# matthewhoung/inference-arena

Measured on AMD Instinct MI355X. Metric: req/sec (whole node) + P50/P99 e2e latency, YOLOv5n→MobileNetV2 at 1/2/4/8 GPU, higher is better.
Workload: dtype fp32

## Files before the change

### csrc/bindings.cpp

```cpp
#include <pybind11/numpy.h>
#include <pybind11/pybind11.h>
#include <pybind11/stl.h>

#include <cstring>
#include <malloc.h>
#include <map>
#include <mutex>

#include "kernels/launch.h"
#include "runtime/executor.h"
#include "runtime/echo_instance.h"
#include "runtime/http_front.h"
#include "runtime/http_loadgen.h"
#include "runtime/ipc_buffer.h"
#include "runtime/peer.h"
#include "runtime/jpeg_decode.h"
#include "runtime/jpeg_ingest.h"
#include "runtime/batcher.h"
#include "runtime/split.h"
#include "runtime/crash_trace.h"

namespace py = pybind11;
using namespace arena;

namespace arena {
void bind_jpeg(py::module& m);
}

namespace {

template <typename T>
T get(const py::dict& d, const char* k, T dflt) {
  if (!d.contains(k)) return dflt;
  py::object o = d[k];
  if (o.is_none()) return dflt;
  return o.cast<T>();
}
template <typename T>
T req(const py::dict& d, const char* k) {
  if (!d.contains(k)) throw std::runtime_error(std::string("missing kernel parameter '") + k + "'");
  return d[k].cast<T>();
}
template <typename P>
P ptr(const py::dict& d, const char* k) {
  return reinterpret_cast<P>(get<uintptr_t>(d, k, 0));
}
hipStream_t stream_of(const py::dict& d) { return reinterpret_cast<hipStream_t>(get<uintptr_t>(d, "stream", 0)); }

void py_conv2d(const py::dict& d) {
  ConvParams p{};
  p.x = ptr<const void*>(d, "x");
  p.B = req<int>(d, "B");
  p.H = req<int>(d, "H");
  p.W = req<int>(d, "W");
  p.xs = req<int>(d, "xs");
  p.Cin = req<int>(d, "Cin");
  p.w = ptr<const void*>(d, "w");
  p.Kpad = req<int>(d, "Kpad");
  p.bias = ptr<const float*>(d, "bias");
  p.y = ptr<void*>(d, "y");
  p.Ho = req<int>(d, "Ho");
  p.Wo = req<int>(d, "Wo");
  p.ys = req<int>(d, "ys");
  p.Cout = req<int>(d, "Cout");
  p.Cout_pad = req<int>(d, "Cout_pad");
  p.KH = req<int>(d, "KH");
  p.KW = req<int>(d, "KW");
  p.stride = get<int>(d, "stride", 1);
  p.pad_t = get<int>(d, "pad_t", 0);
  p.pad_l = get<int>(d, "pad_l", 0);
  p.res = ptr<const void*>(d, "res");
  p.rs = get<int>(d, "rs", 0);
  p.y2 = ptr<void*>(d, "y2");
  p.y2s = get<int>(d, "y2s", 0);
  p.act = get<int>(d, "act", 0);
  p.f32out = get<int>(d, "f32out", 0);
  p.bdev = ptr<const int*>(d, "bdev");
  p.impl = get<int>(d, "impl", 0);
  p.pw_w = ptr<const void*>(d, "pw_w");
  p.pw_bias = ptr<const float*>(d, "pw_bias");
  p.pw_y = ptr<void*>(d, "pw_y");
  p.pw_ys = get<int>(d, "pw_ys", 0);
  p.pw_cout = get<int>(d, "pw_cout", 0);
  p.pw_kpad = get<int>(d, "pw_kpad", 0);
  p.pw_act = get<int>(d, "pw_act", 0);
  p.gate = ptr<const float*>(d, "gate");
  p.gate_n = get<int>(d, "gate_n", 0);
  p.gate_min = get<float>(d, "gate_min", 0.f);
  p.n_lo = get<int>(d, "n_lo", 0);
  p.n_hi = get<int>(d, "n_hi", 0);
  p.marks = ptr<const int*>(d, "marks");
  p.mark_uh = get<int>(d, "mark_uh", 0);
  p.mark_uw = get<int>(d, "mark_uw", 0);
  p.mark_halo = get<int>(d, "mark_halo", 0);
  p.w3 = ptr<const void*>(d, "w3");
  p.sk_ws = ptr<float*>(d, "sk_ws");
  p.sk_ws_bytes = get<int64_t>(d, "sk_ws_bytes", 0);
  prepare_kernels();
  if (get<int>(d, "f32", 0))
    conv2d_f32(p, stream_of(d));
  else
    conv2d(p, stream_of(d));
}

void py_head_mark(const py::dict& d) {
  HeadMarkParams p{};
  const std::vector<uintptr_t> logits = req<std::vector<uintptr_t>>(d, "logits");
  const std::vector<uintptr_t> marks = req<std::vector<uintptr_t>>(d, "marks");
  const std::vector<int> H = req<std::vector<int>>(d, "H"), W = req<std::vector<int>>(d, "W");
  const std::vector<int> ps = req<std::vector<int>>(d, "ps");
  const size_t n = logits.size();
  if (n < 1 || n > (size_t)kMarkMaxLevels || marks.size() != n || H.size() != n || W.size() != n || ps.size() != n)
    throw std::runtime_error("head_mark: 1..3 levels, one entry per level in every list");
  p.n_levels = (int)n;
  for (size_t l = 0; l < n; ++l) {
    p.logits[l] = reinterpret_cast<const float*>(logits[l]);
    p.marks[l] = reinterpret_cast<int*>(marks[l]);
    p.H[l] = H[l];
    p.W[l] = W[l];
    p.ps[l] = ps[l];
  }
  p.n = req<int>(d, "n");
  p.gate_min = req<float>(d, "gate_min");
  p.B = req<int>(d, "B");
  p.bdev = ptr<const int*>(d, "bdev");
  head_mark(p, stream_of(d));
}

void py_dwconv(const py::dict& d) {
  DwParams p{};
  p.x = ptr<const void*>(d, "x");
  p.B = req<int>(d, "B");
  p.H = req<int>(d, "H");
  p.W = req<int>(d, "W");
  p.xs = req<int>(d, "xs");
  p.C = req<int>(d, "C");
  p.w = ptr<const void*>(d, "w");
  p.bias = ptr<const float*>(d, "bias");
  p.y = ptr<void*>(d, "y");
  p.Ho = req<int>(d, "Ho");
  p.Wo = req<int>(d, "Wo");
  p.ys = req<int>(d, "ys");
  p.stride = get<int>(d, "stride", 1);
  p.act = get<int>(d, "act", 0);
  p.bdev = ptr<const int*>(d, "bdev");
  if (get<int>(d, "f32", 0))
    dwconv3x3_f32(p, stream_of(d));
  else
    dwconv3x3(p, stream_of(d));
}

void py_ir_block(const py::dict& d) {
  IrParams p{};
  p.x = ptr<const void*>(d, "x");
  p.x_cs = req<int>(d, "x_cs");
  p.H = req<int>(d, "H");
  p.W = req<int>(d, "W");
  p.inp = req<int>(d, "inp");
  p.inp_pad = req<int>(d, "inp_pad");
  p.hid_pad = req<int>(d, "hid_pad");
  p.oup = req<int>(d, "oup");
  p.oup_pad = req<int>(d, "oup_pad");
  p.stride = req<int>(d, "stride");
  p.expand = req<int>(d, "expand");
  p.res = get<int>(d, "res", 0);
  p.we = ptr<const void*>(d, "we");
  p.be = ptr<const float*>(d, "be");
  p.wd = ptr<const void*>(d, "wd");
  p.bd = ptr<const float*>(d, "bd");
  p.wp = ptr<const void*>(d, "wp");
  p.bp = ptr<const float*>(d, "bp");
  p.y = ptr<void*>(d, "y");
  p.y_cs = req<int>(d, "y_cs");
  p.Ho = req<int>(d, "Ho");
  p.Wo = req<int>(d, "Wo");
  p.B = req<int>(d, "B");
  p.bdev = ptr<const int*>(d, "bdev");
  p.x3w = get<int>(d, "x3w", 0);
  p.x_parts = get<int>(d, "x_parts", 0);
  p.y_parts = get<int>(d, "y_parts", 0);
  prepare_kernels();
  if (get<int>(d, "f32", 0))
    ir_block_f32(p, stream_of(d));
  else
    ir_block(p, stream_of(d));
}

void py_c3_block(const py::dict& d) {
  C3Params p{};
  p.x = ptr<const void*>(d, "x");
  p.xs = req<int>(d, "xs");
  p.B = req<int>(d, "B");
  p.H = req<int>(d, "H");
  p.W = req<int>(d, "W");
  p.bdev = ptr<const int*>(d, "bdev");
  p.C1 = req<int>(d, "C1");
  p.CH = req<int>(d, "CH");
  p.NB = req<int>(d, "NB");
  p.res = req<int>(d, "res");
  p.w12 = ptr<const void*>(d, "w12");
  p.b12 = ptr<const float*>(d, "b12");
  p.wb1[0] = p.wb1[1] = ptr<const void*>(d, "wb1");
  p.bb1[0] = p.bb1[1] = ptr<const float*>(d, "bb1");
  p.wb2[0] = p.wb2[1] = ptr<const void*>(d, "wb2");
  p.bb2[0] = p.bb2[1] = ptr<const float*>(d, "bb2");
  p.w3 = ptr<const void*>(d, "w3");
  p.b3 = ptr<const float*>(d, "b3");
  p.y = ptr<void*>(d, "y");
  p.ys = req<int>(d, "ys");
  prepare_kernels();
  if (get<int>(d, "f32", 0))
    c3_x3(p, stream_of(d));
  else
    c3_fused(p, stream_of(d));
}

void py_sppf(const py::dict& d) {
  SppfParams p{};
  p.buf = ptr<void*>(d, "buf");
  p.B = req<int>(d, "B");
  p.H = req<int>(d, "H");
  p.W = req<int>(d, "W");
  p.xs = req<int>(d, "xs");
  p.C = req<int>(d, "C");
  p.bdev = ptr<const int*>(d, "bdev");
  if (get<int>(d, "f32", 0))
    sppf_pool_f32(p, stream_of(d));
  else
    sppf_pool(p, stream_of(d));
}

void py_letterbox(const py::dict& d) {
  LetterboxParams p{};
  p.pool = ptr<const uint8_t*>(d, "pool");
  p.meta = ptr<const ImageMeta*>(d, "meta");
  p.ctrl = ptr<const Ctrl*>(d, "ctrl");
  p.out = ptr<void*>(d, "out");
  p.B = req<int>(d, "B");
  p.T = req<int>(d, "T");
  p.f32 = get<int>(d, "f32", 0);
  letterbox_s2d(p, stream_of(d));
}

void py_decode(const py::dict& d) {
  DecodeParams p{};
  auto heads = req<std::vector<uintptr_t>>(d, "head");
  auto hw = req<std::vector<int>>(d, "hw");
  auto xs = req<std::vector<int>>(d, "xs");
  auto st = req<std::vector<float>>(d, "strides");
  for (int l = 0; l < 3; ++l) {
    p.head[l] = (const void*)heads.at(l);
    p.hw[l] = hw.at(l);
    p.xs[l] = xs.at(l);
    p.stride[l] = st.at(l);
  }
  p.B = req<int>(d, "B");
  p.conf_thr = req<float>(d, "conf_thr");
  p.cand = ptr<Candidate*>(d, "cand");
  p.cand_count = ptr<int*>(d, "cand_count");
  p.cand_cap = req<int>(d, "cand_cap");
  p.ctrl = ptr<const Ctrl*>(d, "ctrl");
  p.f32 = get<int>(d, "f32", 0);
  detect_decode(p, stream_of(d));
}

void py_yolo_raw(const py::dict& d) {
  YoloRawParams p{};
  auto heads = req<std::vector<uintptr_t>>(d, "head");
  auto hw = req<std::vector<int>>(d, "hw");
  auto xs = req<std::vector<int>>(d, "xs");
  auto st = req<std::vector<float>>(d, "strides");
  for (int l = 0; l < 3; ++l) {
    p.head[l] = (const void*)heads.at(l);
    p.hw[l] = hw.at(l);
    p.xs[l] = xs.at(l);
    p.stride[l] = st.at(l);
  }
  p.B = req<int>(d, "B");
  p.out = ptr<void*>(d, "out");
  p.out_stride = req<size_t>(d, "out_stride");
  p.ctrl = ptr<const Ctrl*>(d, "ctrl");
  p.f32 = get<int>(d, "f32", 0);
  yolo_raw(p, stream_of(d));
}

void py_tensor_in(const py::dict& d) {
  TensorInParams p{};
  p.pool = ptr<const uint8_t*>(d, "pool");
  p.meta = ptr<const ImageMeta*>(d, "meta");
  p.ctrl = ptr<const Ctrl*>(d, "ctrl");
  p.out = ptr<void*>(d, "out");
  p.B = req<int>(d, "B");
  p.S = req<int>(d, "S");
  p.f32 = get<int>(d, "f32", 0);
  tensor_in_s2d(p, stream_of(d));
}

void py_nms(const py::dict& d) {
  prepare_kernels();
  NmsParams p{};
  p.cand = ptr<const Candidate*>(d, "cand");
  p.cand_count = ptr<const int*>(d, "cand_count");
  p.cand_cap = req<int>(d, "cand_cap");
  p.meta = ptr<const ImageMeta*>(d, "meta");
  p.B = req<int>(d, "B");
  p.iou_thr = req<float>(d, "iou_thr");
  p.det = ptr<Detection*>(d, "det");
  p.det_count = ptr<int*>(d, "det_count");
  p.max_det = req<int>(d, "max_det");
  p.ctrl = ptr<const Ctrl*>(d, "ctrl");
  nms(p, stream_of(d));
}

void py_crop_plan(const py::dict& d) {
  CropPlanParams p{};
  p.det = ptr<Detection*>(d, "det");
  p.det_count = ptr<int*>(d, "det_count");
  p.max_det = req<int>(d, "max_det");
  p.meta = ptr<const ImageMeta*>(d, "meta");
  p.B = req<int>(d, "B");
  p.crops = ptr<CropRef*>(d, "crops");
  p.ctrl = ptr<Ctrl*>(d, "ctrl");
  p.crop_cap = req<int>(d, "crop_cap");
  p.whole = get<int>(d, "whole", 0);
  crop_plan(p, stream_of(d));
}

void py_crop_gather(const py::dict& d) {
  CropGatherParams p{};
  p.pool = ptr<const uint8_t*>(d, "pool");
  p.meta = ptr<const ImageMeta*>(d, "meta");
  p.crops = ptr<const CropRef*>(d, "crops");
  p.ctrl = ptr<const Ctrl*>(d, "ctrl");
  p.out = ptr<void*>(d, "out");
  p.cap = req<int>(d, "cap");
  p.S = req<int>(d, "S");
  auto mean = req<std::vector<float>>(d, "mean");
  auto inv_std = req<std::vector<float>>(d, "inv_std");
  for (int c = 0; c < 3; ++c) {
    p.mean[c] = mean.at(c);
    p.inv_std[c] = inv_std.at(c);
  }
  p.f32 = get<int>(d, "f32", 0);
  crop_gather_s2d(p, stream_of(d));
}

void py_head_pool(const py::dict& d) {
  HeadPoolParams p{};
  p.x = ptr<const void*>(d, "x");
  p.xs = req<int>(d, "xs");
  p.HW = req<int>(d, "HW");
  p.K = req<int>(d, "K");
  p.w = ptr<const void*>(d, "w");
  p.Kpad = req<int>(d, "Kpad");
  p.bias = ptr<const float*>(d, "bias");
  p.N = req<int>(d, "N");
  p.Npad = req<int>(d, "Npad");
  p.y = ptr<void*>(d, "y");
  p.ys = req<int>(d, "ys");
  p.act = get<int>(d, "act", 0);
  p.B = req<int>(d, "B");
  p.bdev = ptr<const int*>(d, "bdev");
  prepare_kernels();
  if (get<int>(d, "f32", 0))
    head_pool_f32(p, stream_of(d));
  else
    head_pool(p, stream_of(d));
}

void py_avgpool(const py::dict& d) {
  AvgPoolParams p{};
  p.x = ptr<const void*>(d, "x");
  p.B = req<int>(d, "B");
  p.HW = req<int>(d, "HW");
  p.C = req<int>(d, "C");
  p.y = ptr<void*>(d, "y");
  p.bdev = ptr<const int*>(d, "bdev");
  p.f32 = get<int>(d, "f32", 0);
  global_avgpool(p, stream_of(d));
}

void py_topk(const py::dict& d) {
  TopkParams p{};
  p.logits = ptr<const float*>(d, "logits");
  p.B = req<int>(d, "B");
  p.N = req<int>(d, "N");
  p.ld = req<int>(d, "ld");
  p.out = ptr<TopkResult*>(d, "out");
  p.ctrl = ptr<const Ctrl*>(d, "ctrl");
  p.bdev = ptr<const int*>(d, "bdev");
  topk_softmax(p, stream_of(d));
}

ExecutorConfig config_from(const py::dict& d) {
  ExecutorConfig c;
  c.device = get<int>(d, "device", c.device);
  c.max_batch = get<int>(d, "max_batch", c.max_batch);
  c.max_det = get<int>(d, "max_det", c.max_det);
  c.cand_cap = get<int>(d, "cand_cap", c.cand_cap);
  c.crop_cap_per_image = get<int>(d, "crop_cap_per_image", c.crop_cap_per_image);
  c.min_crop_cap = get<int>(d, "min_crop_cap", c.min_crop_cap);
  c.pool_bytes_per_image = get<int64_t>(d, "pool_bytes_per_image", c.pool_bytes_per_image);
  c.pool_factor = get<int>(d, "pool_factor", c.pool_factor);
  c.det_size = get<int>(d, "det_size", c.det_size);
  c.cls_size = get<int>(d, "cls_size", c.cls_size);
  c.host_threads = get<int>(d, "host_threads", c.host_threads);
  c.raw_out_bytes = get<int64_t>(d, "raw_out_bytes", c.raw_out_bytes);
  return c;
}

ResultCallback py_result_cb(py::function cb) {
  std::shared_ptr<py::function> pycb(new py::function(std::move(cb)), [](py::function* fn) {
    py::gil_scoped_acquire gil;
    delete fn;
  });
  return [pycb](RequestResult&& r) {
    py::gil_scoped_acquire gil;
    py::dict d;
    d["id"] = r.id;
    d["error"] = r.error;
    d["det_count"] = r.det_count;
    const int k = (int)r.det.size();
    py::array_t<float> det({k, 8});
    if (k) std::memcpy(det.mutable_data(), r.det.data(), sizeof(Detection) * k);
    const int t = (int)r.topk.size();
    py::array_t<int32_t> ti({t, 5});
    py::array_t<float> tl({t, 5}), tp({t, 5});
    for (int i = 0; i < t; ++i)
      for (int j = 0; j < 5; ++j) {
        ti.mutable_at(i, j) = r.topk[i].idx[j];
        tl.mutable_at(i, j) = r.topk[i].logit[j];
        tp.mutable_at(i, j) = r.topk[i].prob[j];
      }
    d["det"] = det;
    d["topk_idx"] = ti;
    d["topk_logit"] = tl;
    d["topk_prob"] = tp;
    if (!r.raw.empty()) {
      py::array_t<uint8_t> raw((py::ssize_t)r.raw.size());
      std::memcpy(raw.mutable_data(), r.raw.data(), r.raw.size());
      d["raw"] = raw;
    }
    d["batch_size"] = r.batch_size;
    d["queue_us"] = r.queue_us;
    d["compute_us"] = r.compute_us;
    d["detection_ms"] = r.det_ms;
    d["classification_ms"] = r.cls_ms;
    try {
      (*pycb)(d);
    } catch (py::error_already_set& e) {
      e.discard_as_unraisable("DynamicBatcher callback");
    }
  };
}

struct JpegHolder {
  JpegInfo info;
  std::vector<int16_t> coef;
};
using JpegKeep = std::vector<std::shared_ptr<JpegHolder>>;
std::mutex g_jkeep_mu;
std::map<std::pair<const void*, int>, JpegKeep> g_jkeep;
struct JpegSet;
std::map<std::pair<const void*, int>, std::shared_ptr<JpegSet>> g_jset_keep;

struct JpegSet {
  struct Item {
    JpegInfo info;
    int16_t* coef = nullptr;
    bool pinned = false;
    ~Item() {
      if (coef == nullptr) return;
      if (pinned) (void)hipHostFree(coef);
      else std::free(coef);
    }
  };
  std::vector<std::shared_ptr<Item>> items;
};

std::shared_ptr<JpegSet> make_jpeg_set(const py::list& uploads, bool pinned) {
  auto set = std::make_shared<JpegSet>();
  for (auto h : uploads) {
    const std::string data = h.cast<std::string>();
    auto it = std::make_shared<JpegSet::Item>();
    std::string err;
    JpegStatus st = jpeg_parse((const uint8_t*)data.data(), data.size(), it->info, err);
    if (st != JpegStatus::Ok) throw py::value_error("JpegSet: not decodable by the split decoder: " + err);
    const bool compact = jpeg_compact_enabled();
    const size_t bytes =
        std::max<size_t>(2, compact ? (size_t)jpeg_compact_capacity(it->info) : (size_t)it->info.coef_count * 2);
    void* p = nullptr;
    if (pinned && hipHostMalloc(&p, bytes, hipHostMallocPortable) == hipSuccess) {
      it->pinned = true;
    } else {
      (void)hipGetLastError();
      p = std::malloc(bytes);
      if (p == nullptr) throw std::bad_alloc();
    }
    it->coef = (int16_t*)p;
    st = compact ? jpeg_decode_compact((const uint8_t*)data.data(), data.size(), it->info, (uint8_t*)it->coef, err)
                 : jpeg_decode_coefs((const uint8_t*)data.data(), data.size(), it->info, it->coef, err);
    if (st != JpegStatus::Ok) throw py::value_error("JpegSet: entropy decode failed: " + err);
    set->items.push_back(it);
  }
  return set;
}

std::vector<InputImage> images_from(const py::list& imgs, std::vector<py::array>& keep, JpegKeep* jkeep = nullptr) {
  std::vector<InputImage> v;
  v.reserve(imgs.size());
  for (auto h : imgs) {
    if (py::isinstance<py::bytes>(h)) {
      if (jkeep == nullptr) throw std::runtime_error("JPEG inputs are not accepted here");
      const std::string data = h.cast<std::string>();
      auto jh = std::make_shared<JpegHolder>();
      std::string err;
      JpegStatus st = jpeg_parse((const uint8_t*)data.data(), data.size(), jh->info, err);
      if (st == JpegStatus::Ok) {
        jh->coef.assign((size_t)jh->info.coef_count, 0);
        st = jpeg_decode_coefs((const uint8_t*)data.data(), data.size(), jh->info, jh->coef.data(), err);
      }
      if (st != JpegStatus::Ok) throw py::value_error("JPEG input not decodable by the split decoder: " + err);
      InputImage im{(const uint8_t*)jh->coef.data(), jh->info.out_height, jh->info.out_width};
      im.jpeg = &jh->info;
      jkeep->push_back(jh);
      v.push_back(im);
      continue;
    }
    py::array a = py::array::ensure(h, py::array::c_style);
    if (!a) throw std::runtime_error("inputs must be numpy arrays");
    InputImage im;
    if (a.ndim() == 3 && a.shape(2) == 3 && a.itemsize() == 1) {
      im.h = (int)a.shape(0);
      im.w = (int)a.shape(1);
    } else if (a.ndim() == 3 && a.shape(0) == 3 && a.itemsize() == 4 && a.shape(1) == a.shape(2)) {
      im.h = im.w = (int)a.shape(1);
      im.bytes = (int64_t)a.nbytes();
    } else {
      throw std::runtime_error("inputs must be uint8 HxWx3 images or float32 [3,S,S] tensors");
    }
    keep.push_back(a);
    im.data = (const uint8_t*)a.data();
    v.push_back(im);
  }
  return v;
}

py::dict result_to_py(const BatchResult& r, int max_det) {
  py::dict out;
  const int n = r.n_images;
  py::array_t<int32_t> cnt(n);
  std::memcpy(cnt.mutable_data(), r.det_count.data(), sizeof(int) * n);
  py::array_t<float> det({n, max_det, 8});
  static_assert(sizeof(Detection) == 32, "Detection layout");
  if (n) std::memcpy(det.mutable_data(), r.det.data(), sizeof(Detection) * (size_t)n * max_det);
  py::array_t<int32_t> offs(n + 1);
  std::memcpy(offs.mutable_data(), r.crop_offset.data(), sizeof(int) * (n + 1));
  static_assert(sizeof(TopkResult) == 64, "TopkResult layout");
  py::array_t<int32_t> tk_idx({(int)r.topk.size(), 5});
  py::array_t<float> tk_logit({(int)r.topk.size(), 5});
  py::array_t<float> tk_prob({(int)r.topk.size(), 5});
  for (size_t i = 0; i < r.topk.size(); ++i)
    for (int k = 0; k < 5; ++k) {
      tk_idx.mutable_at(i, k) = r.topk[i].idx[k];
      tk_logit.mutable_at(i, k) = r.topk[i].logit[k];
      tk_prob.mutable_at(i, k) = r.topk[i].prob[k];
    }
  out["det_count"] = cnt;
  out["det"] = det;
  out["crop_offset"] = offs;
  out["topk_idx"] = tk_idx;
  out["topk_logit"] = tk_logit;
  out["topk_prob"] = tk_prob;
  out["gpu_ms"] = r.gpu_ms;
  out["detection_ms"] = r.det_ms;
  out["classification_ms"] = r.cls_ms;
  out["bucket"] = r.bucket;
  out["total_crops"] = r.total_crops;
  if (!r.raw.empty()) {
    py::array_t<uint8_t> raw((py::ssize_t)r.raw.size());
    std::memcpy(raw.mutable_data(), r.raw.data(), r.raw.size());
    out["raw"] = raw;
  }
  return out;
}

}

PYBIND11_MODULE(_C, m) {
  m.doc() = "MI355X-native kernels and runtime of inference_arena_amd (gfx950)";
  {
    const char* e = std::getenv("ARENA_CRASH_TRACE");
    if (e == nullptr || std::strcmp(e, "0") != 0) arena::install_crash_trace();
  }
  m.def("install_crash_trace", &arena::install_crash_trace);
  m.def("crash_trace_installed", &arena::crash_trace_installed);
  m.def("dump_thread_stack", &arena::dump_thread_stack, py::arg("tid"));
  m.def("malloc_trim", []() {
    py::gil_scoped_release nogil;
    return malloc_trim(0) != 0;
  });
  m.def("malloc_info", []() {
    const struct mallinfo2 mi = mallinfo2();
    py::dict d;
    d["arena"] = (uint64_t)mi.arena;
    d["mmapped"] = (uint64_t)mi.hblkhd;
    d["in_use"] = (uint64_t)mi.uordblks;
    d["free"] = (uint64_t)mi.fordblks;
    d["releasable"] = (uint64_t)mi.keepcost;
    return d;
  });
  bind_jpeg(m);
  m.def("conv2d", &py_conv2d);
  m.def("set_conv_impl", &set_conv_impl);
  m.def("get_conv_impl", &get_conv_impl);
  m.def("dwconv3x3", &py_dwconv);
  m.def("sppf_pool", &py_sppf);
  m.def("ir_block", &py_ir_block);
  m.def("c3_block", &py_c3_block);
  m.def("set_conv_pw", &set_conv_pw);
  m.def("set_conv_v3", &set_conv_v3);
  m.def("set_ir_wave", &set_ir_wave);
  m.def("set_irx_parts", &set_irx_parts);
  m.def("set_irx_slices_big", &set_irx_slices_big);
  m.def("set_ir_t14", &set_ir_t14);
  m.def("set_ir_crop", &set_ir_crop);
  m.def("set_ir_s2k16", &set_ir_s2k16);
  m.def("set_ir_crop_split", &set_ir_crop_split);
  m.def("set_head_gate", &set_head_gate);
  m.def("get_head_gate", &get_head_gate);
  m.def(
      "head_gate_min",
      [](float conf_thr) -> py::object {
        float g;
        if (!head_gate_min(conf_thr, &g)) return py::none();
        return py::float_(g);
      },
      py::arg("conf_thr"), "the gate's logit threshold for a confidence threshold (float32); None: the gate is off");
  m.def(
      "head_gate_pairs",
      [](py::array_t<int64_t, py::array::c_style> ops) {
        if (ops.ndim() != 2 || ops.shape(1) != kOpFields) throw std::runtime_error("ops must be int64 [n, OP_FIELDS]");
        py::list out;
        for (const HeadGatePair& gp : head_gate_pairs(ops.data(), (int)ops.shape(0), kOpFields))
          out.append(py::make_tuple(gp.box, gp.cls, gp.level));
        return out;
      },
      py::arg("ops"), "[(box conv op, class conv op, level)] of a program's records");
  m.def("set_head_split", &set_head_split);
  m.def("get_head_split", &get_head_split);
  m.attr("HEAD_SPLIT_MIN_BUCKET") = kHeadSplitMinBucket;
  m.attr("HEAD_SPLIT_BOX_IMPL") = kF32X3HP + kHeadSplitBoxVariant;
  m.attr("HEAD_SPLIT_CLS_IMPL") = kF32X3HP + kHeadSplitClsVariant;
  m.attr("MARK_CELL") = kMarkCell;
  m.def("head_mark", &py_head_mark);
  m.def(
      "head_gate_first_convs",
      [](py::array_t<int64_t, py::array::c_style> ops) {
        if (ops.ndim() != 2 || ops.shape(1) != kOpFields) throw std::runtime_error("ops must be int64 [n, OP_FIELDS]");
        py::list out;
        for (const HeadGatePair& gp : head_gate_pairs(ops.data(), (int)ops.shape(0), kOpFields))
          out.append(head_gate_first_conv(ops.data(), (int)ops.shape(0), kOpFields, gp));
        return out;
      },
      py::arg("ops"), "per head-gate pair of a program's records: the op of its first head conv, or -1");
  m.def(
      "head_marks_needed",
      [](py::array_t<int, py::array::c_style | py::array::forcecast> marks, int H, int W, int th, int tw, int uh,
         int uw, int halo) {
        if (H <= 0 || W <= 0 || th <= 0 || tw <= 0 || uh <= 0 || uw <= 0 || halo < 0 || marks.ndim() != 2 ||
            marks.shape(0) != head_mark_cells(H) || marks.shape(1) != head_mark_cells(W))
          throw std::runtime_error("head_marks_needed: marks must be int32 [ceil(H / 8), ceil(W / 8)], sizes > 0");
        const int nty = (H + th - 1) / th, ntx = (W + tw - 1) / tw;
        py::array_t<bool> out({nty, ntx});
        auto o = out.mutable_unchecked<2>();
        for (int ty = 0; ty < nty; ++ty)
          for (int tx = 0; tx < ntx; ++tx)
            o(ty, tx) = head_marks_needed(marks.data(), H, W, ty, tx, th, tw, uh, uw, halo);
        return out;
      },
      py::arg("marks"), py::arg("H"), py::arg("W"), py::arg("th"), py::arg("tw"), py::arg("uh"), py::arg("uw"),
      py::arg("halo"),
      "bool [tiles_y, tiles_x]: the th x tw producer tiles of one image that a continuing uh x uw consumer tile, "
      "grown by halo pixels, reads (the host oracle of the x3hp mark gate)");
  m.attr("HEAD_BOX_CHANNELS") = kHeadBoxChannels;
  m.attr("HEAD_CLS_CHANNELS") = kHeadClsChannels;
  m.def("letterbox_s2d", &py_letterbox);
  m.def("detect_decode", &py_decode);
  m.def("yolo_raw", &py_yolo_raw);
  m.def("tensor_in_s2d", &py_tensor_in);
  m.def("nms", &py_nms);
  m.def("crop_plan", &py_crop_plan);
  m.def("crop_gather_s2d", &py_crop_gather);
  m.def("global_avgpool", &py_avgpool);
  m.def("head_pool", &py_head_pool);
  m.def("topk_softmax", &py_topk);
  m.attr("SIZEOF_IMAGE_META") = (int)sizeof(ImageMeta);
  m.attr("SIZEOF_CTRL") = (int)sizeof(Ctrl);
  m.attr("SIZEOF_CANDIDATE") = (int)sizeof(Candidate);
  m.attr("SIZEOF_DETECTION") = (int)sizeof(Detection);
  m.attr("SIZEOF_CROPREF") = (int)sizeof(CropRef);
  m.attr("SIZEOF_TOPK") = (int)sizeof(TopkResult);
  m.attr("OP_FIELDS") = kOpFields;

  py::class_<Executor, std::shared_ptr<Executor>>(m, "Executor")
      .def(py::init([](const py::dict& cfg) { return std::make_shared<Executor>(config_from(cfg)); }))
      .def("set_weights",
           [](Executor& e, py::array_t<uint8_t, py::array::c_style> blob) { e.set_weights(blob.data(), blob.size()); })
      .def("set_weights_device",
           [](Executor& e, uintptr_t ptr, size_t bytes) {
             py::gil_scoped_release nogil;
             e.set_weights_device((const void*)ptr, bytes);
           })
      .def("weights_host",
           [](Executor& e) {
             std::vector<uint8_t> v;
             {
               py::gil_scoped_release nogil;
               v = e.weights_host();
             }
             return py::bytes((const char*)v.data(), v.size());
           })
      .def("set_program",
           [](Executor& e, py::array_t<int64_t, py::array::c_style> ops, py::array_t<int64_t, py::array::c_style> cls) {
             if (ops.ndim() != 2 || ops.shape(1) != kOpFields || cls.ndim() != 2 || cls.shape(1) != kOpFields)
               throw std::runtime_error("programs must be int64 [n, OP_FIELDS]");
             e.set_program(ops.data(), (int)ops.shape(0), cls.data(), (int)cls.shape(0));
           })
      .def("add_bucket",
           [](Executor& e, int B, py::array_t<int64_t, py::array::c_style> offs, int64_t arena_bytes,
              py::object impl) {
             if (impl.is_none()) {
               e.add_bucket(B, offs.data(), (int)offs.size(), arena_bytes);
             } else {
               const std::vector<int> v = impl.cast<std::vector<int>>();
               e.add_bucket(B, offs.data(), (int)offs.size(), arena_bytes, &v);
             }
           },
           py::arg("B"), py::arg("offsets"), py::arg("arena_bytes"), py::arg("impl") = py::none())
      .def("buckets", &Executor::buckets)
      .def("crop_cap_for", &Executor::crop_cap_for)
      .def("submit",
           [](Executor& e, const py::list& imgs) {
             std::vector<py::array> keep;
             JpegKeep jkeep;
             auto v = images_from(imgs, keep, &jkeep);
             int slot;
             {
               py::gil_scoped_release nogil;
               slot = e.submit(v);
             }
             if (!jkeep.empty()) {
               std::lock_guard<std::mutex> lk(g_jkeep_mu);
               g_jkeep[{(const void*)&e, slot}] = std::move(jkeep);
             }
             return slot;
           })
      .def("submit_jpeg_set",
           [](Executor& e, std::shared_ptr<JpegSet> set, const std::vector<int>& idx) {
             std::vector<InputImage> v;
             v.reserve(idx.size());
             for (int i : idx) {
               if (i < 0 || i >= (int)set->items.size()) throw py::index_error("submit_jpeg_set: index out of range");
               const auto& it = set->items[i];
               InputImage im{(const uint8_t*)it->coef, it->info.out_height, it->info.out_width};
               im.jpeg = &it->info;
               v.push_back(im);
             }
             int slot;
             {
               py::gil_scoped_release nogil;
               slot = e.submit(v);
             }
             std::lock_guard<std::mutex> lk(g_jkeep_mu);
             g_jset_keep[{(const void*)&e, slot}] = set;
             return slot;
           })
      .def("collect",
           [](Executor& e, int slot) {
             BatchResult r;
             {
               py::gil_scoped_release nogil;
               r = e.collect(slot);
             }
             {
               std::lock_guard<std::mutex> lk(g_jkeep_mu);
               g_jkeep.erase({(const void*)&e, slot});
               g_jset_keep.erase({(const void*)&e, slot});
             }
             return result_to_py(r, e.config().max_det);
           })
      .def("run",
           [](Executor& e, const py::list& imgs) {
             std::vector<py::array> keep;
             JpegKeep jkeep;
             auto v = images_from(imgs, keep, &jkeep);
             BatchResult r;
             {
               py::gil_scoped_release nogil;
               r = e.run(v);
             }
             return result_to_py(r, e.config().max_det);
           })
      .def("replay",
           [](Executor& e, int B, int slot, int iters) {
             py::gil_scoped_release nogil;
             e.replay(B, slot, iters);
           })
      .def("num_slots", &Executor::num_slots)
      .def("synchronize",
           [](Executor& e) {
             py::gil_scoped_release nogil;
             e.synchronize();
           })
      .def("arena_ptr", &Executor::arena_ptr)
      .def("read_arena",
           [](Executor& e, int B, int64_t offset, size_t bytes) {
             py::array_t<uint8_t> out(bytes);
             {
               py::gil_scoped_release nogil;
               e.read_arena(B, offset, out.mutable_data(), bytes);
             }
             return out;
           })
      .def("weights_ptr", &Executor::weights_ptr)
      .def("set_peer_stage", &Executor::set_peer_stage)
      .def("device", &Executor::device)
      .def("submit_peer",
           [](Executor& e, Executor& src, int slot) {
             py::gil_scoped_release nogil;
             return e.submit_peer(src, slot);
           })
      .def("submit_device",
           [](Executor& e, const std::vector<std::tuple<uintptr_t, int, int, int>>& images,
              const std::vector<py::array_t<float, py::array::c_style | py::array::forcecast>>& boxes) {
             if (images.size() != boxes.size()) throw std::runtime_error("submit_device: one box array per image");
             std::vector<Executor::DeviceImage> imgs;
             std::vector<std::vector<Detection>> dets(images.size());
             for (size_t i = 0; i < images.size(); ++i) {
               Executor::DeviceImage d;
               d.ptr = std::get<0>(images[i]);
               d.h = std::get<1>(images[i]);
               d.w = std::get<2>(images[i]);
               d.device = std::get<3>(images[i]);
               imgs.push_back(d);
               const auto& b = boxes[i];
               if (b.size() == 0) continue;
               if (b.ndim() != 2 || b.shape(1) != 6) throw std::runtime_error("submit_device: boxes must be [k, 6]");
               const float* q = b.data();
               for (ssize_t k = 0; k < b.shape(0); ++k, q += 6) {
                 Detection dd{};
                 dd.x1 = q[0];
                 dd.y1 = q[1];
                 dd.x2 = q[2];
                 dd.y2 = q[3];
                 dd.conf = q[4];
                 dd.cls = (int)q[5];
                 dets[i].push_back(dd);
               }
             }
             py::gil_scoped_release nogil;
             return e.submit_device(imgs, dets);
           })
      .def("conv_choices", &Executor::conv_choices)
      .def("exec_order", &Executor::exec_order, py::arg("B"),
           "program op indices in the order bucket B's graphs launch them")
      .def("gated_ops", &Executor::gated_ops, py::arg("B"), "ops of bucket B that run with a tile gate")
      .def("launch_order", &Executor::launch_order, py::arg("B"),
           "every kernel launch of bucket B's graphs in order as (op, kind): 0 the whole op, 1 / 2 the class / "
           "box window of a split first head conv, 3 the cell marks launched before op's box conv")
      .def("stream", &Executor::stream);

  py::class_<SplitInstance, std::shared_ptr<SplitInstance>>(m, "SplitInstance")
      .def(py::init([](std::shared_ptr<Executor> det, std::shared_ptr<Executor> cls) {
        return std::make_shared<SplitInstance>(det, cls);
      }))
      .def("submit",
           [](SplitInstance& s, const py::list& imgs) {
             std::vector<py::array> keep;
             auto v = images_from(imgs, keep);
             py::gil_scoped_release nogil;
             return s.submit(v);
           })
      .def("collect",
           [](SplitInstance& s, int slot) {
             BatchResult r;
             {
               py::gil_scoped_release nogil;
               r = s.collect(slot);
             }
             return result_to_py(r, s.max_det());
           })
      .def("num_slots", &SplitInstance::num_slots)
      .def("buckets", &SplitInstance::buckets);

  py::class_<JpegSet, std::shared_ptr<JpegSet>>(m, "JpegSet")
      .def(py::init(&make_jpeg_set), py::arg("uploads"), py::arg("pinned") = true,
           "JPEG uploads entropy-decoded once into (pinned) host buffers, for Executor.submit_jpeg_set")
      .def("__len__", [](const JpegSet& s) { return s.items.size(); })
      .def("coef_bytes", [](const JpegSet& s, int i) { return (int64_t)jpeg_payload_bytes(s.items.at(i)->info); })
      .def_property_readonly("pinned", [](const JpegSet& s) {
        for (const auto& it : s.items)
          if (!it->pinned) return false;
        return true;
      });

  py::class_<EchoInstance, std::shared_ptr<EchoInstance>>(m, "EchoInstance")
      .def(py::init<int, int, int, int, int64_t>(), py::arg("slots") = 2, py::arg("max_batch") = 32,
           py::arg("max_det") = 4, py::arg("latency_us") = 0, py::arg("staging_cap") = 0);

  py::class_<DynamicBatcher>(m, "DynamicBatcher")
      .def(py::init([](py::list executors, const py::dict& cfg) {
             std::vector<std::shared_ptr<BatchInstance>> inst;
             for (auto h : executors) {
               if (py::isinstance<SplitInstance>(h))
                 inst.push_back(h.cast<std::shared_ptr<SplitInstance>>());
               else if (py::isinstance<EchoInstance>(h))
                 inst.push_back(h.cast<std::shared_ptr<EchoInstance>>());
               else
                 inst.push_back(h.cast<std::shared_ptr<Executor>>());
             }
             BatcherConfig c;
             c.max_batch = get<int>(cfg, "max_batch", c.max_batch);
             c.preferred = get<std::vector<int>>(cfg, "preferred", {});
             c.max_queue_delay_us = get<int64_t>(cfg, "max_queue_delay_us", c.max_queue_delay_us);
             c.idle_queue_delay_us = get<int64_t>(cfg, "idle_queue_delay_us", c.idle_queue_delay_us);
             c.max_queue_size = get<int64_t>(cfg, "max_queue_size", c.max_queue_size);
             c.overlap = get<int>(cfg, "overlap", c.overlap);
             return new DynamicBatcher(inst, c);
           }),
           py::keep_alive<1, 2>())
      .def("enqueue",
           [](DynamicBatcher& b, py::array img_in, py::function cb, uintptr_t export_to) {
             py::array img = py::array::ensure(img_in, py::array::c_style);
             int h = 0, w = 0;
             int64_t bytes = 0;
             if (img && img.ndim() == 3 && img.shape(2) == 3 && img.itemsize() == 1) {
               h = (int)img.shape(0);
               w = (int)img.shape(1);
             } else if (img && img.ndim() == 3 && img.shape(0) == 3 && img.itemsize() == 4 &&
                        img.shape(1) == img.shape(2)) {
               h = w = (int)img.shape(1);
               bytes = (int64_t)img.nbytes();
             } else {
               throw std::runtime_error("input must be a uint8 HxWx3 image or a float32 [3,S,S] tensor");
             }
             ResultCallback f = py_result_cb(std::move(cb));
             const uint8_t* data = (const uint8_t*)img.data();
             py::gil_scoped_release nogil;
             return b.enqueue(data, h, w, std::move(f), bytes, (uint8_t*)export_to);
           },
           py::arg("img"), py::arg("cb"), py::arg("export_to") = 0)
      .def("stats",
           [](DynamicBatcher& b) {
             BatcherStats s = b.stats();
             py::dict d;
             d["requests"] = s.requests;
             d["batches"] = s.batches;
             d["rejected"] = s.rejected;
             d["failed"] = s.failed;
             d["queue_depth"] = s.queue_depth;
             d["mean_batch"] = s.batches ? s.sum_batch / s.batches : 0.0;
             d["mean_queue_us"] = s.requests ? s.sum_queue_us / s.requests : 0.0;
             d["mean_compute_us"] = s.batches ? s.sum_compute_us / s.batches : 0.0;
             d["batch_hist"] = s.batch_hist;
             d["device_faults"] = s.device_faults;
             d["last_error"] = s.last_error;
             return d;
           })
      .def("shutdown", [](DynamicBatcher& b) {
        py::gil_scoped_release nogil;
        b.shutdown();
      });

  py::class_<JpegIngest>(m, "JpegIngest")
      .def(py::init([](DynamicBatcher& batcher, const py::dict& cfg) {
             IngestConfig c;
             c.threads = get<int>(cfg, "threads", c.threads);
             c.jpeg_device = get<bool>(cfg, "jpeg_device", c.jpeg_device);
             c.max_image_pixels = get<int64_t>(cfg, "max_image_pixels", c.max_image_pixels);
             c.buffer_cap = get<int64_t>(cfg, "buffer_cap", c.buffer_cap);
             int ndev = 0;
             const bool gpu = hipGetDeviceCount(&ndev) == hipSuccess && ndev > 0;
             (void)hipGetLastError();
             if (get<bool>(cfg, "pinned", gpu)) {
               c.host_alloc = [](size_t n) -> void* {
                 void* p = nullptr;
                 if (hipHostMalloc(&p, n, hipHostMallocPortable) != hipSuccess) {
                   (void)hipGetLastError();
                   return nullptr;
                 }
                 return p;
               };
               c.host_free = [](void* p) { (void)hipHostFree(p); };
             }
             py::gil_scoped_release nogil;
             return new JpegIngest(&batcher, c);
           }),
           py::keep_alive<1, 2>())
      .def(
          "submit",
          [](JpegIngest& g, py::bytes upload, py::function done, py::function fallback, uintptr_t export_to) {
            std::string u = upload;
            std::shared_ptr<py::function> fb(new py::function(std::move(fallback)), [](py::function* fn) {
              py::gil_scoped_acquire gil;
              delete fn;
            });
            ResultCallback cb = py_result_cb(std::move(done));
            py::gil_scoped_release nogil;
            g.submit(std::move(u), std::move(cb), [fb](std::string&&) {
              py::gil_scoped_acquire gil;
              try {
                (*fb)();
              } catch (py::error_already_set& e) {
                e.discard_as_unraisable("JpegIngest fallback");
              }
            }, (uint8_t*)export_to);
          },
          py::arg("upload"), py::arg("done"), py::arg("fallback"), py::arg("export_to") = 0,
          "Split-decode `upload` into the batcher: done(result dict) after its batch; fallback() (no arguments) "
          "when the split decoder does not cover the format (the caller decodes and enqueues it itself).")
      .def("stats",
           [](JpegIngest& g) {
             IngestStats s = g.stats();
             py::dict d;
             d["native"] = s.native;
             d["fallback"] = s.fallback;
             d["errors"] = s.errors;
             d["cpu_decode_ms"] = s.cpu_decode_ms;
             return d;
           })
      .def("stop", [](JpegIngest& g) {
        py::gil_scoped_release nogil;
        g.stop();
      });

  py::class_<IpcBuffer>(m, "IpcBuffer")
      .def(py::init<size_t, int>(), py::arg("bytes"), py::arg("device") = 0)
      .def("handle", [](const IpcBuffer& b) { return py::bytes(b.handle()); })
      .def_property_readonly("ptr", &IpcBuffer::ptr)
      .def_property_readonly("size", &IpcBuffer::size)
      .def_property_readonly("device", &IpcBuffer::device)
      .def("write",
           [](IpcBuffer& b, size_t off, py::buffer data) {
             py::buffer_info bi = data.request();
             const size_t n = (size_t)bi.size * (size_t)bi.itemsize;
             py::gil_scoped_release nogil;
             b.write(off, bi.ptr, n);
           })
      .def("read", [](const IpcBuffer& b, size_t off, size_t n) {
        std::string out(n, '\0');
        {
          py::gil_scoped_release nogil;
          b.read(off, out.data(), n);
        }
        return py::bytes(out);
      });
  m.def("ipc_open", [](py::bytes handle, int device, int src_device) {
    return ipc_open(std::string(handle), device, src_device);
  }, py::arg("handle"), py::arg("device") = 0, py::arg("src_device") = -1);
  m.def("ipc_close", &ipc_close);
  m.def("ipc_open_range", [](py::bytes handle, int device, int src_device) {
    const uintptr_t p = ipc_open(std::string(handle), device, src_device);
    return py::make_tuple(p, ipc_mapped_bytes(p));
  }, py::arg("handle"), py::arg("device") = 0, py::arg("src_device") = -1,
     "ipc_open + the mapped size: (device pointer, bytes); src_device >= 0 is checked for peer access first");
  m.def("can_access_peer", &hip_can_access_peer, py::arg("dst"), py::arg("src"), "hipDeviceCanAccessPeer");
  m.def("require_peer_access", [](int dst, int src, const std::string& what, py::object can) {
    PeerQuery q = hip_can_access_peer;
    if (!can.is_none()) q = [can](int d, int s) { py::gil_scoped_acquire g; return can(d, s).cast<int>(); };
    require_peer_access(dst, src, what.c_str(), q);
  }, py::arg("dst"), py::arg("src"), py::arg("what") = "peer copy", py::arg("can_access") = py::none(),
     "runtime/peer.h policy; can_access(dst, src) -> int overrides hipDeviceCanAccessPeer (tests)");

  auto bodies_py = [](const BodyCapture& c) {
    py::list body;
    for (const std::string& b : c.body) body.append(py::bytes(b));
    py::array_t<int64_t> at((py::ssize_t)c.at.size());
    for (size_t i = 0; i < c.at.size(); ++i) at.mutable_data()[i] = c.at[i];
    py::dict d;
    d["body"] = body;
    d["at"] = at;
    return d;
  };
  py::class_<HttpLoadGen>(m, "HttpLoadGen")
      .def(py::init([](const py::dict& cfg, const py::list& requests) {
             LoadGenConfig c;
             c.host = get<std::string>(cfg, "host", c.host);
             c.port = get<int>(cfg, "port", c.port);
             c.users = get<int>(cfg, "users", c.users);
             c.threads = get<int>(cfg, "threads", c.threads);
             c.max_requests = get<int64_t>(cfg, "max_requests", c.max_requests);
             c.keep_bodies = get<bool>(cfg, "keep_bodies", c.keep_bodies);
             std::vector<std::string> reqs;
             for (auto r : requests) reqs.push_back(r.cast<std::string>());
             return new HttpLoadGen(c, std::move(reqs));
           }))
      .def("start", [](HttpLoadGen& g) {
        py::gil_scoped_release nogil;
        g.start();
      })
      .def(
          "stop",
          [](HttpLoadGen& g, double timeout_s) {
            py::gil_scoped_release nogil;
            g.stop(timeout_s);
          },
          py::arg("timeout_s") = 30.0)
      .def("completed", &HttpLoadGen::completed)
      .def("connect_failures", &HttpLoadGen::connect_failures)
      .def("capture_until", &HttpLoadGen::capture_until, py::arg("n"))
      .def("bodies", [bodies_py](HttpLoadGen& g) { return bodies_py(g.bodies()); })
      .def(
          "wait_completed",
          [](HttpLoadGen& g, int64_t n, double timeout_s) {
            py::gil_scoped_release nogil;
            return g.wait_completed(n, timeout_s);
          },
          py::arg("n"), py::arg("timeout_s") = 600.0)
      .def(
          "records",
          [](HttpLoadGen& g, int64_t from, int64_t to) {
            std::vector<LoadGenRecord> r = g.records(from, to);
            py::array_t<double> t((py::ssize_t)r.size());
            py::array_t<float> lat((py::ssize_t)r.size());
            py::array_t<int16_t> st((py::ssize_t)r.size()), dets((py::ssize_t)r.size());
            for (size_t i = 0; i < r.size(); ++i) {
              t.mutable_data()[i] = r[i].t_done;
              lat.mutable_data()[i] = r[i].latency;
              st.mutable_data()[i] = r[i].status;
              dets.mutable_data()[i] = r[i].dets;
            }
            py::dict d;
            d["t_done"] = t;
            d["latency"] = lat;
            d["status"] = st;
            d["dets"] = dets;
            return d;
          },
          py::arg("from") = 0, py::arg("to") = -1);

  auto records_py = [](const std::vector<LoadGenRecord>& r) {
    py::array_t<double> t((py::ssize_t)r.size());
    py::array_t<float> lat((py::ssize_t)r.size());
    py::array_t<int16_t> st((py::ssize_t)r.size()), dets((py::ssize_t)r.size());
    for (size_t i = 0; i < r.size(); ++i) {
      t.mutable_data()[i] = r[i].t_done;
      lat.mutable_data()[i] = r[i].latency;
      st.mutable_data()[i] = r[i].status;
      dets.mutable_data()[i] = r[i].dets;
    }
    py::dict d;
    d["t_done"] = t;
    d["latency"] = lat;
    d["status"] = st;
    d["dets"] = dets;
    return d;
  };
  py::class_<LocalLoadGen>(m, "LocalLoadGen")
      .def(py::init([](HttpFrontEnd& fe, const py::list& uploads, int users) {
             std::vector<std::string> u;
             for (auto r : uploads) u.push_back(r.cast<std::string>());
             return new LocalLoadGen(&fe, std::move(u), users);
           }),
           py::keep_alive<1, 2>())
      .def("start", [](LocalLoadGen& g) {
        py::gil_scoped_release nogil;
        g.start();
      })
      .def(
// ... 176 lines not shown
```

### csrc/kernels/conv_f32.hip

```cpp
#include <algorithm>
#include <cstdlib>
#include <stdexcept>
#include <string>

#include "common.h"
#include "launch.h"
#include "letterbox.h"

namespace arena {

__device__ __forceinline__ float4 load_f4_or_zero(const float* p, const float* safe, bool ok) {
  const float4 v = *(const float4*)(ok ? p : safe);
  return ok ? v : make_float4(0.f, 0.f, 0.f, 0.f);
}

__device__ __forceinline__ float f4_get(const float4& v, int s) {
  return s == 0 ? v.x : s == 1 ? v.y : s == 2 ? v.z : v.w;
}

__device__ __forceinline__ int xcd_remap(int bx, int nx) {
  const int q = nx / 8, r = nx % 8, x = bx % 8, y = bx / 8;
  return (x < r ? x * (q + 1) : r * (q + 1) + (x - r) * q) + y;
}

// ... 1089 lines not shown
  const int M = live_batch(p.B, p.bdev) * HWo;
  const int tiles = (M + 15) / 16;
  int t = blockIdx.x * 4 + wave;
  if (blockIdx.x * 4 >= tiles) return;

  const float* __restrict__ w = (const float*)p.w;
  for (int i = tid; i < BN * K / 4; i += STR_THREADS) {
    const int row = i / (K / 4), k = 4 * (i - row * (K / 4));
    const bool ok = n0 + row < p.Cout_pad && k < p.Kpad;
    float4 v = *(const float4*)(ok ? w + (size_t)(n0 + row) * p.Kpad + k : w);
    if (!ok) v = make_float4(0.f, 0.f, 0.f, 0.f);
    bf16x4 h, m, l;
    bf16 th, tm, tl;
    split3(v.x, th, tm, tl); h[0] = th; m[0] = tm; l[0] = tl;
    split3(v.y, th, tm, tl); h[1] = th; m[1] = tm; l[1] = tl;
    split3(v.z, th, tm, tl); h[2] = th; m[2] = tm; l[2] = tl;
    split3(v.w, th, tm, tl); h[3] = th; m[3] = tm; l[3] = tl;
    uint8_t* r = sW + row * WP + k * 2;
    *(bf16x4*)r = h;
    *(bf16x4*)(r + 2 * K) = m;
    *(bf16x4*)(r + 4 * K) = l;
  }
  float4 bias[NF];
#pragma unroll
  for (int j = 0; j < NF; ++j) {
    const int cb = n0 + j * 16 + 4 * kq;
    bias[j] = cb < p.Cout ? *(const float4*)(p.bias + cb) : make_float4(0.f, 0.f, 0.f, 0.f);
  }
  __syncthreads();

  const float* __restrict__ x = (const float*)p.x;
  const int tstride = gridDim.x * 4;
  int tdy[KS], tdx[KS], tci[KS];
#pragma unroll
  for (int sl = 0; sl < KS; ++sl) {
    const int k0 = sl * 32 + kq * 8, tap = k0 / p.Cin;
    const int kh = tap / p.KW;
    tci[sl] = k0 - tap * p.Cin;
    tdy[sl] = tap < p.KH * p.KW ? kh - p.pad_t : -(1 << 20);
    tdx[sl] = tap - kh * p.KW - p.pad_l;
  }
  float4 b0[KS], b1[KS];
  auto load_b = [&](int tt) {
    const int pix = tt * 16 + col;
    const int b = pix / HWo, r = pix - b * HWo;
    const int oy = r / p.Wo, ox = r - (r / p.Wo) * p.Wo;
    const float* xb = x + (size_t)b * p.H * p.W * p.xs;
#pragma unroll
    for (int sl = 0; sl < KS; ++sl) {
      const int iy = oy * p.stride + tdy[sl], ix = ox * p.stride + tdx[sl];
      const bool ok = pix < M && (unsigned)iy < (unsigned)p.H && (unsigned)ix < (unsigned)p.W;
      const float* ptr = xb + ((size_t)iy * p.W + ix) * p.xs + tci[sl];
      b0[sl] = load_f4_or_zero(ptr, x, ok);
      b1[sl] = load_f4_or_zero(ptr + 4, x, ok);
    }
  };
  if (t < tiles) load_b(t);
  for (; t < tiles; t += tstride) {
    float4 c0[KS], c1[KS];
#pragma unroll
    for (int sl = 0; sl < KS; ++sl) {
      c0[sl] = b0[sl];
      c1[sl] = b1[sl];
    }
    if (t + tstride < tiles) load_b(t + tstride);
    f32x4 acc[NF];
#pragma unroll
    for (int j = 0; j < NF; ++j) acc[j] = f32x4{0.f, 0.f, 0.f, 0.f};
#pragma unroll
    for (int sl = 0; sl < KS; ++sl) {
      const float v[8] = {c0[sl].x, c0[sl].y, c0[sl].z, c0[sl].w, c1[sl].x, c1[sl].y, c1[sl].z, c1[sl].w};
      bf16x8 bh, bm, bl;
#pragma unroll
      for (int i = 0; i < 8; ++i) {
        bf16 th, tm, tl;
        split3(v[i], th, tm, tl);
        bh[i] = th;
        bm[i] = tm;
        bl[i] = tl;
      }
#pragma unroll
      for (int j = 0; j < NF; ++j) {
        const uint8_t* ra = sW + (j * 16 + col) * WP + sl * 64 + kq * 16;
        acc[j] = mfma_x3f(*(const bf16x8*)ra, *(const bf16x8*)(ra + 2 * K), *(const bf16x8*)(ra + 4 * K), bh, bm,
                          bl, acc[j]);
      }
    }
    const int pix = t * 16 + col;
    if (pix >= M) continue;
#pragma unroll
    for (int j = 0; j < NF; ++j) {
      const int cb = n0 + j * 16 + kq * 4;
      if (cb >= p.Cout) continue;
      float v[4] = {acc[j][0] + bias[j].x, acc[j][1] + bias[j].y, acc[j][2] + bias[j].z, acc[j][3] + bias[j].w};
#pragma unroll
      for (int r = 0; r < 4; ++r) v[r] = apply_act(v[r], p.act);
      if (p.res != nullptr) {
        const float4 rv = *(const float4*)((const float*)p.res + (size_t)pix * p.rs + cb);
        v[0] += rv.x; v[1] += rv.y; v[2] += rv.z; v[3] += rv.w;
      }
      const float4 o = make_float4(v[0], v[1], v[2], v[3]);
      *(float4*)((float*)p.y + (size_t)pix * p.ys + cb) = o;
      if (p.y2 != nullptr) {
        const int b = pix / HWo;
        const int r = pix - b * HWo;
        const int oy = r / p.Wo, ox = r - (r / p.Wo) * p.Wo;
        const int W2 = 2 * p.Wo;
        float* y2 = (float*)p.y2;
        const size_t base = ((size_t)(b * 2 * p.Ho + 2 * oy) * W2 + 2 * ox);
        *(float4*)(y2 + base * p.y2s + cb) = o;
        *(float4*)(y2 + (base + 1) * p.y2s + cb) = o;
        *(float4*)(y2 + (base + W2) * p.y2s + cb) = o;
        *(float4*)(y2 + (base + W2 + 1) * p.y2s + cb) = o;
      }
    }
  }
}

template <int NF, int KS>
static void launch_stream(const ConvParams& p, hipStream_t s) {
  constexpr int BN = NF * 16;
  const int ny = (p.Cout_pad + BN - 1) / BN;
  const long tiles = ((long)p.B * p.Ho * p.Wo + 15) / 16;
  const long gx = std::max(1L, std::min((tiles + 3) / 4, (long)std::max(1, 1024 / ny)));
  hipLaunchKernelGGL((conv_x3_stream_kernel<NF, KS>), dim3((unsigned)gx, (unsigned)ny), dim3(STR_THREADS), 0, s, p);
}

template <int NF>
static bool launch_stream_k(const ConvParams& p, hipStream_t s) {
  switch ((p.Kpad + 31) / 32) {
    case 1: launch_stream<NF, 1>(p, s); return true;
    case 2: launch_stream<NF, 2>(p, s); return true;
    case 3: launch_stream<NF, 3>(p, s); return true;
    case 4: launch_stream<NF, 4>(p, s); return true;
    case 5: launch_stream<NF, 5>(p, s); return true;
    case 6: launch_stream<NF, 6>(p, s); return true;
    default: return false;
  }
}

template <int NF, int KC>
__global__ __launch_bounds__(STR_THREADS) void conv_f32_stream_kernel(const ConvParams p) {
  constexpr int BN = NF * 16, K = KC * 16, WPF = K + 8;
  __shared__ __attribute__((aligned(16))) float sW[BN * WPF];
  const int tid = threadIdx.x, lane = tid & 63, wave = tid >> 6;
  const int col = lane & 15, kq = lane >> 4;
  const int n0 = blockIdx.y * BN;
  const int HWo = p.Ho * p.Wo;
  const int M = live_batch(p.B, p.bdev) * HWo;
  const int tiles = (M + 15) / 16;
  int t = blockIdx.x * 4 + wave;
  if (blockIdx.x * 4 >= tiles) return;

  const float* __restrict__ w = (const float*)p.w;
  for (int i = tid; i < BN * K / 4; i += STR_THREADS) {
    const int row = i / (K / 4), k = 4 * (i - row * (K / 4));
    const bool ok = n0 + row < p.Cout_pad && k < p.Kpad;
    *(float4*)&sW[row * WPF + k] = load_f4_or_zero(w + (size_t)(n0 + row) * p.Kpad + k, w, ok);
  }
  float4 bias[NF];
#pragma unroll
  for (int j = 0; j < NF; ++j) {
    const int cb = n0 + j * 16 + 4 * kq;
    bias[j] = cb < p.Cout ? *(const float4*)(p.bias + cb) : make_float4(0.f, 0.f, 0.f, 0.f);
  }
  __syncthreads();

  const float* __restrict__ x = (const float*)p.x;
  const int tstride = gridDim.x * 4;
  int tdy[KC], tdx[KC], tci[KC];
#pragma unroll
  for (int c = 0; c < KC; ++c) {
    const int k0 = c * 16 + kq * 4, tap = k0 / p.Cin;
    const int kh = tap / p.KW;
    tci[c] = k0 - tap * p.Cin;
    tdy[c] = (tap < p.KH * p.KW && k0 < p.Kpad) ? kh - p.pad_t : -(1 << 20);
    tdx[c] = tap - kh * p.KW - p.pad_l;
  }
  float4 bnext[KC];
  auto load_b = [&](int tt) {
    const int pix = tt * 16 + col;
    const int b = pix / HWo, r = pix - b * HWo;
    const int oy = r / p.Wo, ox = r - (r / p.Wo) * p.Wo;
    const float* xb = x + (size_t)b * p.H * p.W * p.xs;
#pragma unroll
    for (int c = 0; c < KC; ++c) {
      const int iy = oy * p.stride + tdy[c], ix = ox * p.stride + tdx[c];
      const bool ok = pix < M && (unsigned)iy < (unsigned)p.H && (unsigned)ix < (unsigned)p.W;
      bnext[c] = load_f4_or_zero(xb + ((size_t)iy * p.W + ix) * p.xs + tci[c], x, ok);
    }
  };
  if (t < tiles) load_b(t);
  for (; t < tiles; t += tstride) {
    float4 bc[KC];
#pragma unroll
    for (int c = 0; c < KC; ++c) bc[c] = bnext[c];
    if (t + tstride < tiles) load_b(t + tstride);
    f32x4 acc[NF];
#pragma unroll
    for (int j = 0; j < NF; ++j) acc[j] = f32x4{0.f, 0.f, 0.f, 0.f};
#pragma unroll
    for (int c = 0; c < KC; ++c) {
#pragma unroll
      for (int j = 0; j < NF; ++j) {
        const float4 a = *(const float4*)&sW[(j * 16 + col) * WPF + c * 16 + kq * 4];
#pragma unroll
        for (int s4 = 0; s4 < 4; ++s4)
          acc[j] = __builtin_amdgcn_mfma_f32_16x16x4f32(f4_get(a, s4), f4_get(bc[c], s4), acc[j], 0, 0, 0);
      }
    }
    const int pix = t * 16 + col;
    if (pix >= M) continue;
#pragma unroll
    for (int j = 0; j < NF; ++j) {
      const int cb = n0 + j * 16 + kq * 4;
      if (cb >= p.Cout) continue;
      float v[4] = {acc[j][0] + bias[j].x, acc[j][1] + bias[j].y, acc[j][2] + bias[j].z, acc[j][3] + bias[j].w};
#pragma unroll
      for (int r = 0; r < 4; ++r) v[r] = apply_act(v[r], p.act);
      if (p.res != nullptr) {
        const float4 rv = *(const float4*)((const float*)p.res + (size_t)pix * p.rs + cb);
        v[0] += rv.x; v[1] += rv.y; v[2] += rv.z; v[3] += rv.w;
      }
      const float4 o = make_float4(v[0], v[1], v[2], v[3]);
      *(float4*)((float*)p.y + (size_t)pix * p.ys + cb) = o;
      if (p.y2 != nullptr) {
        const int b = pix / HWo;
        const int r = pix - b * HWo;
        const int oy = r / p.Wo, ox = r - (r / p.Wo) * p.Wo;
        const int W2 = 2 * p.Wo;
        float* y2 = (float*)p.y2;
        const size_t base = ((size_t)(b * 2 * p.Ho + 2 * oy) * W2 + 2 * ox);
        *(float4*)(y2 + base * p.y2s + cb) = o;
        *(float4*)(y2 + (base + 1) * p.y2s + cb) = o;
        *(float4*)(y2 + (base + W2) * p.y2s + cb) = o;
        *(float4*)(y2 + (base + W2 + 1) * p.y2s + cb) = o;
      }
    }
  }
}

template <int NF, int KC>
static void launch_stream_exact(const ConvParams& p, hipStream_t s) {
  constexpr int BN = NF * 16;
  const int ny = (p.Cout_pad + BN - 1) / BN;
  const long tiles = ((long)p.B * p.Ho * p.Wo + 15) / 16;
  const long gx = std::max(1L, std::min((tiles + 3) / 4, (long)std::max(1, 1024 / ny)));
  hipLaunchKernelGGL((conv_f32_stream_kernel<NF, KC>), dim3((unsigned)gx, (unsigned)ny), dim3(STR_THREADS), 0, s, p);
}

template <int NF>
static bool launch_stream_exact_k(const ConvParams& p, hipStream_t s) {
  const int kc = p.Kpad / 16;
  if (kc <= 1) launch_stream_exact<NF, 1>(p, s);
  else if (kc <= 2) launch_stream_exact<NF, 2>(p, s);
  else if (kc <= 4) launch_stream_exact<NF, 4>(p, s);
  else if (kc <= 6) launch_stream_exact<NF, 6>(p, s);
  else if (kc <= 8) launch_stream_exact<NF, 8>(p, s);
  else if (kc <= 10) launch_stream_exact<NF, 10>(p, s);
  else if (kc <= 12) launch_stream_exact<NF, 12>(p, s);
  else return false;
  return true;
}

static bool f32_stream(const ConvParams& p, hipStream_t s) {
  if (p.Cin % 4 != 0 || p.Kpad > 192 || p.Kpad % 16 != 0 || p.Kpad < p.KH * p.KW * p.Cin || p.xs % 4 != 0)
    return false;
  const int ncf = p.Cout_pad / 16;
  const int nf = ncf <= 5 ? ncf : ncf % 4 == 0 ? 4 : ncf % 3 == 0 ? 3 : ncf % 5 == 0 ? 5 : ncf % 2 == 0 ? 2 : 1;
  switch (nf) {
    case 1: return launch_stream_exact_k<1>(p, s);
    case 2: return launch_stream_exact_k<2>(p, s);
    case 3: return launch_stream_exact_k<3>(p, s);
    case 4: return launch_stream_exact_k<4>(p, s);
    case 5: return launch_stream_exact_k<5>(p, s);
    default: return false;
  }
}

static bool x3_stream(const ConvParams& p, hipStream_t s, int nf_force) {
  if (p.Cin % 8 != 0 || p.Kpad > 192 || p.Kpad < p.KH * p.KW * p.Cin || p.xs % 4 != 0) return false;
  const int ncf = p.Cout_pad / 16;
  const int nf = nf_force ? nf_force
                          : ncf <= 5 ? ncf : ncf % 4 == 0 ? 4 : ncf % 3 == 0 ? 3 : ncf % 5 == 0 ? 5 : ncf % 2 == 0 ? 2 : 1;
  switch (nf) {
    case 1: return launch_stream_k<1>(p, s);
    case 2: return launch_stream_k<2>(p, s);
    case 3: return launch_stream_k<3>(p, s);
    case 4: return launch_stream_k<4>(p, s);
    case 5: return launch_stream_k<5>(p, s);
    default: return false;
  }
}

void conv2d_f32(const ConvParams& p, hipStream_t s) {
  if (p.Cin % 4 != 0 || p.xs % 4 != 0 || p.Kpad % 16 != 0 || p.Cout_pad % 16 != 0 || p.Cout % 4 != 0 ||
      p.Cout > p.Cout_pad || p.ys % 4 != 0)
    throw std::runtime_error("conv2d_f32: unsupported geometry (Cin/xs/ys %4, Kpad %16, Cout_pad %16, Cout %4)");
  if (p.Cin < 16) throw std::runtime_error("conv2d_f32: Cin must be >= 16");
  if (p.Kpad < p.KH * p.KW * p.Cin) throw std::runtime_error("conv2d_f32: Kpad < KH*KW*Cin");
  if ((p.n_lo != 0 || p.n_hi != 0 || p.marks != nullptr) &&
      !(p.pw_w == nullptr && p.impl >= kF32X3HP && p.impl < kF32X3HP + kF32X3HPVariants))
    throw std::runtime_error("conv2d_f32: an output-channel window or a mark gate needs an x3hp variant");
  if (p.pw_w != nullptr) {
    if (p.impl >= kF32X3HRPw && p.impl < kF32X3HRPw + kF32X3HRPwVariants) {
      if (!conv_x3hr_pw(p, s, p.impl - kF32X3HRPw))
        throw std::runtime_error("conv2d_f32: a fused pointwise epilogue needs an x3hr-pw variant that fits the conv");
      return;
    }
    const int v = x3hg_pw_variant(p.impl, p.Cout_pad);
    if (v < 0 || !conv_x3hg_pw(p, s, v))
      throw std::runtime_error("conv2d_f32: a fused pointwise epilogue needs an x3hg-pw variant that fits the conv");
    return;
  }
  if (p.res != nullptr && p.rs % 4 != 0) throw std::runtime_error("conv2d_f32: residual stride % 4");
  if (p.y2 != nullptr && p.y2s % 4 != 0) throw std::runtime_error("conv2d_f32: upsampled stride % 4");
  const long M = (long)p.B * p.Ho * p.Wo;
  if (M <= 0) return;
  if (M > 0x7fffffffL || (long)p.B * p.H * p.W * p.xs > 0x7fffffffL) throw std::runtime_error("conv2d_f32: too large");
  const int ncf = p.Cout_pad / 16;
  if (p.lb_meta != nullptr) {
    if (p.lb_pool == nullptr || !x3_h16(p, s))
      throw std::runtime_error("conv2d_f32: a letterbox-source conv must be a 3x3 s1 pad-1 conv over 16 channels");
    return;
  }
  if (p.impl >= 10) {
    if (p.impl >= kF32X3G && p.impl < kF32X3G + kF32X3GVariants) {
      if (!conv_x3g(p, s, p.impl - kF32X3G))
        throw std::runtime_error("conv2d_f32: not an x3g-eligible conv (needs pre-split weights)");
      return;
    }
    if (p.impl >= kF32X3GSK && p.impl < kF32X3GSK + kF32X3GSKVariants) {
      if (!conv_x3g_sk(p, s, p.impl - kF32X3GSK))
        throw std::runtime_error("conv2d_f32: not a split-K x3g-eligible conv (pre-split weights, workspace)");
      return;
    }
    if (p.impl >= kF32X3HG && p.impl < kF32X3HG + kF32X3HGVariants) {
      if (!conv_x3hg(p, s, p.impl - kF32X3HG))
        throw std::runtime_error("conv2d_f32: not an x3hg-eligible conv (3x3 s1 with pre-split weights)");
      return;
    }
    if (p.impl >= kF32X3HR && p.impl < kF32X3HR + kF32X3HRVariants) {
      if (!conv_x3hr(p, s, p.impl - kF32X3HR))
        throw std::runtime_error("conv2d_f32: not an x3hr-eligible conv (3x3 s1 with pre-split weights)");
      return;
    }
    if (p.impl >= kF32X3HP && p.impl < kF32X3HP + kF32X3HPVariants) {
      if (!conv_x3hp(p, s, p.impl - kF32X3HP))
        throw std::runtime_error("conv2d_f32: not an x3hp-eligible conv (3x3 s1 with pre-split weights)");
      return;
    }
    if (p.impl == kF32X3H16) {
      if (!x3_h16(p, s)) throw std::runtime_error("conv2d_f32: not an x3-h16-eligible conv (3x3 s1 over 16 channels)");
      return;
    }
    if (p.impl == kF32Fc) {
      if (!conv_fc_f32(p, s)) throw std::runtime_error("conv2d_f32: not an FC-eligible conv (1x1 map, Kpad 1280)");
      return;
    }
    if (p.impl == kF32StreamExact) {
      if (!f32_stream(p, s)) throw std::runtime_error("conv2d_f32: not a stream-eligible conv (Cin % 4, Kpad <= 192)");
      return;
    }
    if (p.impl == kF32Stream || p.impl == kF32StreamN2) {
      if (!x3_stream(p, s, p.impl == kF32StreamN2 ? 2 : 0))
        throw std::runtime_error("conv2d_f32: not a stream-eligible conv (Cin % 8, Kpad <= 192)");
      return;
    }
    if (p.impl == kF32X3Halo || p.impl == kF32X3HaloN3 || p.impl == kF32X3HaloN2 || p.impl == kF32X3Halo16 ||
        p.impl == kF32X3Halo16N3) {
      const int nf = (p.impl == kF32X3HaloN3 || p.impl == kF32X3Halo16N3) ? 3 : p.impl == kF32X3HaloN2 ? 2 : 0;
      const int th = (p.impl == kF32X3Halo16 || p.impl == kF32X3Halo16N3) ? 16 : 8;
      if (!x3_halo(p, s, nf, th)) throw std::runtime_error("conv2d_f32: not an x3-halo-eligible conv");
      return;
    }
    if (p.impl == kF32Halo) {
      if (!halo_f32(p, s, true)) throw std::runtime_error("conv2d_f32: not a halo-eligible conv");
      return;
    }
    if (p.impl >= kF32X3) {
      if (p.impl >= kF32X3 + kF32X3Variants || !launch_x3_variant(p, s, M, p.impl - kF32X3))
        throw std::runtime_error("conv2d_f32: unknown x3 variant");
      return;
    }
    if (p.impl >= 10 + kF32Variants || !launch_lds_variant(p, s, M, p.impl - 10)) throw std::runtime_error("conv2d_f32: unknown variant");
    return;
  }
  if (p.impl == 0 && conv_fc_f32(p, s)) return;
  const int impl = p.impl == 1 ? 1 : p.impl >= 2 ? 2 : f32_conv_family();
  if (impl == 2 && halo_f32(p, s)) return;
  if (impl == 2) {
    if (ncf == 1)
      launch_lds_m<1, 4, 1>(p, s, M);
    else if (ncf == 2)
      launch_lds_m<2, 4, 1>(p, s, M);
    else if (ncf == 3 || ncf == 9)
      launch_lds_m<3, 4, 1>(p, s, M);
    else if (ncf == 5)
      launch_lds_m<5, 4, 1>(p, s, M);
    else if (ncf == 6)
      launch_lds_m<3, 2, 2>(p, s, M);
    else
      launch_lds_m<2, 2, 2>(p, s, M);
    return;
  }
  if (ncf % 4 == 0 || ncf > 12)
    launch_f32_wc<4>(p, s, M);
  else if (ncf % 3 == 0)
    launch_f32_wc<3>(p, s, M);
  else if (ncf % 2 == 0)
    launch_f32_wc<2>(p, s, M);
  else if (ncf == 5)
    launch_f32_wc<5>(p, s, M);
  else
    launch_f32_wc<1>(p, s, M);
}

template <int R, int S, int CX>
__global__ __launch_bounds__(256) void dwconv_f32_kernel(const DwParams p) {
  const int B = live_batch(p.B, p.bdev);
  const int cg = p.C >> 2;
  const int strips = (p.Ho + R - 1) / R;
  const int colb = (p.Wo + CX - 1) / CX;
  const int total = B * strips * colb * cg;
  const int tid = blockIdx.x * blockDim.x + threadIdx.x;
  if (tid >= total) return;
  const int g = tid % cg;
  int t = tid / cg;
  const int ox0 = (t % colb) * CX;
  t /= colb;
  const int st = t % strips;
  const int b = t / strips;
  const int c0 = g * 4;
  const int oy0 = st * R;
  const float* x = (const float*)p.x + (size_t)b * p.H * p.W * p.xs + c0;
  const float* w = (const float*)p.w + c0;
  float4 wt[9];
#pragma unroll
  for (int k = 0; k < 9; ++k) wt[k] = *(const float4*)(w + k * p.C);
  const float4 bias = *(const float4*)(p.bias + c0);
  float4 acc[R][CX];
#pragma unroll
  for (int r = 0; r < R; ++r)
#pragma unroll
    for (int c = 0; c < CX; ++c) acc[r][c] = bias;
  constexpr int NIN = (R - 1) * S + 3, NCOL = (CX - 1) * S + 3;
  const int iy0 = oy0 * S - 1, ix0 = ox0 * S - 1;
#pragma unroll
  for (int ri = 0; ri < NIN; ++ri) {
    const int iy = iy0 + ri;
    if ((unsigned)iy >= (unsigned)p.H) continue;
    const float* row = x + (size_t)iy * p.W * p.xs;
    float4 v[NCOL];
#pragma unroll
    for (int q = 0; q < NCOL; ++q)
      v[q] = load_f4_or_zero(row + (ix0 + q) * p.xs, x, (unsigned)(ix0 + q) < (unsigned)p.W);
#pragma unroll
    for (int r = 0; r < R; ++r) {
      const int ky = ri - r * S;
      if (ky < 0 || ky > 2) continue;
#pragma unroll
      for (int c = 0; c < CX; ++c)
#pragma unroll
        for (int kx = 0; kx < 3; ++kx) {
          const float4 ww = wt[ky * 3 + kx];
          const float4 vv = v[c * S + kx];
          acc[r][c].x = fmaf(vv.x, ww.x, acc[r][c].x);
          acc[r][c].y = fmaf(vv.y, ww.y, acc[r][c].y);
          acc[r][c].z = fmaf(vv.z, ww.z, acc[r][c].z);
          acc[r][c].w = fmaf(vv.w, ww.w, acc[r][c].w);
        }
    }
  }
  float* y = (float*)p.y + (size_t)b * p.Ho * p.Wo * p.ys + c0;
#pragma unroll
  for (int r = 0; r < R; ++r) {
    const int oy = oy0 + r;
    if (oy >= p.Ho) break;
#pragma unroll
    for (int c = 0; c < CX; ++c) {
      const int ox = ox0 + c;
      if (ox >= p.Wo) break;
      const float4 a = acc[r][c];
      *(float4*)(y + (size_t)(oy * p.Wo + ox) * p.ys) =
          make_float4(apply_act(a.x, p.act), apply_act(a.y, p.act), apply_act(a.z, p.act), apply_act(a.w, p.act));
    }
  }
}

template <int R, int S, int CX>
static void dw_f32_launch(const DwParams& p, hipStream_t s) {
  const long total = (long)p.B * ((p.Ho + R - 1) / R) * ((p.Wo + CX - 1) / CX) * (p.C / 4);
  if (total <= 0) return;
  if (total >= (1L << 31) || (long)p.B * p.H * p.W * p.xs >= (1L << 31))
    throw std::runtime_error("dwconv3x3_f32: too large");
  hipLaunchKernelGGL((dwconv_f32_kernel<R, S, CX>), dim3((unsigned)((total + 255) / 256)), dim3(256), 0, s, p);
}

static int dw_f32_cols() {
  static const int v = [] {
    const char* e = std::getenv("ARENA_DW_CX");
    return (e != nullptr && std::atoi(e) == 1) ? 1 : 2;
  }();
  return v;
}

void dwconv3x3_f32(const DwParams& p, hipStream_t s) {
  if (p.C % 4 != 0 || p.xs % 4 != 0 || p.ys % 4 != 0)
    throw std::runtime_error("dwconv3x3_f32: C, xs, ys must be multiples of 4");
  const bool two = dw_f32_cols() == 2;
  if (p.stride == 1)
    two ? dw_f32_launch<4, 1, 2>(p, s) : dw_f32_launch<4, 1, 1>(p, s);
  else if (p.stride == 2)
    two ? dw_f32_launch<2, 2, 2>(p, s) : dw_f32_launch<2, 2, 1>(p, s);
  else
    throw std::runtime_error("dwconv3x3_f32: stride must be 1 or 2");
}

constexpr int SPPF_F32_MAX_PIX = 512;

__global__ __launch_bounds__(256) void sppf_f32_kernel(const SppfParams p) {
  __shared__ float4 in[SPPF_F32_MAX_PIX];
  __shared__ float4 h5[SPPF_F32_MAX_PIX], h9[SPPF_F32_MAX_PIX], h13[SPPF_F32_MAX_PIX];
  const int B = live_batch(p.B, p.bdev);
  const int groups = p.C >> 2;
  const int b = blockIdx.x / groups;
  if (b >= B) return;
  const int c0 = (blockIdx.x - b * groups) * 4;
  const int H = p.H, W = p.W, HW = H * W;
  float* buf = (float*)p.buf + (size_t)b * HW * p.xs;
  for (int i = threadIdx.x; i < HW; i += 256) in[i] = *(const float4*)(buf + (size_t)i * p.xs + c0);
  __syncthreads();
  auto mx = [](float4 a, float4 v) {
    return make_float4(fmaxf(a.x, v.x), fmaxf(a.y, v.y), fmaxf(a.z, v.z), fmaxf(a.w, v.w));
  };
  const float4 ninf = make_float4(-INFINITY, -INFINITY, -INFINITY, -INFINITY);
  for (int i = threadIdx.x; i < HW; i += 256) {
    const int y = i / W, xx = i - y * W;
    float4 m5 = ninf, m9 = ninf, m13 = ninf;
#pragma unroll
    for (int dx = -6; dx <= 6; ++dx) {
      const int ix = xx + dx;
      if ((unsigned)ix >= (unsigned)W) continue;
      const float4 v = in[y * W + ix];
      const int a = dx < 0 ? -dx : dx;
      m13 = mx(m13, v);
      if (a <= 4) m9 = mx(m9, v);
      if (a <= 2) m5 = mx(m5, v);
    }
    h5[i] = m5;
    h9[i] = m9;
    h13[i] = m13;
  }
  __syncthreads();
  for (int i = threadIdx.x; i < HW; i += 256) {
    const int y = i / W, xx = i - y * W;
    float4 m5 = ninf, m9 = ninf, m13 = ninf;
#pragma unroll
    for (int dy = -6; dy <= 6; ++dy) {
      const int iy = y + dy;
      if ((unsigned)iy >= (unsigned)H) continue;
      const int j = iy * W + xx;
      const int a = dy < 0 ? -dy : dy;
      m13 = mx(m13, h13[j]);
      if (a <= 4) m9 = mx(m9, h9[j]);
      if (a <= 2) m5 = mx(m5, h5[j]);
    }
    float* o = buf + (size_t)i * p.xs + c0;
    *(float4*)(o + p.C) = m5;
    *(float4*)(o + 2 * p.C) = m9;
    *(float4*)(o + 3 * p.C) = m13;
  }
}

void sppf_pool_f32(const SppfParams& p, hipStream_t s) {
  if (p.C % 4 != 0 || p.xs < 4 * p.C || p.xs % 4 != 0 || p.H * p.W > SPPF_F32_MAX_PIX)
    throw std::runtime_error("sppf_pool_f32: bad geometry (C % 4, xs >= 4C, H*W <= 512)");
  if (p.B <= 0) return;
  hipLaunchKernelGGL(sppf_f32_kernel, dim3((unsigned)(p.B * (p.C / 4))), dim3(256), 0, s, p);
}

}
```

### csrc/kernels/gemm_x3.hip

```cpp
#include <stdexcept>
#include <string>

#include "common.h"
#include "launch.h"

namespace arena {

namespace {

typedef float f32x16 __attribute__((ext_vector_type(16)));
typedef unsigned u32x4 __attribute__((ext_vector_type(4)));

constexpr int XG_PITCH = 104;

__host__ __device__ constexpr int xg_lds_bytes(int BM, int BN) { return 2 * (BM + BN) * XG_PITCH * 2; }

__device__ __forceinline__ int xg_xcd_remap(int bx, int nx) {
  const int q = nx / 8, r = nx % 8, x = bx % 8, y = bx / 8;
  return (x < r ? x * (q + 1) : r * (q + 1) + (x - r) * q) + y;
}

__device__ __forceinline__ f32x4 xg_load_f4(const float* p, const float* safe, bool ok) {
  const f32x4 v = *(const f32x4*)(ok ? p : safe);
  return ok ? v : f32x4{0.f, 0.f, 0.f, 0.f};
}

__device__ __forceinline__ u32x4 xg_load_u4(const bf16* p, const bf16* safe, bool ok) {
  const u32x4 v = *(const u32x4*)(ok ? p : safe);
  return ok ? v : u32x4{0u, 0u, 0u, 0u};
}

__device__ __forceinline__ void xg_split8(const f32x4 a, const f32x4 b, bf16x8& h, bf16x8& m, bf16x8& l) {
  const float v[8] = {a[0], a[1], a[2], a[3], b[0], b[1], b[2], b[3]};
#pragma unroll
  for (int i = 0; i < 8; ++i) {
    const bf16 th = (bf16)v[i];
    const float r = v[i] - (float)th;
    const bf16 tm = (bf16)r;
    h[i] = th;
    m[i] = tm;
    l[i] = (bf16)(r - (float)tm);
  }
}

__device__ __forceinline__ f32x16 xg_mfma_x3(const bf16x8& ah, const bf16x8& am, const bf16x8& al,
                                             const bf16x8& bh, const bf16x8& bm, const bf16x8& bl, f32x16 c) {
  c = __builtin_amdgcn_mfma_f32_32x32x16_bf16(am, bm, c, 0, 0, 0);
  c = __builtin_amdgcn_mfma_f32_32x32x16_bf16(al, bh, c, 0, 0, 0);
  c = __builtin_amdgcn_mfma_f32_32x32x16_bf16(ah, bl, c, 0, 0, 0);
  c = __builtin_amdgcn_mfma_f32_32x32x16_bf16(am, bh, c, 0, 0, 0);
  c = __builtin_amdgcn_mfma_f32_32x32x16_bf16(ah, bm, c, 0, 0, 0);
  return __builtin_amdgcn_mfma_f32_32x32x16_bf16(ah, bh, c, 0, 0, 0);
}

}

template <int WM, int WN, int TM, int TN, bool IL = false, bool SK = false>
__global__ __launch_bounds__(WM * WN * 64) void conv_x3g_kernel(const ConvParams p) {
  constexpr int NT = WM * WN * 64;
  static_assert(WM * WN == 4 || WM * WN == 8, "four or eight waves");
  constexpr int BM = WM * TM * 32, BN = WN * TN * 32;
  constexpr int AI = BM * 4 / NT;
  constexpr int WI = (BN * 12 + NT - 1) / NT;
  static_assert(BM * 4 % NT == 0, "every thread stages the same number of pixel rows");
  extern __shared__ __attribute__((aligned(16))) bf16 xg_lds[];
  bf16* sA = xg_lds;
  bf16* sB = xg_lds + 2 * BM * XG_PITCH;

  const int tid = threadIdx.x, lane = tid & 63, wave = tid >> 6;
  const int wm = wave % WM, wn = wave / WM;
  const int HWo = p.Ho * p.Wo;
  const int M = live_batch(p.B, p.bdev) * HWo;
  const int ntn = (p.Cout_pad + BN - 1) / BN;
  const int nsplit = SK ? p.sk_splits : 1;
  const int ntiles = (int)gridDim.x / nsplit;
  const int split = SK ? (int)blockIdx.x / ntiles : 0;
  const int bx = xg_xcd_remap((int)blockIdx.x - split * ntiles, ntiles);
  const int mt = bx / ntn, nt = bx - mt * ntn;
  const int m0 = mt * BM, n0 = nt * BN;
  if (m0 >= M) return;

  const __amdgpu_buffer_rsrc_t xr = __builtin_amdgcn_make_buffer_rsrc(
      const_cast<void*>(p.x), (short)0, (int)((size_t)p.B * p.H * p.W * p.xs * 4), 0x00020000);
  const int Cin32 = (p.Cin + 31) & ~31;
  const int nk_all = p.KH * p.KW * (Cin32 >> 5);
  const int kc_begin = SK ? split * nk_all / nsplit : 0;
  const int nk = SK ? (split + 1) * nk_all / nsplit - kc_begin : nk_all;
  const __amdgpu_buffer_rsrc_t wr = __builtin_amdgcn_make_buffer_rsrc(
      const_cast<void*>(p.w3), (short)0, (int)((size_t)nk_all * p.Cout_pad * 192), 0x00020000);
  const int Cin = p.Cin, H = p.H, W = p.W, S = p.stride;
  constexpr int kOob = 0x7fffffff & ~15;

  int a_iy[AI], a_ix[AI], a_off[AI];
#pragma unroll
  for (int j = 0; j < AI; ++j) {
    const int i = tid + NT * j;
    const int m = m0 + (i >> 2);
    if (m < M) {
      const int b = m / HWo, r = m - b * HWo;
      const int oy = r / p.Wo, ox = r - oy * p.Wo;
      a_iy[j] = oy * S - p.pad_t;
      a_ix[j] = ox * S - p.pad_l;
      a_off[j] = (((b * H + a_iy[j]) * W + a_ix[j]) * p.xs + 8 * (i & 3)) * 4;
    } else {
      a_iy[j] = -0x40000000;
      a_ix[j] = 0;
      a_off[j] = 0;
    }
  }
  int w_off[WI];
#pragma unroll
  for (int j = 0; j < WI; ++j) {
    const int i = tid + NT * j;
    const int row = i / 12, part = i - (i / 12) * 12;
    w_off[j] = i < BN * 12 ? ((n0 + row) * 96 + part * 8) * 2 : kOob;
  }

  f32x4 ra0[AI][2], ra1[AI][2];
  u32x4 rw0[WI], rw1[WI];
  int ld_ky = 0, ld_kx = 0, ld_c0 = 0;
  if (SK) {
    const int cpt = Cin32 >> 5, tap = kc_begin / cpt;
    ld_c0 = (kc_begin - tap * cpt) * 32;
    ld_ky = tap / p.KW;
    ld_kx = tap - ld_ky * p.KW;
  }
  auto load = [&](int kc_local, f32x4 (&ra)[AI][2], u32x4 (&rw)[WI]) {
    const int kc = kc_begin + kc_local;
    const int ky = ld_ky, kx = ld_kx, c0 = ld_c0;
    ld_c0 += 32;
    const bool wrap = ld_c0 >= Cin32;
    ld_c0 = wrap ? 0 : ld_c0;
    ld_kx += wrap ? 1 : 0;
    const bool wrap2 = ld_kx == p.KW;
    ld_kx = wrap2 ? 0 : ld_kx;
    ld_ky += wrap2 ? 1 : 0;
    const int step = ((ky * W + kx) * p.xs + c0) * 4;
#pragma unroll
    for (int j = 0; j < AI; ++j) {
      const int i = tid + NT * j;
      const int c = c0 + 8 * (i & 3);
      const bool in = (unsigned)(a_iy[j] + ky) < (unsigned)H && (unsigned)(a_ix[j] + kx) < (unsigned)W;
      const int o0 = in && c < Cin ? a_off[j] + step : kOob;
      const int o1 = in && c + 4 < Cin ? a_off[j] + step + 16 : kOob;
      ra[j][0] = __builtin_bit_cast(f32x4, __builtin_amdgcn_raw_buffer_load_b128(xr, o0, 0, 0));
      ra[j][1] = __builtin_bit_cast(f32x4, __builtin_amdgcn_raw_buffer_load_b128(xr, o1, 0, 0));
    }
    const int wstep = kc * p.Cout_pad * 192;
#pragma unroll
    for (int j = 0; j < WI; ++j) rw[j] = __builtin_amdgcn_raw_buffer_load_b128(wr, w_off[j], wstep, 0);
  };
  auto store = [&](int buf, const f32x4 (&ra)[AI][2], const u32x4 (&rw)[WI]) {
    bf16* a = sA + buf * BM * XG_PITCH;
    bf16* bw = sB + buf * BN * XG_PITCH;
#pragma unroll
    for (int j = 0; j < AI; ++j) {
      const int i = tid + NT * j;
      bf16x8 h, m, l;
      xg_split8(ra[j][0], ra[j][1], h, m, l);
      bf16* d = a + (i >> 2) * XG_PITCH + 8 * (i & 3);
      *(bf16x8*)d = h;
      *(bf16x8*)(d + 32) = m;
      *(bf16x8*)(d + 64) = l;
    }
#pragma unroll
    for (int j = 0; j < WI; ++j) {
      const int i = tid + NT * j;
      if (BN * 12 % NT == 0 || i < BN * 12) {
        const int row = i / 12, part = i - (i / 12) * 12;
        *(u32x4*)(bw + row * XG_PITCH + part * 8) = rw[j];
      }
    }
  };

  f32x16 acc[TM][TN];
#pragma unroll
  for (int a = 0; a < TM; ++a)
#pragma unroll
    for (int b = 0; b < TN; ++b)
#pragma unroll
      for (int r = 0; r < 16; ++r) acc[a][b][r] = 0.f;

  const int fr = lane & 31, fk = 8 * (lane >> 5);
  auto compute = [&](int buf) {
    const bf16* a = sA + buf * BM * XG_PITCH;
    const bf16* bw = sB + buf * BN * XG_PITCH;
#pragma unroll
    for (int ks = 0; ks < 2; ++ks) {
      bf16x8 wh[TN], wmid[TN], wl[TN];
#pragma unroll
      for (int tn = 0; tn < TN; ++tn) {
        const bf16* r = bw + ((wn * TN + tn) * 32 + fr) * XG_PITCH + ks * 16 + fk;
        wh[tn] = *(const bf16x8*)r;
        wmid[tn] = *(const bf16x8*)(r + 32);
        wl[tn] = *(const bf16x8*)(r + 64);
      }
#pragma unroll
      for (int tm = 0; tm < TM; ++tm) {
        const bf16* r = a + ((wm * TM + tm) * 32 + fr) * XG_PITCH + ks * 16 + fk;
        const bf16x8 xh = *(const bf16x8*)r, xm = *(const bf16x8*)(r + 32), xl = *(const bf16x8*)(r + 64);
#pragma unroll
        for (int tn = 0; tn < TN; ++tn) acc[tm][tn] = xg_mfma_x3(wh[tn], wmid[tn], wl[tn], xh, xm, xl, acc[tm][tn]);
      }
    }
  };

  load(0, ra0, rw0);
  if (nk > 1) load(1, ra1, rw1);
  store(0, ra0, rw0);
  __syncthreads();
  int kc = 0;
  constexpr int NMF = TM * TN * 12;
  constexpr int NVA = (AI * 40 + NMF - 1) / NMF;
  auto shape = [&]() {
    if constexpr (IL) {
#pragma unroll
      for (int i = 0; i < NMF; ++i) {
        __builtin_amdgcn_sched_group_barrier(0x008, 1, 0);
        __builtin_amdgcn_sched_group_barrier(0x002, NVA, 0);
        if (i % 4 == 3) __builtin_amdgcn_sched_group_barrier(0x200, 1, 0);
      }
    }
  };
  for (; kc + 1 < nk; kc += 2) {
    load(kc + 2, ra0, rw0);
    compute(0);
    store(1, ra1, rw1);
    shape();
    __syncthreads();
    load(kc + 3, ra1, rw1);
    compute(1);
    store(0, ra0, rw0);
    shape();
    __syncthreads();
  }
  if (kc < nk) compute(0);

  const int kh4 = 4 * (lane >> 5);
  if constexpr (SK) {
    const int Mcap = p.B * HWo;
    float* ws = p.sk_ws + (size_t)split * Mcap * p.Cout_pad;
#pragma unroll
    for (int tm = 0; tm < TM; ++tm) {
      const int m = m0 + (wm * TM + tm) * 32 + fr;
      if (m >= M) continue;
#pragma unroll
      for (int tn = 0; tn < TN; ++tn)
#pragma unroll
        for (int g = 0; g < 4; ++g) {
          const int c = n0 + (wn * TN + tn) * 32 + 8 * g + kh4;
          if (c >= p.Cout) continue;
          *(float4*)(ws + (size_t)m * p.Cout_pad + c) =
              make_float4(acc[tm][tn][4 * g], acc[tm][tn][4 * g + 1], acc[tm][tn][4 * g + 2], acc[tm][tn][4 * g + 3]);
        }
    }
    return;
  }

#pragma unroll
  for (int tm = 0; tm < TM; ++tm) {
    const int m = m0 + (wm * TM + tm) * 32 + fr;
    if (m >= M) continue;
    int b = 0, oy = 0, ox = 0;
    if (p.y2 != nullptr) {
      b = m / HWo;
      const int r = m - b * HWo;
      oy = r / p.Wo;
      ox = r - oy * p.Wo;
    }
#pragma unroll
    for (int tn = 0; tn < TN; ++tn) {
#pragma unroll
      for (int g = 0; g < 4; ++g) {
        const int c = n0 + (wn * TN + tn) * 32 + 8 * g + kh4;
        if (c >= p.Cout) continue;
        const float4 bias = *(const float4*)(p.bias + c);
        float v[4] = {acc[tm][tn][4 * g] + bias.x, acc[tm][tn][4 * g + 1] + bias.y, acc[tm][tn][4 * g + 2] + bias.z,
                      acc[tm][tn][4 * g + 3] + bias.w};
#pragma unroll
        for (int r = 0; r < 4; ++r) v[r] = apply_act(v[r], p.act);
        if (p.res != nullptr) {
          const float4 rv = *(const float4*)((const float*)p.res + (size_t)m * p.rs + c);
          v[0] += rv.x; v[1] += rv.y; v[2] += rv.z; v[3] += rv.w;
        }
        const float4 o = make_float4(v[0], v[1], v[2], v[3]);
        *(float4*)((float*)p.y + (size_t)m * p.ys + c) = o;
        if (p.y2 != nullptr) {
          const int W2 = 2 * p.Wo;
          float* y2 = (float*)p.y2;
          const size_t base = ((size_t)(b * 2 * p.Ho + 2 * oy) * W2 + 2 * ox);
          *(float4*)(y2 + base * p.y2s + c) = o;
          *(float4*)(y2 + (base + 1) * p.y2s + c) = o;
          *(float4*)(y2 + (base + W2) * p.y2s + c) = o;
          *(float4*)(y2 + (base + W2 + 1) * p.y2s + c) = o;
        }
      }
    }
  }
}


__global__ __launch_bounds__(256) void x3g_sk_reduce_kernel(const ConvParams p) {
  const int HWo = p.Ho * p.Wo;
  const int M = live_batch(p.B, p.bdev) * HWo, Mcap = p.B * HWo;
  const int c4n = p.Cout >> 2;
  const int i = (int)blockIdx.x * 256 + (int)threadIdx.x;
  if (i >= M * c4n) return;
  const int m = i / c4n, c = 4 * (i - m * c4n);
  float4 a = *(const float4*)(p.sk_ws + (size_t)m * p.Cout_pad + c);
  for (int k = 1; k < p.sk_splits; ++k) {
    const float4 v = *(const float4*)(p.sk_ws + ((size_t)k * Mcap + m) * p.Cout_pad + c);
    a.x += v.x; a.y += v.y; a.z += v.z; a.w += v.w;
  }
  const float4 bias = *(const float4*)(p.bias + c);
  float v[4] = {a.x + bias.x, a.y + bias.y, a.z + bias.z, a.w + bias.w};
#pragma unroll
  for (int r = 0; r < 4; ++r) v[r] = apply_act(v[r], p.act);
  if (p.res != nullptr) {
    const float4 rv = *(const float4*)((const float*)p.res + (size_t)m * p.rs + c);
    v[0] += rv.x; v[1] += rv.y; v[2] += rv.z; v[3] += rv.w;
  }
  const float4 o = make_float4(v[0], v[1], v[2], v[3]);
  *(float4*)((float*)p.y + (size_t)m * p.ys + c) = o;
  if (p.y2 != nullptr) {
    const int b = m / HWo, r = m - b * HWo, oy = r / p.Wo, ox = r - oy * p.Wo;
    const int W2 = 2 * p.Wo;
    float* y2 = (float*)p.y2;
    const size_t base = ((size_t)(b * 2 * p.Ho + 2 * oy) * W2 + 2 * ox);
    *(float4*)(y2 + base * p.y2s + c) = o;
    *(float4*)(y2 + (base + 1) * p.y2s + c) = o;
    *(float4*)(y2 + (base + W2) * p.y2s + c) = o;
    *(float4*)(y2 + (base + W2 + 1) * p.y2s + c) = o;
  }
}

namespace {

template <int WM, int WN, int TM, int TN, bool IL>
void xg_launch(const ConvParams& p, hipStream_t s) {
  constexpr int BM = WM * TM * 32, BN = WN * TN * 32;
  const long M = (long)p.B * p.Ho * p.Wo;
  const long tiles = ((M + BM - 1) / BM) * ((p.Cout_pad + BN - 1) / BN);
  hipLaunchKernelGGL((conv_x3g_kernel<WM, WN, TM, TN, IL>), dim3((unsigned)tiles), dim3(WM * WN * 64), xg_lds_bytes(BM, BN), s,
                     p);
}

template <int WM, int WN, int TM, int TN>
bool xg_launch_sk(const ConvParams& p, hipStream_t s, int splits) {
  constexpr int BM = WM * TM * 32, BN = WN * TN * 32;
  const long M = (long)p.B * p.Ho * p.Wo;
  const int nk = p.KH * p.KW * ((p.Cin + 31) / 32);
  splits = splits < nk ? splits : nk;
  if (p.sk_ws == nullptr || splits < 2 || (long)splits * M * p.Cout_pad * 4 > p.sk_ws_bytes || p.Cout_pad % 4)
    return false;
  const long tiles = ((M + BM - 1) / BM) * ((p.Cout_pad + BN - 1) / BN);
  ConvParams q = p;
  q.sk_splits = splits;
  hipLaunchKernelGGL((conv_x3g_kernel<WM, WN, TM, TN, false, true>), dim3((unsigned)(tiles * splits)),
                     dim3(WM * WN * 64), xg_lds_bytes(BM, BN), s, q);
  const long items = M * (p.Cout / 4);
  hipLaunchKernelGGL(x3g_sk_reduce_kernel, dim3((unsigned)((items + 255) / 256)), dim3(256), 0, s, q);
  return true;
}

#define XG_SK_VARIANTS(X) \
  X(0, 2, 2, 1, 1, 2)   \
  X(1, 2, 2, 1, 1, 4)  \
  X(2, 2, 2, 1, 1, 8)  \
  X(3, 4, 1, 1, 1, 2)   \
  X(4, 4, 1, 1, 1, 4)  \
  X(5, 4, 1, 1, 1, 8)  \
  X(6, 2, 2, 1, 2, 2)   \
  X(7, 2, 2, 1, 2, 4)  \
  X(8, 2, 2, 1, 2, 8)

#define XG_VARIANTS(X) \
  X(0, 2, 2, 2, 1)      \
  X(1, 2, 2, 2, 2)      \
  X(2, 4, 1, 1, 1)      \
  X(3, 4, 1, 1, 2)      \
  X(4, 2, 2, 1, 2)      \
  X(5, 2, 2, 1, 1)      \
  X(6, 2, 4, 2, 1)      \
  X(7, 4, 2, 1, 2)      \
  X(8, 4, 2, 2, 1)      \
  X(9, 4, 2, 1, 1)


}

bool x3g_supported(const ConvParams& p) {
  const size_t x_bytes = (size_t)p.B * p.H * p.W * p.xs * 4;
  const size_t w_bytes = (size_t)p.KH * p.KW * ((p.Cin + 31) / 32) * p.Cout_pad * 192;
  return p.w3 != nullptr && x_bytes < (1u << 31) - (1u << 20) && w_bytes < (1u << 31) - (1u << 20) && p.Cin % 4 == 0 && p.xs % 4 == 0 && p.Kpad >= p.KH * p.KW * p.Cin &&
         p.Cout % 4 == 0 && p.ys % 4 == 0 &&
         (p.res == nullptr || p.rs % 4 == 0) && (p.y2 == nullptr || p.y2s % 4 == 0) && p.lb_meta == nullptr &&
         p.pw_w == nullptr;
}

bool conv_x3g(const ConvParams& p, hipStream_t s, int v) {
  if (!x3g_supported(p)) return false;
  switch (v) {
#define XG_CASE(V, WM, WN, TM, TN) \
  case V: xg_launch<WM, WN, TM, TN, false>(p, s); return true; \
  case V + 10: xg_launch<WM, WN, TM, TN, true>(p, s); return true;
    XG_VARIANTS(XG_CASE)
#undef XG_CASE
    default: return false;
  }
}

bool conv_x3g_sk(const ConvParams& p, hipStream_t s, int v) {
  if (!x3g_supported(p) || p.Cout % 4) return false;
  switch (v) {
#define XG_SK_CASE(V, WM, WN, TM, TN, S)                                   \
  case V:                                                                  \
    if (!xg_launch_sk<WM, WN, TM, TN>(p, s, S)) xg_launch<WM, WN, TM, TN, false>(p, s); \
    return true;
    XG_SK_VARIANTS(XG_SK_CASE)
#undef XG_SK_CASE
    default: return false;
  }
}

void x3g_prepare() {
#define XG_ATTR(V, WM, WN, TM, TN)                                                                       \
  ARENA_HIP_CHECK(hipFuncSetAttribute((const void*)conv_x3g_kernel<WM, WN, TM, TN, false>,                \
                                      hipFuncAttributeMaxDynamicSharedMemorySize,                         \
                                      xg_lds_bytes(WM * TM * 32, WN * TN * 32)));                         \
  ARENA_HIP_CHECK(hipFuncSetAttribute((const void*)conv_x3g_kernel<WM, WN, TM, TN, true>,                 \
                                      hipFuncAttributeMaxDynamicSharedMemorySize,                         \
                                      xg_lds_bytes(WM * TM * 32, WN * TN * 32)));
  XG_VARIANTS(XG_ATTR)
#undef XG_ATTR
#define XG_SK_ATTR(V, WM, WN, TM, TN, S)                                                                  \
  ARENA_HIP_CHECK(hipFuncSetAttribute((const void*)conv_x3g_kernel<WM, WN, TM, TN, false, true>,          \
                                      hipFuncAttributeMaxDynamicSharedMemorySize,                         \
                                      xg_lds_bytes(WM * TM * 32, WN * TN * 32)));
  XG_SK_VARIANTS(XG_SK_ATTR)
#undef XG_SK_ATTR
}

}
```

### csrc/kernels/launch.h

```cpp
#pragma once
#include <hip/hip_runtime.h>
#include <stdint.h>
#include <stdexcept>
#include <string>

namespace arena {

struct ImageMeta;
struct CropRef;
struct Ctrl;
struct ConvParams {
  const void* x;
  int B, H, W;
  int xs;
  int Cin;
  const void* w;
  int Kpad;
  const float* bias;
  void* y;
  int Ho, Wo, ys;
  int Cout;
  int Cout_pad;
  int KH, KW, stride, pad_t, pad_l;
  const void* res;
  int rs;
  void* y2;
  int y2s;
  int act;
  int f32out;
  const int* bdev;
  int impl;
  const void* pw_w;
  const float* pw_bias;
  void* pw_y;
  int pw_ys, pw_cout, pw_kpad, pw_act;
  const float* gate;
  int gate_n;
  float gate_min;
  int n_lo, n_hi;
  const int* marks;
  int mark_uh, mark_uw, mark_halo;
  const uint8_t* lb_pool;
  const ImageMeta* lb_meta;
  const void* w3;
  float* sk_ws;
  int64_t sk_ws_bytes;
  int sk_splits;
};
void conv2d(const ConvParams& p, hipStream_t s);
void conv_igemm(const ConvParams& p, hipStream_t s);
bool conv_pw(const ConvParams& p, hipStream_t s);
void set_conv_pw(bool v);
bool conv3x3_v3(const ConvParams& p, hipStream_t s);
bool conv_fc(const ConvParams& p, hipStream_t s);
void set_conv_v3(bool v);
void set_conv_impl(int v);
int get_conv_impl();

constexpr int kF32Variants = 16;
constexpr int kF32X3 = 40;
constexpr int kF32X3Variants = 12;
constexpr int kF32Halo = 100;
constexpr int kF32X3Halo = 101;
constexpr int kF32X3HaloN3 = 102;
constexpr int kF32X3HaloN2 = 103;
constexpr int kF32Stream = 104;
constexpr int kF32StreamN2 = 105;
constexpr int kF32Fc = 106;
constexpr int kF32StreamExact = 107;
constexpr int kF32X3Halo16 = 108;
constexpr int kF32X3Halo16N3 = 109;
constexpr int kF32X3H16 = 110;
constexpr int kF32X3G = 111;
constexpr int kF32X3GVariants = 20;
void x3_halo_prepare();
bool x3g_supported(const ConvParams& p);
bool conv_x3g(const ConvParams& p, hipStream_t s, int v);
constexpr int kF32X3GSK = 171;
constexpr int kF32X3GSKVariants = 9;
bool conv_x3g_sk(const ConvParams& p, hipStream_t s, int v);
void x3g_prepare();
constexpr int kF32X3HG = 131;
constexpr int kF32X3HGVariants = 14;
bool x3hg_supported(const ConvParams& p);
bool conv_x3hg(const ConvParams& p, hipStream_t s, int v);
void x3hg_prepare();
constexpr int kF32X3HGPw = 145;
constexpr int kF32X3HGPwVariants = 6;
constexpr int kF32X3HGPwSmall = 181;
constexpr int kF32X3HGPwSmallVariants = 2;
bool conv_x3hg_pw(const ConvParams& p, hipStream_t s, int v);
constexpr int kF32X3HR = 151;
constexpr int kF32X3HRVariants = 10;
constexpr int kF32X3HRPw = 161;
constexpr int kF32X3HRPwVariants = 6;
constexpr int kF32X3HP = 191;
constexpr int kF32X3HPVariants = 10;
bool x3hp_supported(const ConvParams& p);
bool conv_x3hp(const ConvParams& p, hipStream_t s, int v);
void x3hp_prepare();
int x3hg_pw_variant(int impl, int cout_pad);
bool x3hg_pw_tile(int impl, int cout_pad, int* th, int* tw);
struct HeadMarkParams {
  int n_levels;
  const float* logits[3];
  int H[3], W[3], ps[3];
  int* marks[3];
  int n;
  float gate_min;
  int B;
  const int* bdev;
};
void head_mark(const HeadMarkParams& p, hipStream_t s);
bool conv_x3hr(const ConvParams& p, hipStream_t s, int v);
bool conv_x3hr_pw(const ConvParams& p, hipStream_t s, int v);
bool conv_fc_f32(const ConvParams& p, hipStream_t s);
void conv2d_f32(const ConvParams& p, hipStream_t s);

struct DwParams {
  const void* x;
  int B, H, W, xs, C;
  const void* w;
  const float* bias;
  void* y;
  int Ho, Wo, ys, stride, act;
  const int* bdev;
};
void dwconv3x3(const DwParams& p, hipStream_t s);
void dwconv3x3_f32(const DwParams& p, hipStream_t s);

struct IrParams {
  const void* x;
  int x_cs, H, W;
  int inp, inp_pad;
  int hid_pad;
  int oup, oup_pad;
  int stride, expand, res;
  const void* we;
  const float* be;
  const void* wd;
  const float* bd;
  const void* wp;
  const float* bp;
  void* y;
  int y_cs, Ho, Wo;
  int B;
  const int* bdev;
  int x3w;
  int x_parts, y_parts;
  int stem;
  const uint8_t* st_pool;
  const ImageMeta* st_meta;
  const CropRef* st_crops;
  const Ctrl* st_ctrl;
  int st_S;
  float st_mean[3], st_inv_std[3];
  const float* st_w;
  const float* st_b;
};
void ir_block(const IrParams& p, hipStream_t s);
void ir_block_f32(const IrParams& p, hipStream_t s);
bool ir_block_f32_supported(int stride, int inp_pad, int hid_pad, int oup_pad, int expand);
bool ir_block_crop_f32(const IrParams& p, hipStream_t s);
bool ir_block_crop_f32_supported(int H, int stride, int inp_pad, int hid_pad, int oup_pad, int expand);
bool ir_tile_x3(const IrParams& p, hipStream_t s);
bool ir_tile_x3_supported(int stride, int inp_pad, int hid_pad, int oup_pad, int expand);
void ir_tile_x3_prepare();
bool ir_stem_x3(const IrParams& p, hipStream_t s);
bool ir_s2k16_x3(const IrParams& p, hipStream_t s);
void set_ir_s2k16(bool v);
void ir_prepare();
void set_ir_t14(bool v);
void set_ir_crop(bool v);
void set_ir_crop_split(int v);
void set_ir_wave(bool v);
void set_irx_slices_big(int n);
void set_irx_parts(int n);

struct C3Params {
  const void* x;
  int xs;
  int B, H, W;
  const int* bdev;
  int C1, CH, NB, res;
  const void* w12;
  const float* b12;
  const void* wb1[2];
  const float* bb1[2];
  const void* wb2[2];
  const float* bb2[2];
  const void* w3;
  const float* b3;
  void* y;
  int ys;
};
bool c3_fused_supported(int C1, int CH, int NB, bool res, int H, int W);
bool c3_x3_supported(int C1, int CH, int NB, bool res, int H, int W);
void c3_x3(const C3Params& p, hipStream_t s);
void c3_x3_prepare();
void c3_fused(const C3Params& p, hipStream_t s);

struct SppfParams {
  void* buf;
  int B, H, W, xs, C;
  const int* bdev;
};
void sppf_pool(const SppfParams& p, hipStream_t s);
void sppf_pool_f32(const SppfParams& p, hipStream_t s);

struct ImageMeta {
  int64_t offset;
  int h, w;
  int new_w, new_h;
  int pad_w, pad_h;
  float scale;
  float pad_[3];
};
static_assert(sizeof(ImageMeta) == 48, "ImageMeta layout");

struct Ctrl {
  int n_images;
  int n_crops;
  int crop_base;
  int total_crops;
  int pad_[12];
};

struct LetterboxParams {
  const uint8_t* pool;
  const ImageMeta* meta;
  const Ctrl* ctrl;
  void* out;
  int B, T;
  int f32;
};
void letterbox_s2d(const LetterboxParams& p, hipStream_t s);

struct TensorInParams {
  const uint8_t* pool;
  const ImageMeta* meta;
  const Ctrl* ctrl;
  void* out;
  int B, S;
  int f32;
};
void tensor_in_s2d(const TensorInParams& p, hipStream_t s);

struct Candidate {
  float x1, y1, x2, y2;
  float score;
  int cls;
  int anchor;
  int pad_;
};
struct DecodeParams {
  const void* head[3];
  int hw[3];
  int xs[3];
  float stride[3];
  int B;
  float conf_thr;
  Candidate* cand;
  int* cand_count;
  int cand_cap;
  const Ctrl* ctrl;
  int f32;
};
void detect_decode(const DecodeParams& p, hipStream_t s);

struct YoloRawParams {
  const void* head[3];
  int hw[3];
  int xs[3];
  float stride[3];
  int B;
  void* out;
  size_t out_stride;
  const Ctrl* ctrl;
  int f32;
};
void yolo_raw(const YoloRawParams& p, hipStream_t s);

struct Detection {
  float x1, y1, x2, y2;
  float conf;
  int cls;
  float pad_[2];
};
struct NmsParams {
  const Candidate* cand;
  const int* cand_count;
  int cand_cap;
  const ImageMeta* meta;
  int B;
  float iou_thr;
  Detection* det;
  int* det_count;
  int max_det;
  const Ctrl* ctrl;
};
void nms(const NmsParams& p, hipStream_t s);

void prepare_kernels();

struct CropRef {
  int img;
  int x1, y1, x2, y2;
  int det;
  int pad_[2];
};
struct CropPlanParams {
  Detection* det;
  int* det_count;
  int max_det;
  const ImageMeta* meta;
  int B;
  CropRef* crops;
  Ctrl* ctrl;
  int crop_cap;
  int whole;
};
void crop_plan(const CropPlanParams& p, hipStream_t s);

struct CropGatherParams {
  const uint8_t* pool;
  const ImageMeta* meta;
  const CropRef* crops;
  const Ctrl* ctrl;
  void* out;
  int cap, S;
  float mean[3], inv_std[3];
  int f32;
};
void crop_gather_s2d(const CropGatherParams& p, hipStream_t s);

struct StemFusedParams {
  int src;
  const uint8_t* pool;
  const ImageMeta* meta;
  const Ctrl* ctrl;
  const CropRef* crops;
  int cap;
  int S;
  float mean[3], inv_std[3];
  int KS;
  const void* w;
  int Kpad;
  const float* bias;
  int Cout;
  void* y;
  int ys;
  int act;
  const void* w2;
  int Kpad2;
  const float* bias2;
  int Cout2, act2;
  void* y2;
  int y2s;
  const void* ir_wd;
  const float* ir_bd;
  const void* ir_wp;
  const float* ir_bp;
  void* ir_y;
  int ir_ys;
};
void stem_fused(const StemFusedParams& p, hipStream_t s);
void stem_s2_f32(const StemFusedParams& p, hipStream_t s);
void stem_s2_f32_prepare();

struct AvgPoolParams {
  const void* x;
  int B, HW, C;
  void* y;
  const int* bdev;
  int f32;
};
void global_avgpool(const AvgPoolParams& p, hipStream_t s);

struct HeadPoolParams {
// ... 44 lines not shown
```

### csrc/runtime/executor.cpp

```cpp
#include "executor.h"
#include "peer.h"

#include <pthread.h>
#include <sys/prctl.h>

#include <algorithm>
#include <chrono>
#include <cmath>
#include <cstdio>
#include <cstdlib>
#include <cstring>
#include <thread>
#include <stdexcept>
#include <string>

#include "../kernels/common.h"
#include "../kernels/jpeg_desc.h"
#include "jpeg_decode.h"
#include "trace.h"

namespace arena {

namespace {
float bits_to_float(int64_t v) {
  uint32_t u = (uint32_t)v;
  float f;
  std::memcpy(&f, &u, 4);
  return f;
}
size_t align_up(size_t v, size_t a) { return (v + a - 1) / a * a; }
constexpr size_t kCtrlBytes = 256;
static_assert(kHgOpConv == OP_CONV && kHgOpDecode == OP_DECODE && kHgDtypeField == kDtypeField &&
                  sizeof(OpRecord) == sizeof(int64_t) * kOpFields,
              "head_gate.h reads the executor's op records");
bool g_head_gate = [] {
  const char* e = std::getenv("ARENA_HEAD_GATE");
  return e == nullptr || std::atoi(e) != 0;
}();
int g_head_split = [] {
  const char* e = std::getenv("ARENA_HEAD_SPLIT");
  return e == nullptr ? 1 : std::max(0, std::min(2, std::atoi(e)));
}();
}

void set_head_gate(bool v) { g_head_gate = v; }
bool get_head_gate() { return g_head_gate; }
void set_head_split(int v) { g_head_split = std::max(0, std::min(2, v)); }
int get_head_split() { return g_head_split; }

Executor::Executor(const ExecutorConfig& cfg) : cfg_(cfg) {
  if (cfg_.max_batch <= 0 || cfg_.max_batch > 1024) throw std::runtime_error("Executor: max_batch out of range");
  if (cfg_.cand_cap > 16384) throw std::runtime_error("Executor: cand_cap > 16384");
  ARENA_HIP_CHECK(hipSetDevice(cfg_.device));
  prepare_kernels();
  max_B_ = cfg_.max_batch;
  {
    int khz = 0;
    if (hipDeviceGetAttribute(&khz, hipDeviceAttributeWallClockRate, cfg_.device) == hipSuccess && khz > 0)
      wall_khz_ = (double)khz;
  }
  {
    const char* e = std::getenv("ARENA_DEBUG_SYNC");
    debug_sync_ = e != nullptr ? std::atoi(e) : 0;
    const char* at = std::getenv("ARENA_AUTOTUNE");
    autotune_ = at != nullptr ? std::atoi(at) : 1;
    const char* c = std::getenv("ARENA_COPY_MODE");
    copy_mode_ = c != nullptr && std::atoi(c) == 2 ? 2 : 0;
    const char* cc = std::getenv("ARENA_CONCURRENT");
    concurrent_ = cc != nullptr ? std::atoi(cc) : 1;
    if (debug_sync_) concurrent_ = 0;
    const char* ns = std::getenv("ARENA_SLOTS");
    n_slots_ = concurrent_ ? std::min(kMaxSlots, std::max(2, ns != nullptr ? std::atoi(ns) : 4)) : 2;
    const char* nc = std::getenv("ARENA_CONCURRENCY");
    n_streams_ = concurrent_ ? std::min(n_slots_, std::max(1, nc != nullptr ? std::atoi(nc) : 3)) : 1;
    const char* sg = std::getenv("ARENA_STAGGER");
    if (concurrent_ && n_streams_ > 1) {
      std::string spec = sg != nullptr ? sg : "0.25";
      for (size_t a = 0; a < spec.size();) {
        size_t e = spec.find(',', a);
        if (e == std::string::npos) e = spec.size();
        const double f = std::atof(spec.substr(a, e - a).c_str());
        if (f > 0.0 && f < 1.0 && (int)stagger_.size() < kMaxStaggerParts - 1) stagger_.push_back(f);
        a = e + 1;
      }
      std::sort(stagger_.begin(), stagger_.end());
    }
    const char* sm = std::getenv("ARENA_STAGGER_MIN_BATCH");
    stagger_min_batch_ = sm != nullptr ? std::max(1, std::atoi(sm)) : 32;
  }
  ARENA_HIP_CHECK(hipStreamCreateWithFlags(&compute_, hipStreamNonBlocking));
  ARENA_HIP_CHECK(hipStreamCreateWithFlags(&copy_, hipStreamNonBlocking));
  streams_[0] = compute_;
  for (int i = 1; i < n_streams_; ++i) ARENA_HIP_CHECK(hipStreamCreateWithFlags(&streams_[i], hipStreamNonBlocking));
  for (int s = 0; s < n_slots_; ++s) {
    slots_[s].idx = s;
    slots_[s].stream = streams_[s % n_streams_];
  }
  alloc_slots();
  const int nthreads = std::max(1, cfg_.host_threads);
  for (int t = 0; t < nthreads; ++t) {
    workers_.emplace_back([this]() {
      pthread_setname_np(pthread_self(), "arena-pack");
      uint64_t seen = 0;
      for (;;) {
        std::vector<std::function<void()>>* jobs;
        {
          std::unique_lock<std::mutex> lk(pool_mu_);
          pool_cv_.wait(lk, [&] { return pool_stop_ || pool_gen_ != seen; });
          if (pool_stop_) return;
          seen = pool_gen_;
          jobs = pool_jobs_;
          if (jobs == nullptr) continue;
          ++pool_active_;
        }
        for (;;) {
          const int i = pool_next_.fetch_add(1);
          if (i >= (int)jobs->size()) break;
          (*jobs)[i]();
        }
        std::lock_guard<std::mutex> lk(pool_mu_);
        if (--pool_active_ == 0) pool_done_cv_.notify_all();
      }
    });
  }
}

Executor::~Executor() {
  {
    std::lock_guard<std::mutex> lk(pool_mu_);
    pool_stop_ = true;
  }
  pool_cv_.notify_all();
  for (auto& t : workers_) t.join();
  hipSetDevice(cfg_.device);
  for (int i = 0; i < n_streams_; ++i)
    if (streams_[i]) hipStreamSynchronize(streams_[i]);
  if (copy_) hipStreamSynchronize(copy_);
  for (auto& kv : buckets_) {
    for (int s = 0; s < n_slots_; ++s) destroy_graphs(kv.second, s);
    free_arenas(kv.second);
  }
  for (int i = 1; i < n_streams_; ++i)
    if (streams_[i]) hipStreamDestroy(streams_[i]);
  for (int s = 0; s < n_slots_; ++s) {
    Slot& sl = slots_[s];
    if (sl.d_in) hipFree(sl.d_in);
    if (sl.d_out) hipFree(sl.d_out);
    if (sl.sk_ws) hipFree(sl.sk_ws);
    if (sl.h_in) hipHostFree(sl.h_in);
    if (sl.h_out) hipHostFree(sl.h_out);
  }
  for (uint8_t* p : retired_h_in_) hipHostFree(p);
  retired_h_in_.clear();
  for (int s = 0; s < n_slots_; ++s) {
    Slot& sl = slots_[s];
    if (sl.copied) hipEventDestroy(sl.copied);
    if (sl.started) hipEventDestroy(sl.started);
    if (sl.done) hipEventDestroy(sl.done);
    if (sl.fork_ev) hipEventDestroy(sl.fork_ev);
    for (hipEvent_t& e : sl.phase)
      if (e) hipEventDestroy(e);
    for (int l = 0; l < kMaxLanes; ++l) {
      if (sl.lane_ev[l]) hipEventDestroy(sl.lane_ev[l]);
      if (sl.lane_stream[l]) hipStreamDestroy(sl.lane_stream[l]);
    }
  }
  if (d_weights_) hipFree(d_weights_);
  if (compute_) hipStreamDestroy(compute_);
  if (copy_) hipStreamDestroy(copy_);
}

size_t Executor::jpeg_desc_off() const { return kCtrlBytes + align_up(sizeof(ImageMeta) * (size_t)max_B_, 256); }
size_t Executor::in_bytes_meta() const { return jpeg_desc_off() + align_up(sizeof(JpegDesc) * (size_t)max_B_, 256); }
size_t Executor::pool_cap() const {
  return align_up((size_t)cfg_.pool_bytes_per_image * (size_t)std::max(1, cfg_.pool_factor) * max_B_, 256);
}
size_t Executor::in_bytes_total() const { return in_bytes_meta() + pool_cap(); }
size_t Executor::out_off_det() const { return align_up(sizeof(int) * (size_t)max_B_, 256); }
size_t Executor::out_off_topk() const {
  return out_off_det() + align_up(sizeof(Detection) * (size_t)max_B_ * cfg_.max_det, 256);
}
size_t Executor::out_off_raw() const {
  return align_up(out_off_topk() + sizeof(TopkResult) * (size_t)max_B_ * cfg_.max_det, 256);
}
size_t Executor::out_off_xcrops() const { return align_up(out_off_raw() + (size_t)cfg_.raw_out_bytes * max_B_, 256); }
size_t Executor::out_off_stamps() const {
  return align_up(out_off_xcrops() + sizeof(CropRef) * (size_t)max_B_ * cfg_.max_det, 256);
}
size_t Executor::out_bytes_total() const { return out_off_stamps() + 4 * sizeof(uint64_t); }

void Executor::sync_slots() {
  for (int i = 0; i < n_streams_; ++i) ARENA_HIP_CHECK(hipStreamSynchronize(streams_[i]));
}

void Executor::free_arenas(Bucket& bk) {
  for (int s = 0; s < n_slots_; ++s) {
    if (bk.d_arena[s] == nullptr) continue;
    bool first = true;
    for (int t = 0; t < s; ++t) first &= bk.d_arena[t] != bk.d_arena[s];
    if (first) hipFree(bk.d_arena[s]);
  }
  for (int s = 0; s < kMaxSlots; ++s) bk.d_arena[s] = nullptr;
}

void Executor::alloc_slots() {
  for (int s = 0; s < n_slots_; ++s) {
    Slot& sl = slots_[s];
    ARENA_HIP_CHECK(hipMalloc(&sl.d_in, in_bytes_total() + 256));
    ARENA_HIP_CHECK(hipMalloc(&sl.d_out, out_bytes_total()));
    ARENA_HIP_CHECK(hipMalloc(&sl.sk_ws, (size_t)sk_lane_bytes() * (kMaxLanes + 1)));
    sl.h_cap = in_bytes_meta() + align_up((size_t)cfg_.pool_bytes_per_image * max_B_, 256);
    ARENA_HIP_CHECK(hipHostMalloc(&sl.h_in, sl.h_cap, hipHostMallocDefault));
    ARENA_HIP_CHECK(hipHostMalloc(&sl.h_out, out_bytes_total(), hipHostMallocDefault));
    ARENA_HIP_CHECK(hipMemset(sl.d_in, 0, in_bytes_total()));
    ARENA_HIP_CHECK(hipMemset(sl.d_out, 0, out_bytes_total()));
    std::memset(sl.h_in, 0, in_bytes_meta());
    ARENA_HIP_CHECK(hipEventCreateWithFlags(&sl.copied, hipEventDisableTiming));
    for (hipEvent_t& e : sl.phase) ARENA_HIP_CHECK(hipEventCreateWithFlags(&e, hipEventDisableTiming));
    ARENA_HIP_CHECK(hipEventCreate(&sl.started));
    static const bool blocking = [] {
      const char* e = std::getenv("ARENA_SYNC");
      return e != nullptr && std::string(e) == "blocking";
    }();
    ARENA_HIP_CHECK(hipEventCreateWithFlags(&sl.done, blocking ? hipEventBlockingSync : hipEventDefault));
  }
}

void Executor::ensure_lanes(Slot& sl) {
  if (sl.fork_ev != nullptr) return;
  bool lanes = false;
  for (const OpRecord& r : prog_) lanes |= r[kLaneField] > 0;
  if (!lanes) return;
  for (int l = 0; l < kMaxLanes; ++l) {
    ARENA_HIP_CHECK(hipStreamCreateWithFlags(&sl.lane_stream[l], hipStreamNonBlocking));
    ARENA_HIP_CHECK(hipEventCreateWithFlags(&sl.lane_ev[l], hipEventDisableTiming));
  }
  ARENA_HIP_CHECK(hipEventCreateWithFlags(&sl.fork_ev, hipEventDisableTiming));
}

void Executor::set_weights(const void* host, size_t bytes) {
  ARENA_HIP_CHECK(hipSetDevice(cfg_.device));
  if (d_weights_ != nullptr && bytes != weights_bytes_) {
    if (!buckets_.empty()) throw std::runtime_error("set_weights: size change after buckets were captured");
    ARENA_HIP_CHECK(hipFree(d_weights_));
    d_weights_ = nullptr;
  }
  if (d_weights_ == nullptr) ARENA_HIP_CHECK(hipMalloc(&d_weights_, bytes));
  sync_slots();
  ARENA_HIP_CHECK(hipMemcpy(d_weights_, host, bytes, hipMemcpyHostToDevice));
  weights_bytes_ = bytes;
}

void Executor::set_weights_device(const void* dev, size_t bytes) {
  ARENA_HIP_CHECK(hipSetDevice(cfg_.device));
  if (d_weights_ == nullptr || bytes != weights_bytes_)
    throw std::runtime_error("set_weights_device: only a same-size update of uploaded weights is supported");
  sync_slots();
  ARENA_HIP_CHECK(hipMemcpy(d_weights_, dev, bytes, hipMemcpyDeviceToDevice));
}

std::vector<uint8_t> Executor::weights_host() {
  std::vector<uint8_t> out(weights_bytes_);
  if (d_weights_ == nullptr || weights_bytes_ == 0) return out;
  ARENA_HIP_CHECK(hipSetDevice(cfg_.device));
  sync_slots();
  ARENA_HIP_CHECK(hipMemcpy(out.data(), d_weights_, weights_bytes_, hipMemcpyDeviceToHost));
  return out;
}

void Executor::set_program(const int64_t* ops, int n_ops, const int64_t* cls_ops, int n_cls_ops) {
  prog_.resize(n_ops);
  for (int i = 0; i < n_ops; ++i) std::memcpy(prog_[i].data(), ops + (size_t)i * kOpFields, sizeof(OpRecord));
  cls_prog_.resize(n_cls_ops);
  for (int i = 0; i < n_cls_ops; ++i)
    std::memcpy(cls_prog_[i].data(), cls_ops + (size_t)i * kOpFields, sizeof(OpRecord));
  has_topk_ = has_det_ = has_raw_ = has_stamps_ = false;
  for (const auto& r : prog_) {
    has_topk_ |= r[0] == OP_TOPK;
    has_stamps_ |= r[0] == OP_STAMP;
    has_det_ |= r[0] == OP_NMS || r[0] == OP_CROPPLAN;
    for (int f = 1; f < kOpFields; ++f) has_raw_ |= r[f] == BUF_RAWOUT && (r[0] == OP_YOLORAW || r[0] == OP_CONV);
  }
  if (has_raw_ && cfg_.raw_out_bytes <= 0) throw std::runtime_error("program exports raw outputs: raw_out_bytes = 0");
  gate_pairs_ = head_gate_pairs(prog_.empty() ? nullptr : prog_[0].data(), n_ops, kOpFields);
  gate_first_.clear();
  for (const HeadGatePair& gp : gate_pairs_)
    gate_first_.push_back(head_gate_first_conv(prog_[0].data(), n_ops, kOpFields, gp));
}

int Executor::crop_cap_for(int B) const { return std::max(cfg_.min_crop_cap, B * cfg_.crop_cap_per_image); }

std::vector<int> Executor::buckets() const {
  std::vector<int> r;
  for (auto& kv : buckets_) r.push_back(kv.first);
  return r;
}

uintptr_t Executor::arena_ptr(int B) const {
  auto it = buckets_.find(B);
  return it == buckets_.end() ? 0 : (uintptr_t)it->second.d_arena[0];
}

void Executor::read_arena(int B, int64_t offset, void* dst, size_t bytes) {
  auto it = buckets_.find(B);
  if (it == buckets_.end()) throw std::runtime_error("read_arena: unknown bucket");
  if (offset < 0 || offset + (int64_t)bytes > it->second.info.arena_bytes)
    throw std::runtime_error("read_arena: range outside the arena");
  ARENA_HIP_CHECK(hipSetDevice(cfg_.device));
  sync_slots();
  ARENA_HIP_CHECK(hipMemcpy(dst, it->second.d_arena[it->second.last_slot] + offset, bytes, hipMemcpyDeviceToHost));
}

void Executor::add_bucket(int B, const int64_t* offsets, int n_buffers, int64_t arena_bytes,
                          const std::vector<int>* impl) {
  if (B <= 0 || B > max_B_) throw std::runtime_error("add_bucket: B outside (0, max_batch]");
  if (prog_.empty()) throw std::runtime_error("add_bucket: set_program first");
  if (d_weights_ == nullptr) throw std::runtime_error("add_bucket: set_weights first");
  ARENA_HIP_CHECK(hipSetDevice(cfg_.device));
  Bucket& bk = buckets_[B];
  bk.info.B = B;
  bk.info.crop_cap = crop_cap_for(B);
  bk.info.offsets.assign(offsets, offsets + n_buffers);
  bk.info.arena_bytes = arena_bytes;
  sync_slots();
  free_arenas(bk);
  size_t abytes = align_up((size_t)std::max<int64_t>(arena_bytes, 256), 256);
  bk.marks_off.assign(gate_pairs_.size(), -1);
  for (size_t i = 0; i < gate_pairs_.size(); ++i) {
    if (gate_first_[i] < 0) continue;
    const OpRecord& f = prog_[gate_first_[i]];
    const OpRecord& c = prog_[gate_pairs_[i].cls];
    const int64_t cb = c[34] > 0 ? c[36] : c[10], cst = c[34] > 0 ? c[38] : c[12];
    if (f[1] < 0 || f[1] >= n_buffers || cb < 0 || cb >= n_buffers) continue;
    const int64_t in_lo = offsets[f[1]], in_hi = in_lo + (int64_t)B * f[4] * f[5] * f[3] * 4;
    const int64_t w_lo = offsets[cb], w_hi = w_lo + (int64_t)B * c[13] * c[14] * cst * 4;
    if (f[1] == cb || (in_lo < w_hi && w_lo < in_hi)) continue;
    bk.marks_off[i] = (int64_t)abytes;
    abytes += align_up((size_t)B * head_mark_cells((int)f[13]) * head_mark_cells((int)f[14]) * sizeof(int), 256);
  }
  for (int s = 0; s < n_slots_; ++s) {
    ARENA_HIP_CHECK(hipMalloc(&bk.d_arena[s], abytes));
    ARENA_HIP_CHECK(hipMemset(bk.d_arena[s], 0, abytes));
  }
  bk.impl.assign(prog_.size(), 0);
  if (impl != nullptr) {
    if (impl->size() != prog_.size()) throw std::runtime_error("add_bucket: tuning table does not match the program");
    for (size_t i = 0; i < prog_.size(); ++i) {
      const int v = (*impl)[i];
      const bool f32 = prog_[i][kDtypeField] == 1;
      const bool ok = f32 ? (v >= 0 && v <= 2) || (v >= 10 && v < 10 + kF32Variants) ||
                                (v >= kF32X3 && v < kF32X3 + kF32X3Variants) || v == kF32Halo || v == kF32X3Halo ||
                                v == kF32X3HaloN3 || v == kF32X3HaloN2 || v == kF32Stream || v == kF32StreamN2 ||
                                v == kF32Fc || v == kF32StreamExact || v == kF32X3Halo16 || v == kF32X3Halo16N3 ||
                                v == kF32X3H16 || (v >= kF32X3G && v < kF32X3G + kF32X3GVariants) ||
                                (v >= kF32X3HG && v < kF32X3HG + kF32X3HGVariants) ||
                                (v >= kF32X3HGPw && v < kF32X3HGPw + kF32X3HGPwVariants) ||
                                (v >= kF32X3HGPwSmall && v < kF32X3HGPwSmall + kF32X3HGPwSmallVariants) ||
                                (v >= kF32X3HR && v < kF32X3HR + kF32X3HRVariants) ||
                                (v >= kF32X3HRPw && v < kF32X3HRPw + kF32X3HRPwVariants) ||
                                (v >= kF32X3HP && v < kF32X3HP + kF32X3HPVariants) ||
                                (v >= kF32X3GSK && v < kF32X3GSK + kF32X3GSKVariants)
                          : v >= 0 && v <= 3;
      if (!ok || (v != 0 && prog_[i][0] != OP_CONV)) throw std::runtime_error("add_bucket: bad tuning entry");
      bk.impl[i] = (int16_t)v;
    }
  } else if (autotune_) {
    autotune(bk);
  }
  for (int s = 0; s < n_slots_; ++s) capture(bk, s);
  if (debug_sync_ || std::getenv("ARENA_DEBUG_ALLOC")) {
    fprintf(stderr, "[arena alloc] bucket %d arena %p..%p (%lld B)\n", B, (void*)bk.d_arena[0],
            (void*)(bk.d_arena[0] + arena_bytes), (long long)arena_bytes);
    for (int s = 0; s < n_slots_; ++s)
      fprintf(stderr, "[arena alloc] slot %d in %p..%p out %p..%p\n", s, (void*)slots_[s].d_in,
              (void*)(slots_[s].d_in + in_bytes_total()), (void*)slots_[s].d_out,
              (void*)(slots_[s].d_out + out_bytes_total()));
    fprintf(stderr, "[arena alloc] weights %p..%p\n", (void*)d_weights_, (void*)(d_weights_ + weights_bytes_));
  }
}

void Executor::autotune(Bucket& bk) {
  Slot& sl = slots_[0];
  Ctrl c{};
  c.n_images = bk.info.B;
  c.n_crops = bk.info.crop_cap;
  ARENA_HIP_CHECK(hipStreamSynchronize(compute_));
  ARENA_HIP_CHECK(hipMemcpy(sl.d_in, &c, sizeof(Ctrl), hipMemcpyHostToDevice));
  hipEvent_t e0, e1;
  ARENA_HIP_CHECK(hipEventCreate(&e0));
  ARENA_HIP_CHECK(hipEventCreate(&e1));
  static const int kF32Candidates[] = {0,      12,     13,     14,     17,     19,     20,         21,
                                       23,     24,     kF32Halo, kF32X3, kF32X3 + 1, kF32X3 + 4, kF32X3 + 5,
                                       kF32X3 + 6, kF32X3 + 7, kF32X3 + 8, kF32X3Halo, kF32X3HaloN3,
                                       kF32X3HaloN2, kF32Stream, kF32StreamN2, kF32Fc, kF32StreamExact,
                                       kF32X3Halo16, kF32X3Halo16N3, kF32X3H16,
                                       kF32X3G + 5, kF32X3G + 6, kF32X3G + 7, kF32X3G + 9, kF32X3G + 15,
                                       kF32X3G + 16, kF32X3G + 17, kF32X3G + 19,
                                       kF32X3HG + 0, kF32X3HG + 1, kF32X3HG + 2, kF32X3HG + 4, kF32X3HG + 6,
                                       kF32X3HG + 7, kF32X3HG + 8, kF32X3HG + 9, kF32X3HG + 10,
                                       kF32X3HGPw + 0, kF32X3HGPw + 1, kF32X3HGPw + 2, kF32X3HGPw + 3,
                                       kF32X3HGPw + 4, kF32X3HGPw + 5, kF32X3HGPwSmall + 0, kF32X3HGPwSmall + 1,
                                       kF32X3HR + 0, kF32X3HR + 1, kF32X3HR + 2, kF32X3HR + 3, kF32X3HR + 4,
                                       kF32X3HR + 5, kF32X3HR + 6, kF32X3HR + 7, kF32X3HR + 8, kF32X3HR + 9,
                                       kF32X3HRPw + 0, kF32X3HRPw + 1, kF32X3HRPw + 2, kF32X3HRPw + 3,
                                       kF32X3HRPw + 4, kF32X3HRPw + 5,
                                       kF32X3HP + 0, kF32X3HP + 1, kF32X3HP + 2, kF32X3HP + 3, kF32X3HP + 4,
                                       kF32X3HP + 5, kF32X3HP + 6, kF32X3HP + 7, kF32X3HP + 8,
                                       kF32X3GSK + 0, kF32X3GSK + 1, kF32X3GSK + 2, kF32X3GSK + 3, kF32X3GSK + 4,
                                       kF32X3GSK + 5, kF32X3GSK + 6, kF32X3GSK + 7, kF32X3GSK + 8};
  static const int kBf16Candidates[] = {1, 2, 3};
  for (size_t i = 0; i < prog_.size(); ++i) {
    if (prog_[i][0] != OP_CONV) continue;
    const bool f32 = prog_[i][kDtypeField] == 1;
    if (prog_[i][1] == BUF_POOL) {
      bk.impl[i] = kF32X3H16;
      continue;
    }
    if (!f32 && prog_[i][34] > 0) {
      bk.impl[i] = 2;
      continue;
    }
    const int reps = f32 ? 5 : 3;
    std::vector<OpRecord> one(1, prog_[i]);
    float best = 1e30f;
    int best_impl = -1;
    const int* cand = f32 ? kF32Candidates : kBf16Candidates;
    const int n_cand = f32 ? (int)(sizeof(kF32Candidates) / sizeof(int)) : 3;
    for (int ci = 0; ci < n_cand; ++ci) {
      const int impl = cand[ci];
      try {
        enqueue_program(one, bk, sl, compute_, (int)i, impl);
      } catch (const std::runtime_error&) {
        continue;
      }
      ARENA_HIP_CHECK(hipEventRecord(e0, compute_));
      for (int k = 0; k < reps; ++k) enqueue_program(one, bk, sl, compute_, (int)i, impl);
      ARENA_HIP_CHECK(hipEventRecord(e1, compute_));
      ARENA_HIP_CHECK(hipEventSynchronize(e1));
      float ms = 0.f;
      ARENA_HIP_CHECK(hipEventElapsedTime(&ms, e0, e1));
      if (best_impl < 0 || ms < best * 0.97f) {
        best = ms;
        best_impl = impl;
      }
    }
    bk.impl[i] = (int16_t)std::max(best_impl, 0);
    if (autotune_ > 1)
      fprintf(stderr, "[arena autotune] B=%d op %zu -> impl %d (%.1f us)\n", bk.info.B, i, best_impl,
              best * 1e3f / reps);
  }
  ARENA_HIP_CHECK(hipEventDestroy(e0));
  ARENA_HIP_CHECK(hipEventDestroy(e1));
  ARENA_HIP_CHECK(hipMemset(bk.d_arena[0], 0, std::max<int64_t>(bk.info.arena_bytes, 256)));
}

static int lanes_max_batch() {
  static const int v = [] {
    const char* e = std::getenv("ARENA_LANES_MAX_BATCH");
    return e != nullptr ? std::atoi(e) : 2;
  }();
  return v;
}

bool Executor::lanes_for(const Bucket& bk) const {
  if (bk.info.B > lanes_max_batch()) return false;
  for (const OpRecord& r : prog_)
    if (r[kLaneField] >= 1 && r[kLaneField] <= kMaxLanes) return true;
  return false;
}

int64_t Executor::sk_lane_bytes() {
  static const int64_t v = [] {
    const char* e = std::getenv("ARENA_SPLITK_WS_MB");
    return (int64_t)std::max(1, e != nullptr ? std::atoi(e) : 16) << 20;
  }();
  return v;
}

void Executor::destroy_graphs(Bucket& bk, int s) {
  if (bk.graph[s]) hipGraphExecDestroy(bk.graph[s]);
  bk.graph[s] = nullptr;
  for (hipGraphExec_t g : bk.parts[s])
    if (g) hipGraphExecDestroy(g);
  bk.parts[s].clear();
  for (auto& sg : bk.segs[s])
    if (sg.g) hipGraphExecDestroy(sg.g);
  bk.segs[s].clear();
}

void Executor::capture(Bucket& bk, int s) {
  Slot& sl = slots_[s];
  hipStream_t st = sl.stream;
  ARENA_HIP_CHECK(hipStreamSynchronize(st));
  destroy_graphs(bk, s);
  if (s == 0) {
    bk.exec_order.clear();
    bk.gated.clear();
    bk.launches.clear();
  }
  auto capture_range = [&](size_t a, size_t b) {
    std::vector<OpRecord> part(prog_.begin() + a, prog_.begin() + b);
    if (s == 0) {
      std::vector<const HeadGatePair*> gate;
      const std::vector<size_t> order = exec_plan(part, bk, (int)a, 0, gate);
      for (size_t k = 0; k < order.size(); ++k) {
        bk.exec_order.push_back((int)(a + order[k]));
        if (gate[k] != nullptr) bk.gated.push_back((int)(a + order[k]));
      }
      for (const Step& st : launch_plan(part, bk, (int)a, 0)) bk.launches.emplace_back((int)(a + st.pos), st.kind);
    }
    hipGraph_t g = nullptr;
    hipGraphExec_t ge = nullptr;
    ARENA_HIP_CHECK(hipStreamBeginCapture(st, hipStreamCaptureModeThreadLocal));
    try {
      enqueue_program(part, bk, sl, st, (int)a);
    } catch (...) {
      hipStreamEndCapture(st, &g);
      if (g) hipGraphDestroy(g);
      throw;
    }
    ARENA_HIP_CHECK(hipStreamEndCapture(st, &g));
    ARENA_HIP_CHECK(hipGraphInstantiate(&ge, g, nullptr, nullptr, 0));
    ARENA_HIP_CHECK(hipGraphDestroy(g));
    return ge;
  };
  if (!lanes_for(bk)) {
    std::vector<size_t> cuts{0};
    if (bk.info.B >= 16)
      for (double f : stagger_) {
        const size_t k = (size_t)std::lround(f * (double)prog_.size());
        if (k > cuts.back() && k < prog_.size()) cuts.push_back(k);
      }
    if (cuts.size() > 1) {
      cuts.push_back(prog_.size());
      for (size_t i = 0; i + 1 < cuts.size(); ++i) bk.parts[s].push_back(capture_range(cuts[i], cuts[i + 1]));
    } else {
      bk.graph[s] = capture_range(0, prog_.size());
    }
    return;
  }
  ensure_lanes(sl);
  auto lane_of = [&](size_t i) {
    const int64_t l = prog_[i][kLaneField];
    return l >= 1 && l <= kMaxLanes ? (int)l : 0;
  };
  for (size_t a = 0; a < prog_.size();) {
    size_t b = a + 1;
    while (b < prog_.size() && lane_of(b) == lane_of(a)) ++b;
    Bucket::Seg sg;
    sg.lane = lane_of(a);
    sg.g = capture_range(a, b);
    bk.segs[s].push_back(sg);
    a = b;
  }
}

void Executor::launch_graph(Bucket& bk, int s, hipStream_t st, int n_live) {
  if (bk.segs[s].empty()) {
    if (!bk.parts[s].empty()) {
      int others = 0;
      for (int k = 0; k < n_slots_; ++k) others += k != s && slots_[k].busy ? 1 : 0;
      const bool gate = n_live < 0 || (n_live >= std::min(stagger_min_batch_, bk.info.B) && others >= 2);
      const Slot* prev = gate && last_launched_ >= 0 && last_launched_ != s ? &slots_[last_launched_] : nullptr;
      const size_t np = bk.parts[s].size();
      for (size_t i = 0; i < np; ++i) {
        if (prev && i + 1 < np) ARENA_HIP_CHECK(hipStreamWaitEvent(st, prev->phase[i], 0));
        ARENA_HIP_CHECK(hipGraphLaunch(bk.parts[s][i], st));
        ARENA_HIP_CHECK(hipEventRecord(slots_[s].phase[i], st));
      }
      last_launched_ = s;
      return;
    }
    ARENA_HIP_CHECK(hipGraphLaunch(bk.graph[s], st));
    return;
  }
  Slot& sl = slots_[s];
  bool forked[kMaxLanes] = {};
  bool fork_recorded = false;
  auto join = [&]() {
    for (int l = 0; l < kMaxLanes; ++l)
      if (forked[l]) {
        ARENA_HIP_CHECK(hipEventRecord(sl.lane_ev[l], sl.lane_stream[l]));
        ARENA_HIP_CHECK(hipStreamWaitEvent(st, sl.lane_ev[l], 0));
        forked[l] = false;
      }
    fork_recorded = false;
  };
  for (const Bucket::Seg& sg : bk.segs[s]) {
    if (sg.lane == 0) {
      join();
      ARENA_HIP_CHECK(hipGraphLaunch(sg.g, st));
      continue;
    }
    const int l = sg.lane - 1;
    if (!forked[l]) {
      if (!fork_recorded) {
        ARENA_HIP_CHECK(hipEventRecord(sl.fork_ev, st));
        fork_recorded = true;
      }
      ARENA_HIP_CHECK(hipStreamWaitEvent(sl.lane_stream[l], sl.fork_ev, 0));
      forked[l] = true;
    }
    ARENA_HIP_CHECK(hipGraphLaunch(sg.g, sl.lane_stream[l]));
  }
  join();
}

uint8_t* Executor::resolve(Bucket& bk, Slot& sl, int64_t buf, int64_t coff, int eb) {
  uint8_t* base = nullptr;
  switch (buf) {
    case BUF_NONE: return nullptr;
    case BUF_CTRL: base = sl.d_in; break;
    case BUF_META: base = sl.d_in + kCtrlBytes; break;
    case BUF_POOL: base = sl.d_in + in_bytes_meta(); break;
    case BUF_DETCOUNT: base = sl.d_out; break;
    case BUF_DET: base = sl.d_out + out_off_det(); break;
    case BUF_TOPK: base = sl.d_out + out_off_topk(); break;
    case BUF_RAWOUT: base = sl.d_out + out_off_raw(); break;
    case BUF_XCROPS: base = sl.d_out + out_off_xcrops(); break;
    default:
      if (buf < 0 || buf >= (int64_t)bk.info.offsets.size())
        throw std::runtime_error("program references unknown buffer " + std::to_string(buf));
      base = bk.d_arena[sl.idx] + bk.info.offsets[buf];
  }
  return base + coff * eb;
}

std::vector<size_t> Executor::exec_plan(const std::vector<OpRecord>& prog, const Bucket& bk, int op_offset,
                                        int force_impl, std::vector<const HeadGatePair*>& gate) const {
  std::vector<size_t> order(prog.size());
  for (size_t k = 0; k < order.size(); ++k) order[k] = k;
  gate.assign(prog.size(), nullptr);
  if (!g_head_gate || force_impl != 0) return order;
  for (const HeadGatePair& gp : gate_pairs_) {
    const long li = (long)gp.box - op_offset;
    float gm;
    if (li < 0 || li + 1 >= (long)prog.size() || gp.cls >= (int)prog_.size()) continue;
    if (!head_gate_min(gp.conf_thr, &gm)) continue;
    if (prog[li] != prog_[gp.box] || prog[li + 1] != prog_[gp.cls]) continue;
    const int impl = gp.box < (int)bk.impl.size() ? bk.impl[gp.box] : 0;
    const bool x3hg_pw = impl == 0 || (impl >= kF32X3HGPw && impl < kF32X3HGPw + kF32X3HGPwVariants) ||
                         (impl >= kF32X3HGPwSmall && impl < kF32X3HGPwSmall + kF32X3HGPwSmallVariants);
    if (!x3hg_pw) continue;
    order[li] = (size_t)li + 1;
    order[li + 1] = (size_t)li;
    gate[li + 1] = &gp;
  }
  return order;
}

std::vector<Executor::Step> Executor::launch_plan(const std::vector<OpRecord>& prog, const Bucket& bk, int op_offset,
                                                  int force_impl) const {
  std::vector<const HeadGatePair*> gate;
  const std::vector<size_t> order = exec_plan(prog, bk, op_offset, force_impl, gate);
  std::vector<Step> steps;
  steps.reserve(order.size() + 6);
  for (size_t k = 0; k < order.size(); ++k) steps.push_back(Step{order[k], LAUNCH_OP, gate[k]});
  if (g_head_split == 0 || (g_head_split == 1 && bk.info.B < kHeadSplitMinBucket)) return steps;
  for (size_t i = 0; i < gate_pairs_.size(); ++i) {
    const HeadGatePair& gp = gate_pairs_[i];
    const int fi = gate_first_[i];
    const long lf = (long)fi - op_offset;
    if (fi < 0 || lf < 0 || i >= bk.marks_off.size() || bk.marks_off[i] < 0) continue;
    size_t k = 0;
    while (k < steps.size() && !(steps[k].kind == LAUNCH_OP && steps[k].gate == &gp)) ++k;
    if (k >= steps.size() || k < 2 || steps[k - 2].pos != (size_t)lf || steps[k - 2].kind != LAUNCH_OP) continue;
    if (prog[lf] != prog_[fi] || prog_[fi][30] != BATCH_IMAGES) continue;
    const int f_impl = fi < (int)bk.impl.size() ? bk.impl[fi] : 0;
    if (!(f_impl >= kF32X3HP && f_impl < kF32X3HP + kF32X3HPVariants)) continue;
    int uh = 0, uw = 0;
    if (gp.box >= (int)bk.impl.size() || !x3hg_pw_tile(bk.impl[gp.box], (int)prog_[gp.box][16], &uh, &uw)) continue;
    if (uh % kMarkCell != 0 || uw % kMarkCell != 0) continue;
    const size_t box_pos = steps[k].pos;
    steps[k - 2].kind = LAUNCH_CLS_WINDOW;
    steps[k - 2].gate = &gp;
    const Step extra[2] = {Step{box_pos, LAUNCH_MARK, &gp}, Step{(size_t)lf, LAUNCH_BOX_WINDOW, &gp}};
    steps.insert(steps.begin() + (long)k, extra, extra + 2);
  }
  return steps;
}

void Executor::enqueue_program(const std::vector<OpRecord>& prog, Bucket& bk, Slot& sl, hipStream_t s_main,
                               int op_offset, int force_impl) {
  Ctrl* ctrl = (Ctrl*)resolve(bk, sl, BUF_CTRL, 0, 1);
  const ImageMeta* meta = (const ImageMeta*)resolve(bk, sl, BUF_META, 0, 1);
  const uint8_t* pool = resolve(bk, sl, BUF_POOL, 0, 1);
  const int B = bk.info.B, CC = bk.info.crop_cap;
  auto batch = [&](int64_t kind) { return kind == BATCH_CROPS ? CC : B; };
  auto bdev = [&](int64_t kind) -> const int* { return kind == BATCH_CROPS ? &ctrl->n_crops : &ctrl->n_images; };
  const uint8_t* W = d_weights_;

  const std::vector<Step> steps = launch_plan(prog, bk, op_offset, force_impl);
  auto marks_of = [&](const HeadGatePair* gp) {
    return (int*)(bk.d_arena[sl.idx] + bk.marks_off[(size_t)(gp - gate_pairs_.data())]);
  };
  for (const Step& step : steps) {
    const size_t oi = step.pos;
    const OpRecord& r = prog[oi];
    hipStream_t s = s_main;
    if (step.kind == LAUNCH_MARK) {
      HeadMarkParams m{};
      m.n_levels = 1;
      m.logits[0] = (const float*)resolve(bk, sl, r[36], r[37] + kHeadBoxChannels, 4);
      m.H[0] = (int)r[13];
      m.W[0] = (int)r[14];
      m.ps[0] = (int)r[38];
      m.marks[0] = marks_of(step.gate);
      m.n = kHeadClsChannels;
      head_gate_min(step.gate->conf_thr, &m.gate_min);
      m.B = batch(r[30]);
      m.bdev = bdev(r[30]);
      head_mark(m, s);
      continue;
    }
    const bool f32 = r[kDtypeField] == 1;
    const int eb = f32 ? 4 : 2;
    switch (r[0]) {
      case OP_CONV: {
        ConvParams p{};
        const size_t gi = (size_t)op_offset + oi;
        p.impl = force_impl ? force_impl : (gi < bk.impl.size() ? bk.impl[gi] : 0);
        p.x = resolve(bk, sl, r[1], r[2], eb);
        p.xs = (int)r[3];
        p.H = (int)r[4];
        p.W = (int)r[5];
        p.Cin = (int)r[6];
        p.w = W + r[7];
        p.Kpad = (int)r[8];
        p.bias = (const float*)(W + r[9]);
        p.f32out = (int)r[29];
        p.y = resolve(bk, sl, r[10], r[11], p.f32out ? 4 : eb);
        p.ys = (int)r[12];
        p.Ho = (int)r[13];
        p.Wo = (int)r[14];
        p.Cout = (int)r[15];
        p.Cout_pad = (int)r[16];
        p.KH = (int)r[17];
        p.KW = (int)r[18];
        p.stride = (int)r[19];
        p.pad_t = (int)r[20];
        p.pad_l = (int)r[21];
        p.res = resolve(bk, sl, r[22], r[23], eb);
        p.rs = (int)r[24];
        p.y2 = resolve(bk, sl, r[25], r[26], eb);
        p.y2s = (int)r[27];
        p.act = (int)r[28];
        p.B = batch(r[30]);
        p.bdev = bdev(r[30]);
        if (r[41] != 0) p.w3 = W + r[40];
        {
          const int64_t ln = r[kLaneField];
          const int li = ln >= 1 && ln <= kMaxLanes ? (int)ln : 0;
          p.sk_ws = (float*)((uint8_t*)sl.sk_ws + (size_t)li * sk_lane_bytes());
          p.sk_ws_bytes = sk_lane_bytes();
        }
        if (r[1] == BUF_POOL) {
          if (!f32 || r[30] != 0) throw std::runtime_error("executor: letterbox-source conv must be fp32 over images");
          p.x = nullptr;
          p.lb_pool = pool;
          p.lb_meta = meta;
          p.impl = kF32X3H16;
        }
        if (r[34] > 0) {
          p.pw_w = W + r[31];
          p.pw_kpad = (int)r[32];
          p.pw_bias = (const float*)(W + r[33]);
          p.pw_cout = (int)r[34];
          p.pw_y = resolve(bk, sl, r[36], r[37], eb);
          p.pw_ys = (int)r[38];
          p.pw_act = (int)r[39];
          if (!f32) p.impl = 2;
          if (step.gate != nullptr) {
            p.gate = (const float*)resolve(bk, sl, r[36], r[37] + kHeadBoxChannels, eb);
            p.gate_n = kHeadClsChannels;
            head_gate_min(step.gate->conf_thr, &p.gate_min);
          }
        }
        if (step.kind == LAUNCH_CLS_WINDOW || step.kind == LAUNCH_BOX_WINDOW) {
          const bool box = step.kind == LAUNCH_BOX_WINDOW;
          p.n_lo = box ? 0 : kHeadBoxChannels;
          p.n_hi = box ? kHeadBoxChannels : kHeadBoxChannels + kHeadClsChannels;
          if (box) {
            p.marks = marks_of(step.gate);
            p.mark_halo = 1;
            x3hg_pw_tile(bk.impl[step.gate->box], (int)prog_[step.gate->box][16], &p.mark_uh, &p.mark_uw);
          }
          if (!conv_x3hp(p, s, box ? kHeadSplitBoxVariant : kHeadSplitClsVariant))
            throw std::runtime_error("executor: the split first head conv does not fit its x3hp window kernel");
          break;
        }
        if (f32)
          conv2d_f32(p, s);
        else
          conv2d(p, s);
        break;
      }
      case OP_DWCONV: {
        DwParams p{};
        p.x = resolve(bk, sl, r[1], r[2], eb);
        p.xs = (int)r[3];
        p.H = (int)r[4];
        p.W = (int)r[5];
        p.C = (int)r[6];
        p.w = W + r[7];
        p.bias = (const float*)(W + r[8]);
        p.y = resolve(bk, sl, r[9], r[10], eb);
        p.ys = (int)r[11];
        p.Ho = (int)r[12];
        p.Wo = (int)r[13];
        p.stride = (int)r[14];
        p.act = (int)r[15];
        p.B = batch(r[16]);
        p.bdev = bdev(r[16]);
        if (f32)
          dwconv3x3_f32(p, s);
        else
          dwconv3x3(p, s);
        break;
      }
      case OP_IRBLOCK: {
        IrParams p{};
        p.x = resolve(bk, sl, r[1], r[2], eb);
        p.x_cs = (int)r[3];
        p.H = (int)r[4];
        p.W = (int)r[5];
        p.inp = (int)r[6];
        p.inp_pad = (int)r[7];
        p.hid_pad = (int)r[8];
        p.oup = (int)r[9];
        p.oup_pad = (int)r[10];
        p.stride = (int)r[11];
        p.expand = (int)r[12];
        p.res = (int)r[13];
        p.we = W + r[14];
        p.be = (const float*)(W + r[15]);
        p.wd = W + r[16];
        p.bd = (const float*)(W + r[17]);
        p.wp = W + r[18];
        p.bp = (const float*)(W + r[19]);
        p.y = resolve(bk, sl, r[20], r[21], eb);
        p.y_cs = (int)r[22];
        p.Ho = (int)r[23];
        p.Wo = (int)r[24];
        p.B = batch(r[25]);
        p.bdev = bdev(r[25]);
        p.x3w = (int)r[26];
        p.x_parts = (int)r[27];
        p.y_parts = (int)r[28];
        if (!f32 && (p.x_parts > 1 || p.y_parts > 1))
          throw std::runtime_error("executor: partial-sum ir_block tensors are fp32-only");
        p.stem = (int)r[31];
        if (p.stem) {
          p.st_pool = pool;
          p.st_meta = meta;
          p.st_crops = (const CropRef*)resolve(bk, sl, r[32], 0, 1);
          p.st_ctrl = ctrl;
          p.st_S = (int)r[33];
          for (int c = 0; c < 3; ++c) {
            p.st_mean[c] = bits_to_float(r[34 + c]);
            p.st_inv_std[c] = bits_to_float(r[37 + c]);
          }
          p.st_w = (const float*)(W + r[40]);
          p.st_b = (const float*)(W + r[41]);
        }
        if (f32)
          ir_block_f32(p, s);
        else
          ir_block(p, s);
        break;
      }
      case OP_SPPF: {
        SppfParams p{};
        p.buf = resolve(bk, sl, r[1], r[2], eb);
        p.xs = (int)r[3];
        p.H = (int)r[4];
        p.W = (int)r[5];
        p.C = (int)r[6];
        p.B = batch(r[7]);
        p.bdev = bdev(r[7]);
        if (f32)
          sppf_pool_f32(p, s);
        else
          sppf_pool(p, s);
        break;
      }
      case OP_LETTERBOX: {
        LetterboxParams p{};
        p.pool = pool;
        p.meta = meta;
        p.ctrl = ctrl;
        p.out = resolve(bk, sl, r[1], 0, eb);
        p.B = B;
        p.T = (int)r[2];
        p.f32 = f32;
        letterbox_s2d(p, s);
        break;
      }
      case OP_STAMP: {
        if (r[1] < 0 || r[1] >= 4) throw std::runtime_error("OP_STAMP: stamp index out of range");
        stamp(sl.d_out + out_off_stamps() + sizeof(uint64_t) * (size_t)r[1], s);
        break;
      }
      case OP_ZERO: {
        uint8_t* ptr = resolve(bk, sl, r[1], 0, 1);
        const size_t bytes = (size_t)r[2] * batch(r[3]);
        zero_fill(ptr, bytes, s);
        break;
      }
      case OP_DECODE: {
        DecodeParams p{};
        for (int l = 0; l < 3; ++l) {
          p.head[l] = resolve(bk, sl, r[1 + 4 * l], r[2 + 4 * l], eb);
          p.xs[l] = (int)r[3 + 4 * l];
          p.hw[l] = (int)r[4 + 4 * l];
          p.stride[l] = (float)r[13 + l];
        }
        p.cand = (Candidate*)resolve(bk, sl, r[16], 0, 1);
        p.cand_count = (int*)resolve(bk, sl, r[17], 0, 1);
        p.conf_thr = bits_to_float(r[18]);
        p.cand_cap = cfg_.cand_cap;
        p.B = B;
        p.ctrl = ctrl;
        p.f32 = f32;
        detect_decode(p, s);
        break;
      }
      case OP_NMS: {
        NmsParams p{};
        p.cand = (const Candidate*)resolve(bk, sl, r[1], 0, 1);
        p.cand_count = (const int*)resolve(bk, sl, r[2], 0, 1);
        p.cand_cap = cfg_.cand_cap;
        p.meta = meta;
        p.B = B;
        p.det = (Detection*)resolve(bk, sl, r[3], 0, 1);
        p.det_count = (int*)resolve(bk, sl, r[4], 0, 1);
        p.max_det = cfg_.max_det;
        p.iou_thr = bits_to_float(r[5]);
        p.ctrl = ctrl;
        nms(p, s);
        break;
      }
      case OP_CROPPLAN: {
        CropPlanParams p{};
        p.det = (Detection*)resolve(bk, sl, r[1], 0, 1);
        p.det_count = (int*)resolve(bk, sl, r[2], 0, 1);
        p.max_det = cfg_.max_det;
        p.meta = meta;
        p.B = B;
        p.crops = (CropRef*)resolve(bk, sl, r[3], 0, 1);
        p.ctrl = ctrl;
        p.crop_cap = CC;
        p.whole = (int)r[4];
        crop_plan(p, s);
        break;
      }
      case OP_CROPGATHER: {
        CropGatherParams p{};
        p.pool = pool;
        p.meta = meta;
        p.crops = (const CropRef*)resolve(bk, sl, r[1], 0, 1);
        p.ctrl = ctrl;
        p.out = resolve(bk, sl, r[2], 0, eb);
        p.f32 = f32;
        p.cap = CC;
        p.S = (int)r[3];
        for (int c = 0; c < 3; ++c) {
          p.mean[c] = bits_to_float(r[4 + c]);
          p.inv_std[c] = bits_to_float(r[7 + c]);
        }
        crop_gather_s2d(p, s);
        break;
      }
      case OP_C3FUSED: {
        C3Params p{};
        p.x = resolve(bk, sl, r[1], r[2], eb);
        p.xs = (int)r[3];
        p.H = (int)r[4];
        p.W = (int)r[5];
        p.C1 = (int)r[6];
        p.CH = (int)r[7];
        p.NB = (int)r[8];
        p.res = (int)r[9];
        p.w12 = W + r[10];
        p.b12 = (const float*)(W + r[11]);
        for (int k = 0; k < 2; ++k) {
          p.wb1[k] = W + r[12 + 4 * k];
          p.bb1[k] = (const float*)(W + r[13 + 4 * k]);
          p.wb2[k] = W + r[14 + 4 * k];
          p.bb2[k] = (const float*)(W + r[15 + 4 * k]);
        }
        p.w3 = W + r[20];
        p.b3 = (const float*)(W + r[21]);
        p.y = resolve(bk, sl, r[22], r[23], eb);
        p.ys = (int)r[24];
        p.B = batch(r[25]);
        p.bdev = bdev(r[25]);
        if (f32)
          c3_x3(p, s);
        else
          c3_fused(p, s);
        break;
      }
      case OP_STEMFUSED: {
        StemFusedParams p{};
        p.src = (int)r[1];
        p.y = resolve(bk, sl, r[2], r[3], eb);
        p.ys = (int)r[4];
        p.S = (int)r[5];
        p.w = W + r[6];
        p.Kpad = (int)r[7];
        p.bias = (const float*)(W + r[8]);
        p.Cout = (int)r[9];
        p.act = (int)r[10];
        p.crops = p.src == 1 ? (const CropRef*)resolve(bk, sl, r[11], 0, 1) : nullptr;
        for (int c = 0; c < 3; ++c) {
          p.mean[c] = bits_to_float(r[12 + c]);
          p.inv_std[c] = bits_to_float(r[15 + c]);
        }
        p.cap = batch(r[18]);
        p.KS = (int)r[19];
        if (r[20]) {
          p.w2 = W + r[21];
          p.Kpad2 = (int)r[22];
          p.bias2 = (const float*)(W + r[23]);
          p.Cout2 = (int)r[24];
          p.act2 = (int)r[25];
          p.y2 = p.y;
          p.y2s = p.ys;
          p.y = nullptr;
        }
        if (r[26]) {
          p.ir_wd = W + r[27];
          p.ir_bd = (const float*)(W + r[28]);
          p.ir_wp = W + r[29];
          p.ir_bp = (const float*)(W + r[30]);
          p.ir_y = p.y;
          p.ir_ys = p.ys;
          p.y = nullptr;
        }
        p.pool = pool;
        p.meta = meta;
        p.ctrl = ctrl;
        if (f32)
          stem_s2_f32(p, s);
        else
          stem_fused(p, s);
        break;
      }
      case OP_HEADPOOL: {
        HeadPoolParams p{};
        p.x = resolve(bk, sl, r[1], r[2], eb);
        p.xs = (int)r[3];
// ... 638 lines not shown
```

### csrc/runtime/executor.h

```cpp
#pragma once
#include <chrono>
#include <hip/hip_runtime.h>

#include <array>
#include <atomic>
#include <condition_variable>
#include <cstdint>
#include <functional>
#include <map>
#include <mutex>
#include <thread>
#include <vector>

#include "../kernels/launch.h"
#include "head_gate.h"
#include "head_marks.h"
#include "instance.h"

namespace arena {

constexpr int kOpFields = 48;
constexpr int kDtypeField = 47;
constexpr int kLaneField = 46;
constexpr int kMaxLanes = 3;
constexpr int kMaxSlots = 6;
constexpr int kMaxStaggerParts = 5;
constexpr int kMaxEstBuckets = 257;
using OpRecord = std::array<int64_t, kOpFields>;

void set_head_gate(bool v);
bool get_head_gate();
void set_head_split(int v);
int get_head_split();
constexpr int kHeadSplitMinBucket = 32;
constexpr int kHeadSplitBoxVariant = 2, kHeadSplitClsVariant = 9;
enum LaunchKind : int { LAUNCH_OP = 0, LAUNCH_CLS_WINDOW = 1, LAUNCH_BOX_WINDOW = 2, LAUNCH_MARK = 3 };

enum OpType : int64_t {
  OP_CONV = 1,
  OP_DWCONV = 2,
  OP_SPPF = 3,
  OP_LETTERBOX = 4,
  OP_ZERO = 5,
  OP_DECODE = 6,
  OP_NMS = 7,
  OP_CROPPLAN = 8,
  OP_CROPGATHER = 9,
  OP_AVGPOOL = 10,
  OP_TOPK = 11,
  OP_TENSORIN = 12,
  OP_YOLORAW = 13,
  OP_IRBLOCK = 14,
  OP_STEMFUSED = 15,
  OP_C3FUSED = 16,
  OP_HEADPOOL = 17,
  OP_STAMP = 18,
};

enum ReservedBuf : int64_t {
  BUF_NONE = -1,
  BUF_CTRL = -10,
  BUF_META = -11,
  BUF_POOL = -12,
  BUF_DET = -13,
  BUF_DETCOUNT = -14,
  BUF_TOPK = -15,
  BUF_RAWOUT = -16,
  BUF_XCROPS = -17,
};

enum BatchKind : int64_t { BATCH_IMAGES = 0, BATCH_CROPS = 1 };

struct ExecutorConfig {
  int device = 0;
  int max_batch = 32;
  int max_det = 300;
  int cand_cap = 8400;
  int crop_cap_per_image = 6;
  int min_crop_cap = 16;
  int64_t pool_bytes_per_image = 640LL * 640 * 3;
  int pool_factor = 3;
  int det_size = 640;
  int cls_size = 224;
  int host_threads = 8;
  int64_t raw_out_bytes = 0;
};

struct BucketInfo {
  int B = 0;
  int crop_cap = 0;
  std::vector<int64_t> offsets;
  int64_t arena_bytes = 0;
};

class Executor : public BatchInstance {
 public:
  explicit Executor(const ExecutorConfig& cfg);
  ~Executor() override;
  Executor(const Executor&) = delete;
  Executor& operator=(const Executor&) = delete;

  void set_weights(const void* host, size_t bytes);
  void set_weights_device(const void* dev, size_t bytes);
  std::vector<uint8_t> weights_host();
  void set_program(const int64_t* ops, int n_ops, const int64_t* cls_ops, int n_cls_ops);
  void add_bucket(int B, const int64_t* offsets, int n_buffers, int64_t arena_bytes,
                  const std::vector<int>* impl = nullptr);
  std::vector<int> buckets() const override;
  int crop_cap_for(int B) const;
  const ExecutorConfig& config() const { return cfg_; }
  int max_det() const override { return cfg_.max_det; }
  int64_t raw_out_bytes() const override { return cfg_.raw_out_bytes; }
  int64_t staging_bytes() const override { return (int64_t)pool_cap(); }

  int submit(const std::vector<InputImage>& imgs) override;
  BatchResult collect(int slot) override;
  int ready(int slot) override;
  double remaining_us(int slot) override;
  BatchResult run(const std::vector<InputImage>& imgs);

  int submit_peer(Executor& src, int src_slot);
  struct DeviceImage {
    uintptr_t ptr = 0;
    int h = 0, w = 0;
    int device = -1;
  };
  int submit_device(const std::vector<DeviceImage>& imgs, const std::vector<std::vector<Detection>>& dets);
  void set_peer_stage(bool v) { peer_stage_ = v; }
  bool peer_stage() const { return peer_stage_; }
  int device() const { return cfg_.device; }

  void replay(int B, int slot, int iters);
  void synchronize();
  int num_slots() const override { return n_slots_; }

  uintptr_t arena_ptr(int B) const;
  void read_arena(int B, int64_t offset, void* dst, size_t bytes);
  uintptr_t weights_ptr() const { return (uintptr_t)d_weights_; }
  uintptr_t stream() const { return (uintptr_t)compute_; }

 private:
  std::vector<uint8_t*> retired_h_in_;
  int64_t staging_growths_ = 0;

 public:
  int64_t staging_growths() const { return staging_growths_; }

 private:
  struct Slot {
    uint8_t* d_in = nullptr;
    uint8_t* d_out = nullptr;
    float* sk_ws = nullptr;
    uint8_t* h_in = nullptr;
    size_t h_cap = 0;
    uint8_t* h_out = nullptr;
    hipEvent_t copied = nullptr, started = nullptr, done = nullptr;
    hipEvent_t phase[kMaxStaggerParts] = {};
    hipStream_t stream = nullptr;
    hipStream_t lane_stream[kMaxLanes] = {};
    hipEvent_t fork_ev = nullptr, lane_ev[kMaxLanes] = {};
    int idx = 0;
    std::chrono::steady_clock::time_point t_submit{};
    bool polled = false;
    std::chrono::steady_clock::time_point t_poll{};
    bool busy = false;
    int bucket = 0;
    int n_images = 0;
    size_t in_used = 0;
  };
  struct Bucket {
    BucketInfo info;
    uint8_t* d_arena[kMaxSlots] = {};
    int last_slot = 0;
    hipGraphExec_t graph[kMaxSlots] = {};
    std::vector<hipGraphExec_t> parts[kMaxSlots];
    struct Seg {
      int lane = 0;
      hipGraphExec_t g = nullptr;
    };
    std::vector<Seg> segs[kMaxSlots];
    std::vector<int16_t> impl;
    std::vector<int> exec_order, gated;
    std::vector<std::pair<int, int>> launches;
    std::vector<int64_t> marks_off;
  };
  struct Step {
    size_t pos;
    int kind;
    const HeadGatePair* gate;
  };

  void alloc_slots();
  void ensure_lanes(Slot& sl);
  void sync_slots();
  void free_arenas(Bucket& bk);
  void capture(Bucket& bk, int slot);
  void wait_done(Slot& sl);
  void note_done(Slot& sl);
  void release_copy(Slot& sl);
  static int64_t sk_lane_bytes();
  uint64_t copy_release_n_ = 0;
  void launch_graph(Bucket& bk, int slot, hipStream_t st, int n_live = -1);
  void destroy_graphs(Bucket& bk, int slot);
  bool lanes_for(const Bucket& bk) const;
  void enqueue_program(const std::vector<OpRecord>& prog, Bucket& bk, Slot& sl, hipStream_t s,
                       int op_offset = 0, int force_impl = 0);
  void autotune(Bucket& bk);
  std::vector<size_t> exec_plan(const std::vector<OpRecord>& prog, const Bucket& bk, int op_offset, int force_impl,
                                std::vector<const HeadGatePair*>& gate) const;
  std::vector<Step> launch_plan(const std::vector<OpRecord>& prog, const Bucket& bk, int op_offset,
                                int force_impl) const;

 public:
  std::vector<int> exec_order(int B) const {
    auto it = buckets_.find(B);
    return it == buckets_.end() ? std::vector<int>{} : it->second.exec_order;
  }
  std::vector<int> gated_ops(int B) const {
    auto it = buckets_.find(B);
    return it == buckets_.end() ? std::vector<int>{} : it->second.gated;
  }
  std::vector<std::pair<int, int>> launch_order(int B) const {
    auto it = buckets_.find(B);
    return it == buckets_.end() ? std::vector<std::pair<int, int>>{} : it->second.launches;
  }
  std::vector<int> conv_choices(int B) const {
    auto it = buckets_.find(B);
    if (it == buckets_.end()) return {};
    return std::vector<int>(it->second.impl.begin(), it->second.impl.end());
  }

 private:
  void enqueue_results_d2h(Bucket& bk, Slot& sl, int n);
  uint8_t* resolve(Bucket& bk, Slot& sl, int64_t buf, int64_t coff_elems, int elem_bytes);
  int pick_bucket(int n) const;
  size_t in_bytes_meta() const;
  size_t jpeg_desc_off() const;
  size_t pool_cap() const;
  size_t in_bytes_total() const;
  size_t out_off_det() const;
  size_t out_off_topk() const;
  size_t out_bytes_total() const;
  size_t out_off_raw() const;
  size_t out_off_xcrops() const;
  size_t out_off_stamps() const;
  int acquire_slot();
  void parallel_copy(std::vector<std::function<void()>>& jobs);

  ExecutorConfig cfg_;
  int max_B_ = 0;
  hipStream_t compute_ = nullptr, copy_ = nullptr;
  uint8_t* d_weights_ = nullptr;
  size_t weights_bytes_ = 0;
  std::vector<OpRecord> prog_, cls_prog_;
  std::vector<HeadGatePair> gate_pairs_;
  std::vector<int> gate_first_;
  std::map<int, Bucket> buckets_;
  Slot slots_[kMaxSlots];
  int n_slots_ = 2;
  int next_slot_ = 0;
  hipStream_t streams_[kMaxSlots] = {};
  int n_streams_ = 1;
  uint64_t seq_ = 0;
  std::vector<double> stagger_;
  int stagger_min_batch_ = 32;
  int last_launched_ = -1;
  bool has_topk_ = false, has_det_ = false, has_raw_ = false, has_stamps_ = false;
  double wall_khz_ = 100000.0;
  bool peer_stage_ = false;
  std::vector<int> peer_enabled_;
  void enable_peer(int src, const char* what);
  int copy_mode_ = 0;
  int concurrent_ = 1;
  int autotune_ = 1;
  int debug_sync_ = 0;
  std::mutex mu_;
  std::vector<std::thread> workers_;
  std::mutex pool_mu_;
  std::condition_variable pool_cv_, pool_done_cv_;
  std::vector<std::function<void()>>* pool_jobs_ = nullptr;
  std::atomic<int> pool_next_{0};
  std::atomic<float> wall_est_us_[kMaxEstBuckets] = {};
  int pool_active_ = 0;
  uint64_t pool_gen_ = 0;
  bool pool_stop_ = false;
};

}
```

### inference_arena_amd/ops/functional.py

```python
from __future__ import annotations

import ctypes
import struct

import numpy as np
import torch

from ..engine.planner import ACT, pack_conv_weight, pack_conv_weight_x3
from . import native

IMAGE_META = struct.Struct("<qiiiiiif12x")


def _stream() -> int:
    return torch.cuda.current_stream().cuda_stream


def _ptr(t: torch.Tensor | None, elem_off: int = 0) -> int:
    if t is None:
        return 0
    return t.data_ptr() + elem_off * t.element_size()


def pack_weights(w: torch.Tensor, b: torch.Tensor, device, dtype: str = "bf16"):
    wb, bb, kpad, cpad = pack_conv_weight(w.detach().cpu().float(), b.detach().cpu().float(), dtype)
    wt = torch.frombuffer(bytearray(wb), dtype=torch.float32 if dtype == "fp32" else torch.bfloat16).to(device)
    bt = torch.frombuffer(bytearray(bb), dtype=torch.float32).to(device)
    w3 = None
    if dtype == "fp32":
        w3 = torch.frombuffer(bytearray(pack_conv_weight_x3(w.detach().cpu().float())), dtype=torch.int16).to(device)
    return wt, bt, kpad, cpad, w3


def conv2d_nhwc(x: torch.Tensor, w: torch.Tensor, b: torch.Tensor, *, stride: int = 1, pad=None, act=None,
                x_coff: int = 0, cin: int | None = None, out: torch.Tensor | None = None, out_coff: int = 0,
                res: torch.Tensor | None = None, res_coff: int = 0, out2: torch.Tensor | None = None,
                out2_coff: int = 0, f32out: bool = False, out_hw=None, bdev: torch.Tensor | None = None,
                packed=None, impl: int = 0, pw=None, pw_out: torch.Tensor | None = None, pw_out_coff: int = 0,
                gate=None, window=None, marks=None) -> torch.Tensor:
    f32 = x.dtype == torch.float32
    B, H, W, Cx = x.shape
    cout, cin_w, kh, kw = w.shape
    cin = cin or cin_w
    if pad is None:
        pad = (kh // 2, kw // 2)
    if isinstance(pad, int):
        pad = (pad, pad)
    if out_hw is None:
        Ho = (H + 2 * pad[0] - kh) // stride + 1
        Wo = (W + 2 * pad[1] - kw) // stride + 1
    else:
        Ho, Wo = out_hw
    if out is None:
        out = torch.empty(B, Ho, Wo, cout, dtype=torch.float32 if (f32out or f32) else torch.bfloat16, device=x.device)
    wt, bt, kpad, cpad, w3 = packed if packed is not None else pack_weights(w, b, x.device, "fp32" if f32 else "bf16")
    pwd = {}
    if pw is not None:
        from ..engine.planner import pack_pw_weight_x3

        if not f32:
            raise ValueError("conv2d_nhwc: the functional fused pointwise path is fp32-only")
        w2, b2 = pw
        co2 = w2.shape[0]
        k2 = (cout + 31) // 32 * 32
        w2p = torch.frombuffer(bytearray(pack_pw_weight_x3(w2.detach().cpu().float(), k2)),
                               dtype=torch.int16).to(x.device)
        b2p = torch.zeros((co2 + 15) // 16 * 16)
        b2p[:co2] = b2.detach().float()
        b2p = b2p.to(x.device)
        if pw_out is None:
            out = torch.empty(B, Ho, Wo, co2, dtype=torch.float32, device=x.device)
            pw_out_coff = 0
        else:
            out = pw_out
            if (out.shape[:3] != (B, Ho, Wo) or out.shape[3] < pw_out_coff + co2 or out.dtype != torch.float32
                    or out.device != x.device or not out.is_contiguous()):
                raise ValueError(f"conv2d_nhwc: pw_out {tuple(out.shape)} {out.dtype} does not fit the 1x1 output")
        pwd = {"pw_w": _ptr(w2p), "pw_bias": _ptr(b2p), "pw_y": _ptr(out, pw_out_coff), "pw_ys": out.shape[-1],
               "pw_cout": co2, "pw_kpad": k2, "pw_act": 0}
        if gate is not None:
            gt, gcoff, gn, gmin = gate
            if (gt.shape != out.shape or gt.dtype != torch.float32 or gt.device != x.device or not gt.is_contiguous()
                    or gcoff < 0 or gn <= 0 or gcoff + gn > gt.shape[3]):
                raise ValueError("conv2d_nhwc: the gate logits must match the 1x1 output tensor's shape and stride")
            pwd.update({"gate": _ptr(gt, gcoff), "gate_n": int(gn), "gate_min": float(gmin)})
    elif gate is not None or pw_out is not None:
        raise ValueError("conv2d_nhwc: gate / pw_out need pw")
    if window is not None:
        pwd.update({"n_lo": int(window[0]), "n_hi": int(window[1])})
    if marks is not None:
        mt, uh, uw, halo = marks
        if (mt.dtype != torch.int32 or mt.device != x.device or not mt.is_contiguous()
                or tuple(mt.shape) != (B, (Ho + 7) // 8, (Wo + 7) // 8)):
            raise ValueError("conv2d_nhwc: marks must be contiguous int32 [B, ceil(Ho / 8), ceil(Wo / 8)]")
        pwd.update({"marks": _ptr(mt), "mark_uh": int(uh), "mark_uw": int(uw), "mark_halo": int(halo)})
    skd = {}
    if 171 <= int(impl) < 180:
        ws = torch.empty(8 * B * Ho * Wo * cpad, dtype=torch.float32, device=x.device)
        skd = {"sk_ws": _ptr(ws), "sk_ws_bytes": ws.numel() * 4}
    native().conv2d({
        "x": _ptr(x, x_coff), "B": B, "H": H, "W": W, "xs": Cx, "Cin": cin,
        "w": _ptr(wt), "Kpad": kpad, "bias": _ptr(bt),
        "y": _ptr(out, out_coff), "Ho": Ho, "Wo": Wo, "ys": out.shape[-1], "Cout": cout, "Cout_pad": cpad,
        "KH": kh, "KW": kw, "stride": stride, "pad_t": pad[0], "pad_l": pad[1],
        "res": _ptr(res, res_coff), "rs": res.shape[-1] if res is not None else 0,
        "y2": _ptr(out2, out2_coff), "y2s": out2.shape[-1] if out2 is not None else 0,
        "act": ACT[act], "f32out": int(f32out), "bdev": _ptr(bdev), "stream": _stream(), "f32": int(f32),
        "impl": int(impl), "w3": _ptr(w3), **pwd, **skd,
    })
    if pw is not None:
        torch.cuda.synchronize(x.device)
    return out


def head_mark(logits: torch.Tensor, coff: int, n: int, gate_min: float, marks: torch.Tensor | None = None,
              bdev: torch.Tensor | None = None, levels=None) -> torch.Tensor | list:
    lv = [(logits, marks)] + list(levels or [])
    out = []
    for lg, mk in lv:
        B, H, W, C = lg.shape
        if lg.dtype != torch.float32 or not lg.is_contiguous() or coff < 0 or coff + n > C:
            raise ValueError("head_mark: logits must be contiguous float32 [B, H, W, >= coff + n]")
        if mk is None:
            mk = torch.zeros(B, (H + 7) // 8, (W + 7) // 8, dtype=torch.int32, device=lg.device)
        if (mk.dtype != torch.int32 or mk.device != lg.device or not mk.is_contiguous()
                or tuple(mk.shape) != (B, (H + 7) // 8, (W + 7) // 8) or B != lv[0][0].shape[0]):
            raise ValueError("head_mark: marks must be contiguous int32 [B, ceil(H / 8), ceil(W / 8)]")
        out.append(mk)
    native().head_mark({"logits": [_ptr(lg, coff) for lg, _ in lv], "marks": [_ptr(mk) for mk in out],
                        "H": [lg.shape[1] for lg, _ in lv], "W": [lg.shape[2] for lg, _ in lv],
                        "ps": [lg.shape[3] for lg, _ in lv], "n": int(n), "gate_min": float(gate_min),
                        "B": lv[0][0].shape[0], "bdev": _ptr(bdev), "stream": _stream()})
    return out if levels else out[0]


def dwconv3x3_nhwc(x: torch.Tensor, w: torch.Tensor, b: torch.Tensor, *, stride: int = 1, act="relu6",
                   bdev: torch.Tensor | None = None) -> torch.Tensor:
    B, H, W, C = x.shape
    f32 = x.dtype == torch.float32
    Ho, Wo = (H - 1) // stride + 1, (W - 1) // stride + 1
    y = torch.empty(B, Ho, Wo, C, dtype=x.dtype, device=x.device)
    wt = w.detach().float().reshape(C, 9).t().contiguous().to(x.dtype).to(x.device)
    bt = b.detach().float().contiguous().to(x.device)
    native().dwconv3x3({"x": _ptr(x), "B": B, "H": H, "W": W, "xs": C, "C": C, "w": _ptr(wt), "bias": _ptr(bt),
                        "y": _ptr(y), "Ho": Ho, "Wo": Wo, "ys": C, "stride": stride, "act": ACT[act],
                        "bdev": _ptr(bdev), "stream": _stream(), "f32": int(f32)})
    return y


def ir_block_nhwc(x: torch.Tensor, expand, dw, project, *, stride: int, res: bool = False,
                  bdev: torch.Tensor | None = None, x_parts: int = 1, y_parts: int = 1,
                  out: torch.Tensor | None = None) -> torch.Tensor:
    from ..engine.planner import ir_x3_plan, pack_ir_weights, split_bf16x3

    B, H, W, Ct = x.shape
    C = Ct // x_parts
    f32 = x.dtype == torch.float32
    pk = pack_ir_weights(expand, dw, project, C, k_align=16 if f32 else 32)
    x3w = 0
    if f32:
        x3w, inp_x3 = ir_x3_plan(H, W, stride, C, pk["hid_pad"], pk["oup_pad"], int(expand is not None))
        if x3w and inp_x3 != pk["inp_pad"]:
            pk = pack_ir_weights(expand, dw, project, C, k_align=32)
    Ho, Wo = (H - 1) // stride + 1, (W - 1) // stride + 1
    y = out if out is not None else torch.empty(B, Ho, Wo, pk["oup"] * y_parts, dtype=x.dtype, device=x.device)
    if (y.shape[:3] != (B, Ho, Wo) or y.shape[3] < pk["oup"] * y_parts or y.dtype != x.dtype or y.device != x.device
            or not y.is_contiguous()):
        raise ValueError(f"ir_block_nhwc: out {tuple(y.shape)} {y.dtype} does not fit the block's output")
    mat = torch.float32 if f32 else torch.bfloat16
    dev = {k: (pk[k].to(mat) if k in ("we", "wd", "wp") else pk[k].float()).contiguous().to(x.device)
           for k in ("we", "be", "wd", "bd", "wp", "bp")}
    if x3w:
        dev["we"] = split_bf16x3(pk["we"]).to(x.device)
        dev["wp"] = split_bf16x3(pk["wp"]).to(x.device)
    native().ir_block({"x": _ptr(x), "x_cs": Ct, "H": H, "W": W, "inp": C, "inp_pad": pk["inp_pad"],
                       "hid_pad": pk["hid_pad"], "oup": pk["oup"], "oup_pad": pk["oup_pad"], "stride": stride,
                       "expand": int(expand is not None), "res": int(res),
                       **{k: _ptr(v) for k, v in dev.items()}, "y": _ptr(y), "y_cs": y.shape[3], "Ho": Ho,
                       "Wo": Wo, "B": B, "bdev": _ptr(bdev), "stream": _stream(), "f32": int(f32), "x3w": x3w,
                       "x_parts": x_parts, "y_parts": y_parts})
    torch.cuda.synchronize(x.device)
    return y


def c3_x3_nhwc(x: torch.Tensor, cv12, bottleneck, cv3) -> torch.Tensor:
    from ..engine.planner import split_bf16x3

    B, H, W, C = x.shape
    (w1, b1), (w2, b2) = bottleneck
    w2k = torch.zeros(16, 160)
    w2k[:, :144] = w2.detach().float().permute(0, 2, 3, 1).reshape(16, 144)
    dev = {"w12": split_bf16x3(cv12[0].reshape(32, 32)), "b12": cv12[1].float(),
           "wb1": split_bf16x3(w1.reshape(16, 16)), "bb1": b1.float(), "wb2": split_bf16x3(w2k), "bb2": b2.float(),
           "w3": split_bf16x3(cv3[0].reshape(32, 32)), "b3": cv3[1].float()}
    dev = {k: v.contiguous().to(x.device) for k, v in dev.items()}
    y = torch.empty(B, H, W, 32, dtype=torch.float32, device=x.device)
    native().c3_block({"x": _ptr(x), "xs": C, "B": B, "H": H, "W": W, "bdev": 0, "C1": 32, "CH": 16, "NB": 1,
                       "res": 1, **{k: _ptr(v) for k, v in dev.items()}, "y": _ptr(y), "ys": 32,
                       "stream": _stream(), "f32": 1})
    torch.cuda.synchronize(x.device)
    return y


def sppf_nhwc(buf: torch.Tensor, C: int) -> torch.Tensor:
    B, H, W, Ct = buf.shape
    native().sppf_pool({"buf": _ptr(buf), "B": B, "H": H, "W": W, "xs": Ct, "C": C, "stream": _stream(),
                        "f32": int(buf.dtype == torch.float32)})
    return buf


def image_meta_bytes(images: list[np.ndarray], T: int) -> tuple[bytes, np.ndarray]:
    from ..processing.transforms import letterbox_geometry

    metas, chunks, off = [], [], 0
    for im in images:
        h, w = im.shape[:2]
        scale, nw, nh, pw, ph = letterbox_geometry(h, w, T)
        metas.append(IMAGE_META.pack(off, h, w, nw, nh, pw, ph, scale))
        data = np.ascontiguousarray(im, np.uint8).tobytes()
        pad = (-len(data)) % 256
        chunks.append(data + b"\0" * pad)
        off += len(data) + pad
    return b"".join(metas), np.frombuffer(b"".join(chunks), dtype=np.uint8)


def ctrl_tensor(n_images: int, device, n_crops: int = 0, crop_base: int = 0) -> torch.Tensor:
    c = torch.zeros(16, dtype=torch.int32)
    c[0], c[1], c[2] = n_images, n_crops, crop_base
    return c.to(device)


def letterbox_s2d(images: list[np.ndarray], T: int, device, dtype=torch.bfloat16) -> torch.Tensor:
    meta, pool = image_meta_bytes(images, T)
    meta_t = torch.frombuffer(bytearray(meta), dtype=torch.uint8).to(device)
    pool_t = torch.from_numpy(pool.copy()).to(device)
    ctrl = ctrl_tensor(len(images), device)
    out = torch.empty(len(images), T // 2, T // 2, 16, dtype=dtype, device=device)
    native().letterbox_s2d({"pool": _ptr(pool_t), "meta": _ptr(meta_t), "ctrl": _ptr(ctrl), "out": _ptr(out),
                            "B": len(images), "T": T, "stream": _stream(), "f32": int(dtype == torch.float32)})
    torch.cuda.current_stream().synchronize()
    return out


def s2d_to_nchw(x: torch.Tensor) -> torch.Tensor:
    B, h, w, _ = x.shape
    y = x[..., :12].float().reshape(B, h, w, 2, 2, 3)
    return y.permute(0, 5, 1, 3, 2, 4).reshape(B, 3, 2 * h, 2 * w)


def avgpool_nhwc(x: torch.Tensor) -> torch.Tensor:
    B, H, W, C = x.shape
    y = torch.empty(B, C, dtype=x.dtype, device=x.device)
    native().global_avgpool({"x": _ptr(x), "B": B, "HW": H * W, "C": C, "y": _ptr(y), "stream": _stream(),
                             "f32": int(x.dtype == torch.float32)})
    return y


def head_pool_nhwc(x: torch.Tensor, w: torch.Tensor, b: torch.Tensor, act: str | None = "relu6",
                   bdev: torch.Tensor | None = None) -> torch.Tensor:
    from ..engine.planner import ACT, pack_conv_weight

    B, H, W, C = x.shape
    N = w.shape[0]
    f32 = x.dtype == torch.float32
    wb, bb, kpad, npad = pack_conv_weight(w, b, "fp32" if f32 else "bf16")
    wd = torch.frombuffer(bytearray(wb), dtype=torch.float32 if f32 else torch.bfloat16).to(x.device)
    bd = torch.frombuffer(bytearray(bb), dtype=torch.float32).to(x.device)
    y = torch.empty(B, N, dtype=x.dtype, device=x.device)
    native().head_pool({"x": _ptr(x), "xs": C, "HW": H * W, "K": C, "w": _ptr(wd), "Kpad": kpad, "bias": _ptr(bd),
                        "N": N, "Npad": npad, "y": _ptr(y), "ys": N, "act": ACT[act], "B": B, "bdev": _ptr(bdev),
                        "stream": _stream(), "f32": int(f32)})
    torch.cuda.synchronize(x.device)
    return y


def topk_softmax(logits: torch.Tensor):
    B, N = logits.shape
    out = torch.empty(B, 16, dtype=torch.int32, device=logits.device)
    native().topk_softmax({"logits": _ptr(logits), "B": B, "N": N, "ld": logits.stride(0), "out": _ptr(out),
                           "stream": _stream()})
    torch.cuda.current_stream().synchronize()
    o = out.cpu()
    return o[:, 0:5].clone(), o[:, 5:10].view(torch.float32).clone(), o[:, 10:15].view(torch.float32).clone()
```

### inference_arena_amd/utils/settings.py

```python
from __future__ import annotations

import functools
import os
from pathlib import Path

from pydantic import BaseModel


def _read_dotenv(path: Path) -> dict[str, str]:
    out: dict[str, str] = {}
    if not path.exists():
        return out
    for line in path.read_text(encoding="utf-8").splitlines():
        line = line.strip()
        if not line or line.startswith("#") or "=" not in line:
            continue
        k, v = line.split("=", 1)
        v = v.strip()
        if v[:1] in ("'", '"') and v[0] in v[1:]:
            v = v[1:v.index(v[0], 1)]
        else:
            v = v.split(" #", 1)[0].split("\t#", 1)[0].strip()
        out[k.strip()] = v
    return out


class Settings(BaseModel):
    LOG_LEVEL: str = "INFO"
    PORT: int = 8100
    HOST: str = "0.0.0.0"
    MODELS_DIR: str = "model_repository"
    LABELS_FILE: str = ""
    CLASSIFICATION_GRPC_ENDPOINT: str = "127.0.0.1:8201"
    TRITON_GRPC_ENDPOINT: str = "127.0.0.1:8001"
    TRITON_HTTP_ENDPOINT: str = "127.0.0.1:8000"
    TRITON_TIMEOUT_SECONDS: float = 60.0
    ARENA_DEVICE: str = "gpu"
    ARENA_GPU: int = 0
    ARENA_GPUS: str = ""
    ARENA_CLS_GPU: int = -1
    ARENA_MAX_BATCH: int = 32
    ARENA_QUEUE_DELAY_US: int = 500
    ARENA_DECODE_THREADS: int = 8
    ARENA_CONFIDENCE: str = ""
    ARENA_CROP_TRANSPORT: str = "jpeg"
    ARENA_DEVICE_RING_SLOTS: int = 512
    ARENA_CROP_ENCODE: str = "pil"
    ARENA_FANOUT: str = "parallel"
    ARENA_GATEWAY_MODE: str = "pipeline"
    ARENA_INSTANCES: int = 1
    ARENA_WEIGHT_SEED: int = 0
    ARENA_FAULT_EVERY: int = 0
    ARENA_INFER_SERVICE: int = 0
    ARENA_IR_S2K16: int = 1
    ARENA_HEAD_GATE: int = 1
    ARENA_HEAD_SPLIT: int = 1

    @classmethod
    def from_env(cls, env_file: str | Path = ".env", **overrides) -> "Settings":
        vals: dict[str, str] = _read_dotenv(Path(env_file))
        for k in cls.model_fields:
            if k in os.environ:
                vals[k] = os.environ[k]
        vals.update({k: v for k, v in overrides.items() if v is not None})
        return cls(**vals)


@functools.lru_cache
def get_settings() -> Settings:
    return Settings.from_env()
```

Before: 11350.

## Fuse nearest-upsample into 1x1 x3g conv by reading the producer's half-resolution map

Adds an up-read path for YOLO neck convs that consume [up2(P) | skip]. For input channels below the upsampled count, the x3g 1x1 conv kernel now reads the producer's half-resolution output directly through a second buffer source. The producer then skips writing the upsampled copy (y2), saving that write and its reread. A static pass finds eligible producer/consumer pairs and checks per bucket that no intervening launch overwrites the producer's arena range. The path is on by default for buckets of 16 or more, and it adds a per-chunk source select plus new kernel instantiations.

After: 11440 (median of 6 runs). About the same (+0.7%).

```diff
diff --git a/csrc/bindings.cpp b/csrc/bindings.cpp
--- a/csrc/bindings.cpp
+++ b/csrc/bindings.cpp
@@ -96,6 +96,11 @@
   p.w3 = ptr<const void*>(d, "w3");
   p.sk_ws = ptr<float*>(d, "sk_ws");
   p.sk_ws_bytes = get<int64_t>(d, "sk_ws_bytes", 0);
+  p.x2 = ptr<const void*>(d, "x2");
+  p.x2s = get<int>(d, "x2s", 0);
+  p.x2_c = get<int>(d, "x2_c", 0);
+  p.x2_H = get<int>(d, "x2_H", 0);
+  p.x2_W = get<int>(d, "x2_W", 0);
   prepare_kernels();
   if (get<int>(d, "f32", 0))
     conv2d_f32(p, stream_of(d));
@@ -647,6 +652,32 @@
         return out;
       },
       py::arg("ops"), "[(box conv op, class conv op, level)] of a program's records");
+  m.def("set_up_read", &set_up_read);
+  m.def("get_up_read", &get_up_read);
+  m.attr("UP_READ_MIN_BUCKET") = kUpReadMinBucket;
+  m.def(
+      "up_read_pairs",
+      [](py::array_t<int64_t, py::array::c_style> ops) {
+        if (ops.ndim() != 2 || ops.shape(1) != kOpFields) throw std::runtime_error("ops must be int64 [n, OP_FIELDS]");
+        py::list out;
+        for (const UpReadPair& pr : up_read_pairs(ops.data(), (int)ops.shape(0), kOpFields))
+          out.append(py::make_tuple(pr.producer, pr.consumer));
+        return out;
+      },
+      py::arg("ops"), "[(producer op, consumer op)] of a program's records: convs over [up2(P) | skip] that may read P");
+  m.def(
+      "up_read_ranges_clear",
+      [](py::array_t<int64_t, py::array::c_style> ops, int producer, int consumer,
+         py::array_t<int64_t, py::array::c_style | py::array::forcecast> offsets, int B) {
+        if (ops.ndim() != 2 || ops.shape(1) != kOpFields) throw std::runtime_error("ops must be int64 [n, OP_FIELDS]");
+        if (offsets.ndim() != 1 || producer < 0 || consumer <= producer || consumer >= ops.shape(0))
+          throw std::runtime_error("up_read_ranges_clear: offsets must be 1-d, 0 <= producer < consumer < n");
+        return up_read_ranges_clear(ops.data(), kOpFields, UpReadPair{producer, consumer}, offsets.data(),
+                                    (int)offsets.shape(0), B);
+      },
+      py::arg("ops"), py::arg("producer"), py::arg("consumer"), py::arg("offsets"), py::arg("B"),
+      "nothing launched after the producer up to and including the consumer writes arena memory of the producer's "
+      "output (offsets: arena byte offset per buffer id of a bucket of B images)");
   m.def("set_head_split", &set_head_split);
   m.def("get_head_split", &get_head_split);
   m.attr("HEAD_SPLIT_MIN_BUCKET") = kHeadSplitMinBucket;
@@ -866,6 +897,8 @@
       .def("exec_order", &Executor::exec_order, py::arg("B"),
            "program op indices in the order bucket B's graphs launch them")
       .def("gated_ops", &Executor::gated_ops, py::arg("B"), "ops of bucket B that run with a tile gate")
+      .def("up_read_fused", &Executor::up_read_fused, py::arg("B"),
+           "the (producer op, consumer op) pairs bucket B's graphs run with the upsample read-through")
       .def("launch_order", &Executor::launch_order, py::arg("B"),
            "every kernel launch of bucket B's graphs in order as (op, kind): 0 the whole op, 1 / 2 the class / "
            "box window of a split first head conv, 3 the cell marks launched before op's box conv")
diff --git a/csrc/kernels/conv_f32.hip b/csrc/kernels/conv_f32.hip
--- a/csrc/kernels/conv_f32.hip
+++ b/csrc/kernels/conv_f32.hip
@@ -1415,6 +1415,9 @@
   if ((p.n_lo != 0 || p.n_hi != 0 || p.marks != nullptr) &&
       !(p.pw_w == nullptr && p.impl >= kF32X3HP && p.impl < kF32X3HP + kF32X3HPVariants))
     throw std::runtime_error("conv2d_f32: an output-channel window or a mark gate needs an x3hp variant");
+  if (p.x2 != nullptr && !(p.pw_w == nullptr && p.impl >= kF32X3G && p.impl < kF32X3G + kF32X3GVariants &&
+                           x3g_x2_supported(p)))
+    throw std::runtime_error("conv2d_f32: a second source needs an x3g variant on a 1x1 conv over twice its map");
   if (p.pw_w != nullptr) {
     if (p.impl >= kF32X3HRPw && p.impl < kF32X3HRPw + kF32X3HRPwVariants) {
       if (!conv_x3hr_pw(p, s, p.impl - kF32X3HRPw))
diff --git a/csrc/kernels/gemm_x3.hip b/csrc/kernels/gemm_x3.hip
--- a/csrc/kernels/gemm_x3.hip
+++ b/csrc/kernels/gemm_x3.hip
@@ -55,8 +55,9 @@
 
 }
 
-template <int WM, int WN, int TM, int TN, bool IL = false, bool SK = false>
+template <int WM, int WN, int TM, int TN, bool IL = false, bool SK = false, bool X2 = false>
 __global__ __launch_bounds__(WM * WN * 64) void conv_x3g_kernel(const ConvParams p) {
+  static_assert(!(SK && X2), "the second source is for the unsplit kernels");
   constexpr int NT = WM * WN * 64;
   static_assert(WM * WN == 4 || WM * WN == 8, "four or eight waves");
   constexpr int BM = WM * TM * 32, BN = WN * TN * 32;
@@ -92,6 +93,7 @@
   constexpr int kOob = 0x7fffffff & ~15;
 
   int a_iy[AI], a_ix[AI], a_off[AI];
+  int a_off2[X2 ? AI : 1];
 #pragma unroll
   for (int j = 0; j < AI; ++j) {
     const int i = tid + NT * j;
@@ -102,10 +104,12 @@
       a_iy[j] = oy * S - p.pad_t;
       a_ix[j] = ox * S - p.pad_l;
       a_off[j] = (((b * H + a_iy[j]) * W + a_ix[j]) * p.xs + 8 * (i & 3)) * 4;
+      if constexpr (X2) a_off2[j] = (((b * p.x2_H + (oy >> 1)) * p.x2_W + (ox >> 1)) * p.x2s + 8 * (i & 3)) * 4;
     } else {
       a_iy[j] = -0x40000000;
       a_ix[j] = 0;
       a_off[j] = 0;
+      if constexpr (X2) a_off2[j] = 0;
     }
   }
   int w_off[WI];
@@ -136,15 +140,33 @@
     ld_kx = wrap2 ? 0 : ld_kx;
     ld_ky += wrap2 ? 1 : 0;
     const int step = ((ky * W + kx) * p.xs + c0) * 4;
-#pragma unroll
-    for (int j = 0; j < AI; ++j) {
-      const int i = tid + NT * j;
-      const int c = c0 + 8 * (i & 3);
-      const bool in = (unsigned)(a_iy[j] + ky) < (unsigned)H && (unsigned)(a_ix[j] + kx) < (unsigned)W;
-      const int o0 = in && c < Cin ? a_off[j] + step : kOob;
-      const int o1 = in && c + 4 < Cin ? a_off[j] + step + 16 : kOob;
-      ra[j][0] = __builtin_bit_cast(f32x4, __builtin_amdgcn_raw_buffer_load_b128(xr, o0, 0, 0));
-      ra[j][1] = __builtin_bit_cast(f32x4, __builtin_amdgcn_raw_buffer_load_b128(xr, o1, 0, 0));
+    if constexpr (X2) {
+      const bool u2 = c0 < p.x2_c;
+      const __amdgpu_buffer_rsrc_t sr = __builtin_amdgcn_make_buffer_rsrc(
+          const_cast<void*>(u2 ? p.x2 : p.x), (short)0,
+          u2 ? (int)((size_t)p.B * p.x2_H * p.x2_W * p.x2s * 4) : (int)((size_t)p.B * H * W * p.xs * 4), 0x00020000);
+#pragma unroll
+      for (int j = 0; j < AI; ++j) {
+        const int i = tid + NT * j;
+        const int c = c0 + 8 * (i & 3);
+        const bool in = a_iy[j] >= 0;
+        const int base = (u2 ? a_off2[j] : a_off[j]) + c0 * 4;
+        const int o0 = in && c < Cin ? base : kOob;
+        const int o1 = in && c + 4 < Cin ? base + 16 : kOob;
+        ra[j][0] = __builtin_bit_cast(f32x4, __builtin_amdgcn_raw_buffer_load_b128(sr, o0, 0, 0));
+        ra[j][1] = __builtin_bit_cast(f32x4, __builtin_amdgcn_raw_buffer_load_b128(sr, o1, 0, 0));
+      }
+    } else {
+#pragma unroll
+      for (int j = 0; j < AI; ++j) {
+        const int i = tid + NT * j;
+        const int c = c0 + 8 * (i & 3);
+        const bool in = (unsigned)(a_iy[j] + ky) < (unsigned)H && (unsigned)(a_ix[j] + kx) < (unsigned)W;
+        const int o0 = in && c < Cin ? a_off[j] + step : kOob;
+        const int o1 = in && c + 4 < Cin ? a_off[j] + step + 16 : kOob;
+        ra[j][0] = __builtin_bit_cast(f32x4, __builtin_amdgcn_raw_buffer_load_b128(xr, o0, 0, 0));
+        ra[j][1] = __builtin_bit_cast(f32x4, __builtin_amdgcn_raw_buffer_load_b128(xr, o1, 0, 0));
+      }
     }
     const int wstep = kc * p.Cout_pad * 192;
 #pragma unroll
@@ -341,8 +363,12 @@
   constexpr int BM = WM * TM * 32, BN = WN * TN * 32;
   const long M = (long)p.B * p.Ho * p.Wo;
   const long tiles = ((M + BM - 1) / BM) * ((p.Cout_pad + BN - 1) / BN);
-  hipLaunchKernelGGL((conv_x3g_kernel<WM, WN, TM, TN, IL>), dim3((unsigned)tiles), dim3(WM * WN * 64), xg_lds_bytes(BM, BN), s,
-                     p);
+  if (p.x2 != nullptr)
+    hipLaunchKernelGGL((conv_x3g_kernel<WM, WN, TM, TN, IL, false, true>), dim3((unsigned)tiles), dim3(WM * WN * 64),
+                       xg_lds_bytes(BM, BN), s, p);
+  else
+    hipLaunchKernelGGL((conv_x3g_kernel<WM, WN, TM, TN, IL>), dim3((unsigned)tiles), dim3(WM * WN * 64), xg_lds_bytes(BM, BN), s,
+                       p);
 }
 
 template <int WM, int WN, int TM, int TN>
@@ -398,8 +424,17 @@
          p.pw_w == nullptr;
 }
 
+bool x3g_x2_supported(const ConvParams& p) {
+  const size_t x2_bytes = (size_t)p.B * p.x2_H * p.x2_W * p.x2s * 4;
+  return p.x2 != nullptr && p.KH == 1 && p.KW == 1 && p.stride == 1 && p.pad_t == 0 && p.pad_l == 0 &&
+         p.Ho == p.H && p.Wo == p.W && p.x2_H > 0 && p.x2_W > 0 && p.H == 2 * p.x2_H && p.W == 2 * p.x2_W &&
+         p.x2_c > 0 && p.x2_c % 32 == 0 && p.x2_c <= p.Cin && p.x2s % 4 == 0 && p.x2s >= p.x2_c &&
+         x2_bytes < (1u << 31) - (1u << 20);
+}
+
 bool conv_x3g(const ConvParams& p, hipStream_t s, int v) {
   if (!x3g_supported(p)) return false;
+  if (p.x2 != nullptr && !x3g_x2_supported(p)) return false;
   switch (v) {
 #define XG_CASE(V, WM, WN, TM, TN) \
   case V: xg_launch<WM, WN, TM, TN, false>(p, s); return true; \
@@ -411,7 +446,7 @@
 }
 
 bool conv_x3g_sk(const ConvParams& p, hipStream_t s, int v) {
-  if (!x3g_supported(p) || p.Cout % 4) return false;
+  if (!x3g_supported(p) || p.Cout % 4 || p.x2 != nullptr) return false;
   switch (v) {
 #define XG_SK_CASE(V, WM, WN, TM, TN, S)                                   \
   case V:                                                                  \
@@ -429,6 +464,12 @@
                                       hipFuncAttributeMaxDynamicSharedMemorySize,                         \
                                       xg_lds_bytes(WM * TM * 32, WN * TN * 32)));                         \
   ARENA_HIP_CHECK(hipFuncSetAttribute((const void*)conv_x3g_kernel<WM, WN, TM, TN, true>,                 \
+                                      hipFuncAttributeMaxDynamicSharedMemorySize,                         \
+                                      xg_lds_bytes(WM * TM * 32, WN * TN * 32)));                         \
+  ARENA_HIP_CHECK(hipFuncSetAttribute((const void*)conv_x3g_kernel<WM, WN, TM, TN, false, false, true>,   \
+                                      hipFuncAttributeMaxDynamicSharedMemorySize,                         \
+                                      xg_lds_bytes(WM * TM * 32, WN * TN * 32)));                         \
+  ARENA_HIP_CHECK(hipFuncSetAttribute((const void*)conv_x3g_kernel<WM, WN, TM, TN, true, false, true>,    \
                                       hipFuncAttributeMaxDynamicSharedMemorySize,                         \
                                       xg_lds_bytes(WM * TM * 32, WN * TN * 32)));
   XG_VARIANTS(XG_ATTR)
diff --git a/csrc/kernels/launch.h b/csrc/kernels/launch.h
--- a/csrc/kernels/launch.h
+++ b/csrc/kernels/launch.h
@@ -46,6 +46,8 @@
   float* sk_ws;
   int64_t sk_ws_bytes;
   int sk_splits;
+  const void* x2;
+  int x2s, x2_c, x2_H, x2_W;
 };
 void conv2d(const ConvParams& p, hipStream_t s);
 void conv_igemm(const ConvParams& p, hipStream_t s);
@@ -75,6 +77,7 @@
 constexpr int kF32X3GVariants = 20;
 void x3_halo_prepare();
 bool x3g_supported(const ConvParams& p);
+bool x3g_x2_supported(const ConvParams& p);
 bool conv_x3g(const ConvParams& p, hipStream_t s, int v);
 constexpr int kF32X3GSK = 171;
 constexpr int kF32X3GSKVariants = 9;
diff --git a/csrc/runtime/chain_fuse.h b/csrc/runtime/chain_fuse.h
--- /dev/null
+++ b/csrc/runtime/chain_fuse.h
@@ -0,0 +1,81 @@
+#pragma once
+#include <cstdint>
+#include <vector>
+
+namespace arena {
+
+constexpr int64_t kCfOpConv = 1, kCfOpDecode = 6, kCfOpYoloRaw = 13;
+constexpr int kCfDtypeField = 47;
+constexpr int kCfChunk = 32;
+
+struct UpReadPair {
+  int producer;
+  int consumer;
+};
+
+inline bool chain_reads(const int64_t* r, int64_t buf, int64_t c_lo, int64_t c_hi) {
+  if (r[0] == kCfOpConv) {
+    if (r[1] == buf && r[2] < c_hi && c_lo < r[2] + r[6]) return true;
+    return r[22] == buf && r[23] < c_hi && c_lo < r[23] + r[15];
+  }
+  if (r[1] == buf) return true;
+  if (r[0] == kCfOpDecode || r[0] == kCfOpYoloRaw) return r[5] == buf || r[9] == buf;
+  return false;
+}
+
+inline bool chain_conv_writes(const int64_t* r, int64_t buf, int64_t c_lo, int64_t c_hi) {
+  if (r[34] == 0 && r[10] == buf && r[11] < c_hi && c_lo < r[11] + r[15]) return true;
+  if (r[25] == buf && r[26] < c_hi && c_lo < r[26] + r[15]) return true;
+  return r[34] > 0 && r[36] == buf && r[37] < c_hi && c_lo < r[37] + r[34];
+}
+
+inline std::vector<UpReadPair> up_read_pairs(const int64_t* ops, int n, int fields) {
+  std::vector<UpReadPair> out;
+  if (ops == nullptr || fields <= kCfDtypeField) return out;
+  auto rec = [&](int i) { return ops + (size_t)i * fields; };
+  for (int pi = 0; pi < n; ++pi) {
+    const int64_t* p = rec(pi);
+    if (p[0] != kCfOpConv || p[kCfDtypeField] != 1 || p[25] < 0 || p[10] < 0 || p[34] != 0 || p[30] != 0) continue;
+    const int64_t buf = p[25], lo = p[26], hi = p[26] + p[15], cs = p[27];
+    if (p[15] <= 0 || p[15] % kCfChunk != 0) continue;
+    int ci = -1;
+    for (int i = pi + 1; i < n && ci < 0; ++i)
+      if (chain_reads(rec(i), buf, lo, hi)) ci = i;
+    if (ci < 0) continue;
+    const int64_t* c = rec(ci);
+    if (!(c[0] == kCfOpConv && c[kCfDtypeField] == 1 && c[34] == 0 && c[30] == 0)) continue;
+    if (!(c[17] == 1 && c[18] == 1 && c[19] == 1 && c[20] == 0 && c[21] == 0)) continue;
+    if (!(c[1] == buf && c[2] == lo && c[3] == cs && c[6] >= p[15] && c[4] == 2 * p[13] && c[5] == 2 * p[14])) continue;
+    if (c[22] == buf && c[23] < hi && lo < c[23] + c[15]) continue;
+    bool ok = true;
+    for (int i = pi + 1; i < ci && ok; ++i) ok = rec(i)[0] == kCfOpConv && !chain_conv_writes(rec(i), buf, lo, hi);
+    for (int i = 0; i < n && ok; ++i)
+      if (i != ci && i != pi && chain_reads(rec(i), buf, lo, hi)) ok = false;
+    if (ok) out.push_back(UpReadPair{pi, ci});
+  }
+  return out;
+}
+
+inline bool up_read_ranges_clear(const int64_t* ops, int fields, const UpReadPair& pr, const int64_t* offsets,
+                                 int n_buffers, int B) {
+  auto rec = [&](int i) { return ops + (size_t)i * fields; };
+  const int64_t* p = rec(pr.producer);
+  if (offsets == nullptr || p[10] < 0 || p[10] >= n_buffers || B <= 0) return false;
+  const int64_t lo = offsets[p[10]], hi = lo + (int64_t)B * p[13] * p[14] * p[12] * 4;
+  for (int i = pr.producer + 1; i <= pr.consumer; ++i) {
+    const int64_t* r = rec(i);
+    if (r[0] != kCfOpConv) return false;
+    const int64_t w[3][2] = {{r[34] == 0 ? r[10] : -1, r[13] * r[14] * r[12]},
+                             {r[25], 4 * r[13] * r[14] * r[27]},
+                             {r[34] > 0 ? r[36] : -1, r[13] * r[14] * r[38]}};
+    for (const auto& t : w) {
+      if (t[0] < 0) continue;
+      if (t[0] >= n_buffers || t[0] == p[10]) return false;
+      const int64_t w_lo = offsets[t[0]], w_hi = w_lo + (int64_t)B * t[1] * 4;
+      if (w_lo < hi && lo < w_hi) return false;
+    }
+  }
+  return true;
+}
+
+}
diff --git a/csrc/runtime/executor.cpp b/csrc/runtime/executor.cpp
--- a/csrc/runtime/executor.cpp
+++ b/csrc/runtime/executor.cpp
@@ -33,6 +33,9 @@
 static_assert(kHgOpConv == OP_CONV && kHgOpDecode == OP_DECODE && kHgDtypeField == kDtypeField &&
                   sizeof(OpRecord) == sizeof(int64_t) * kOpFields,
               "head_gate.h reads the executor's op records");
+static_assert(kCfOpConv == OP_CONV && kCfOpDecode == OP_DECODE && kCfOpYoloRaw == OP_YOLORAW &&
+                  kCfDtypeField == kDtypeField,
+              "chain_fuse.h reads the executor's op records");
 bool g_head_gate = [] {
   const char* e = std::getenv("ARENA_HEAD_GATE");
   return e == nullptr || std::atoi(e) != 0;
@@ -41,8 +44,14 @@
   const char* e = std::getenv("ARENA_HEAD_SPLIT");
   return e == nullptr ? 1 : std::max(0, std::min(2, std::atoi(e)));
 }();
-}
-
+int g_up_read = [] {
+  const char* e = std::getenv("ARENA_UP_READ");
+  return e == nullptr ? 1 : std::max(0, std::min(2, std::atoi(e)));
+}();
+}
+
+void set_up_read(int v) { g_up_read = std::max(0, std::min(2, v)); }
+int get_up_read() { return g_up_read; }
 void set_head_gate(bool v) { g_head_gate = v; }
 bool get_head_gate() { return g_head_gate; }
 void set_head_split(int v) { g_head_split = std::max(0, std::min(2, v)); }
@@ -286,6 +295,7 @@
   gate_first_.clear();
   for (const HeadGatePair& gp : gate_pairs_)
     gate_first_.push_back(head_gate_first_conv(prog_[0].data(), n_ops, kOpFields, gp));
+  up_pairs_ = up_read_pairs(prog_.empty() ? nullptr : prog_[0].data(), n_ops, kOpFields);
 }
 
 int Executor::crop_cap_for(int B) const { return std::max(cfg_.min_crop_cap, B * cfg_.crop_cap_per_image); }
@@ -338,6 +348,9 @@
     bk.marks_off[i] = (int64_t)abytes;
     abytes += align_up((size_t)B * head_mark_cells((int)f[13]) * head_mark_cells((int)f[14]) * sizeof(int), 256);
   }
+  bk.up_clear.assign(up_pairs_.size(), 0);
+  for (size_t i = 0; i < up_pairs_.size(); ++i)
+    bk.up_clear[i] = up_read_ranges_clear(prog_[0].data(), kOpFields, up_pairs_[i], offsets, n_buffers, B);
   for (int s = 0; s < n_slots_; ++s) {
     ARENA_HIP_CHECK(hipMalloc(&bk.d_arena[s], abytes));
     ARENA_HIP_CHECK(hipMemset(bk.d_arena[s], 0, abytes));
@@ -497,6 +510,7 @@
     bk.exec_order.clear();
     bk.gated.clear();
     bk.launches.clear();
+    bk.up_fused.clear();
   }
   auto capture_range = [&](size_t a, size_t b) {
     std::vector<OpRecord> part(prog_.begin() + a, prog_.begin() + b);
@@ -508,6 +522,11 @@
         if (gate[k] != nullptr) bk.gated.push_back((int)(a + order[k]));
       }
       for (const Step& st : launch_plan(part, bk, (int)a, 0)) bk.launches.emplace_back((int)(a + st.pos), st.kind);
+      std::vector<int> up_src;
+      std::vector<char> up_drop;
+      up_read_plan(part, bk, (int)a, 0, up_src, up_drop);
+      for (size_t k = 0; k < up_src.size(); ++k)
+        if (up_src[k] >= 0) bk.up_fused.emplace_back((int)a + up_src[k], (int)(a + k));
     }
     hipGraph_t g = nullptr;
     hipGraphExec_t ge = nullptr;
@@ -680,6 +699,24 @@
   return steps;
 }
 
+void Executor::up_read_plan(const std::vector<OpRecord>& prog, const Bucket& bk, int op_offset, int force_impl,
+                            std::vector<int>& src, std::vector<char>& drop_y2) const {
+  src.assign(prog.size(), -1);
+  drop_y2.assign(prog.size(), 0);
+  if (g_up_read == 0 || (g_up_read == 1 && bk.info.B < kUpReadMinBucket) || force_impl != 0) return;
+  for (size_t i = 0; i < up_pairs_.size(); ++i) {
+    const UpReadPair& pr = up_pairs_[i];
+    const long lp = (long)pr.producer - op_offset, lc = (long)pr.consumer - op_offset;
+    if (lp < 0 || lc >= (long)prog.size() || pr.consumer >= (int)prog_.size()) continue;
+    if (i >= bk.up_clear.size() || !bk.up_clear[i]) continue;
+    if (prog[lp] != prog_[pr.producer] || prog[lc] != prog_[pr.consumer]) continue;
+    const int impl = pr.consumer < (int)bk.impl.size() ? bk.impl[pr.consumer] : 0;
+    if (!(impl >= kF32X3G && impl < kF32X3G + kF32X3GVariants)) continue;
+    src[lc] = (int)lp;
+    drop_y2[lp] = 1;
+  }
+}
+
 void Executor::enqueue_program(const std::vector<OpRecord>& prog, Bucket& bk, Slot& sl, hipStream_t s_main,
                                int op_offset, int force_impl) {
   Ctrl* ctrl = (Ctrl*)resolve(bk, sl, BUF_CTRL, 0, 1);
@@ -691,6 +728,9 @@
   const uint8_t* W = d_weights_;
 
   const std::vector<Step> steps = launch_plan(prog, bk, op_offset, force_impl);
+  std::vector<int> up_src;
+  std::vector<char> up_drop;
+  up_read_plan(prog, bk, op_offset, force_impl, up_src, up_drop);
   auto marks_of = [&](const HeadGatePair* gp) {
     return (int*)(bk.d_arena[sl.idx] + bk.marks_off[(size_t)(gp - gate_pairs_.data())]);
   };
@@ -748,6 +788,15 @@
         p.B = batch(r[30]);
         p.bdev = bdev(r[30]);
         if (r[41] != 0) p.w3 = W + r[40];
+        if (step.kind == LAUNCH_OP && up_drop[oi]) p.y2 = nullptr;
+        if (step.kind == LAUNCH_OP && up_src[oi] >= 0) {
+          const OpRecord& pr = prog[(size_t)up_src[oi]];
+          p.x2 = resolve(bk, sl, pr[10], pr[11], 4);
+          p.x2s = (int)pr[12];
+          p.x2_c = (int)pr[15];
+          p.x2_H = (int)pr[13];
+          p.x2_W = (int)pr[14];
+        }
         {
           const int64_t ln = r[kLaneField];
           const int li = ln >= 1 && ln <= kMaxLanes ? (int)ln : 0;
diff --git a/csrc/runtime/executor.h b/csrc/runtime/executor.h
--- a/csrc/runtime/executor.h
+++ b/csrc/runtime/executor.h
@@ -13,6 +13,7 @@
 #include <vector>
 
 #include "../kernels/launch.h"
+#include "chain_fuse.h"
 #include "head_gate.h"
 #include "head_marks.h"
 #include "instance.h"
@@ -34,6 +35,9 @@
 int get_head_split();
 constexpr int kHeadSplitMinBucket = 32;
 constexpr int kHeadSplitBoxVariant = 2, kHeadSplitClsVariant = 9;
+void set_up_read(int v);
+int get_up_read();
+constexpr int kUpReadMinBucket = 16;
 enum LaunchKind : int { LAUNCH_OP = 0, LAUNCH_CLS_WINDOW = 1, LAUNCH_BOX_WINDOW = 2, LAUNCH_MARK = 3 };
 
 enum OpType : int64_t {
@@ -183,6 +187,8 @@
     std::vector<int> exec_order, gated;
     std::vector<std::pair<int, int>> launches;
     std::vector<int64_t> marks_off;
+    std::vector<char> up_clear;
+    std::vector<std::pair<int, int>> up_fused;
   };
   struct Step {
     size_t pos;
@@ -210,6 +216,8 @@
                                 std::vector<const HeadGatePair*>& gate) const;
   std::vector<Step> launch_plan(const std::vector<OpRecord>& prog, const Bucket& bk, int op_offset,
                                 int force_impl) const;
+  void up_read_plan(const std::vector<OpRecord>& prog, const Bucket& bk, int op_offset, int force_impl,
+                    std::vector<int>& src, std::vector<char>& drop_y2) const;
 
  public:
   std::vector<int> exec_order(int B) const {
@@ -223,6 +231,10 @@
   std::vector<std::pair<int, int>> launch_order(int B) const {
     auto it = buckets_.find(B);
     return it == buckets_.end() ? std::vector<std::pair<int, int>>{} : it->second.launches;
+  }
+  std::vector<std::pair<int, int>> up_read_fused(int B) const {
+    auto it = buckets_.find(B);
+    return it == buckets_.end() ? std::vector<std::pair<int, int>>{} : it->second.up_fused;
   }
   std::vector<int> conv_choices(int B) const {
     auto it = buckets_.find(B);
@@ -255,6 +267,7 @@
   std::vector<OpRecord> prog_, cls_prog_;
   std::vector<HeadGatePair> gate_pairs_;
   std::vector<int> gate_first_;
+  std::vector<UpReadPair> up_pairs_;
   std::map<int, Bucket> buckets_;
   Slot slots_[kMaxSlots];
   int n_slots_ = 2;
diff --git a/inference_arena_amd/ops/functional.py b/inference_arena_amd/ops/functional.py
--- a/inference_arena_amd/ops/functional.py
+++ b/inference_arena_amd/ops/functional.py
@@ -37,7 +37,7 @@
                 res: torch.Tensor | None = None, res_coff: int = 0, out2: torch.Tensor | None = None,
                 out2_coff: int = 0, f32out: bool = False, out_hw=None, bdev: torch.Tensor | None = None,
                 packed=None, impl: int = 0, pw=None, pw_out: torch.Tensor | None = None, pw_out_coff: int = 0,
-                gate=None, window=None, marks=None) -> torch.Tensor:
+                gate=None, window=None, marks=None, x2=None) -> torch.Tensor:
     f32 = x.dtype == torch.float32
     B, H, W, Cx = x.shape
     cout, cin_w, kh, kw = w.shape
@@ -94,6 +94,13 @@
                 or tuple(mt.shape) != (B, (Ho + 7) // 8, (Wo + 7) // 8)):
             raise ValueError("conv2d_nhwc: marks must be contiguous int32 [B, ceil(Ho / 8), ceil(Wo / 8)]")
         pwd.update({"marks": _ptr(mt), "mark_uh": int(uh), "mark_uw": int(uw), "mark_halo": int(halo)})
+    if x2 is not None:
+        t2, c2, coff2 = x2 if len(x2) == 3 else (*x2, 0)
+        if (t2.dtype != torch.float32 or t2.device != x.device or not t2.is_contiguous() or t2.dim() != 4
+                or t2.shape[0] != B or (2 * t2.shape[1], 2 * t2.shape[2]) != (H, W) or c2 <= 0 or coff2 < 0
+                or coff2 + c2 > t2.shape[3]):
+            raise ValueError("conv2d_nhwc: x2 must be contiguous float32 [B, H / 2, W / 2, >= coff + c2]")
+        pwd.update({"x2": _ptr(t2, coff2), "x2s": t2.shape[3], "x2_c": int(c2), "x2_H": t2.shape[1], "x2_W": t2.shape[2]})
     skd = {}
     if 171 <= int(impl) < 180:
         ws = torch.empty(8 * B * Ho * Wo * cpad, dtype=torch.float32, device=x.device)
diff --git a/inference_arena_amd/utils/settings.py b/inference_arena_amd/utils/settings.py
--- a/inference_arena_amd/utils/settings.py
+++ b/inference_arena_amd/utils/settings.py
@@ -55,6 +55,7 @@
     ARENA_IR_S2K16: int = 1
     ARENA_HEAD_GATE: int = 1
     ARENA_HEAD_SPLIT: int = 1
+    ARENA_UP_READ: int = 1
 
     @classmethod
     def from_env(cls, env_file: str | Path = ".env", **overrides) -> "Settings":
```
